# microsoft/singleshotpose

Hardware: AMD Instinct MI355X
Metric: images/sec (fwd+bwd) yolo-pose 416x416 bs=64/GPU (higher is better)
Workload: dtype f32; 1 GPU; cfg/yolo-pose.cfg train step (zero_grad+fwd+RegionLoss+bwd+grad all-reduce+SGD), 416x416, batch 64/GPU, random-init weights, 1 label/image; global_batch=64, parallelism=dp1

## Files before the change

include/ssp_hip.h:

```cpp
#ifndef SSP_HIP_H
#define SSP_HIP_H
#include <stdint.h>

#ifdef __cplusplus
extern "C" {
#endif

const char* ssp_last_error(void);
int ssp_abi_version(void);
int ssp_set_option(const char* name, int value);


int ssp_conv_fwd(const float* in, const float* wt, float* out, const float* bias, float* stats, int B, int H, int W,
                 int Cin, int Cout, int ldin, int ldout, int R, int accumulate, int plan, float* workspace,
                 int64_t workspace_floats, void* stream);
int ssp_conv_fwd_affine(const float* in, const float* wt, float* out, const float* scale, const float* shift,
                        float slope, int B, int H, int W, int Cin, int Cout, int ldin, int ldout, int R, int plan,
                        float* workspace, int64_t workspace_floats, void* stream);
int ssp_conv_stats_tile_m(int B, int H, int W, int Cin, int Cout, int R, int plan);
int ssp_conv_stats_tiles(int B, int H, int W, int Cin, int Cout, int R, int plan);
int64_t ssp_conv_stats_floats(int B, int H, int W, int Cin, int Cout, int R, int plan);
int ssp_conv_plan_wino_tile(int plan);
int64_t ssp_conv_wino_tiles(int B, int H, int W, int tile);
int ssp_wino_filter_transform_t(const float* w9, float* U, int rows, int K, int tile, void* stream);
int ssp_wino_filter_transform(const float* w9, float* U, int rows, int K, void* stream);
int64_t ssp_conv_workspace_floats(int B, int H, int W, int Cin, int Cout, int R, int plan);

int ssp_conv_dgrad(const float* dy, const float* wt, float* dx, int B, int H, int W, int Cout_dy, int Cin_dx, int lddy,
                   int lddx, int R, int accumulate, int plan, float* workspace, int64_t workspace_floats,
                   void* stream);

int ssp_conv_dgrad_bnbwd(const float* dy, const float* wt, float* dx, int B, int H, int W, int Cout_dy, int Cin_dx,
                         int lddy, int lddx, int R, int plan, float* workspace, int64_t workspace_floats,
                         const float* raw, int ldraw, const float* scale, const float* shift, const float* mean,
                         const float* invstd, float slope, float* partial, int partial_rows, void* stream);

int ssp_conv_wgrad(const float* dy, const float* x, float* dw, int B, int H, int W, int Cin, int Cout, int lddy,
                   int ldx, int R, void* stream);
int ssp_conv_wgrad_route(int B, int H, int W, int Cin, int Cout, int lddy, int ldx, int R);
int64_t ssp_conv_wgrad_wino_workspace_floats_t(int B, int H, int W, int Cin, int Cout, int tile);
int ssp_wino_input_transform_t(const float* x, int ldx, float* V, int B, int H, int W, int C, int tile, void* stream);
int ssp_conv_wgrad_wino_t(const float* dy, const float* x, float* dw, int B, int H, int W, int Cin, int Cout, int lddy,
                          int ldx, int tile, float* workspace, int64_t workspace_floats, void* stream);
int64_t ssp_conv_wgrad_wino_workspace_floats(int B, int H, int W, int Cin, int Cout);
int ssp_conv_wgrad_wino(const float* dy, const float* x, float* dw, int B, int H, int W, int Cin, int Cout, int lddy,
                        int ldx, float* workspace, int64_t workspace_floats, void* stream);

int ssp_bn_fwd_finalize(const float* stats, int ntile, int tile_m, int M, int C, const float* gamma,
                        const float* beta, float* running_mean, float* running_var, float momentum, float eps,
                        float* mean, float* invstd, float* scale, float* shift, void* stream);
int ssp_bn_eval_prepare(int C, const float* gamma, const float* beta, const float* running_mean,
                        const float* running_var, float eps, float* mean, float* invstd, float* scale, float* shift,
                        void* stream);
int ssp_bn_act_fwd(const float* x, int ldx, float* out, int ldo, const float* scale, const float* shift, int C, int B,
                   int H, int W, int pool, float slope, void* stream);
int ssp_bn_bwd_blocks(void);
int ssp_bn_act_bwd(const float* x, int ldx, const float* g, int ldg, float* dx, int lddx, const float* scale,
                   const float* shift, const float* mean, const float* invstd, int C, int B, int H, int W, int pool,
                   float slope, int training, float* partial, float* dgamma, float* dbeta, float* c1, float* c2,
                   void* stream);
int ssp_bn_act_bwd_partials(const float* x, int ldx, const float* g, int ldg, float* dx, int lddx, const float* scale,
                            const float* shift, const float* mean, const float* invstd, int C, int B, int H, int W,
                            float slope, int training, float* partial, int npartial, int zero_after, float* dgamma,
                            float* dbeta, float* c1, float* c2, void* stream);
int ssp_bn_act_bwd_affine(const float* x, int ldx, const float* g, int ldg, float* dx, int lddx, const float* scale,
                          const float* shift, const float* mean, const float* invstd, int C, int B, int H, int W, int pool,
                          float slope, void* stream);
int ssp_bn_bwd_finalize(float* partial, int npartial, int C, int64_t npix, int training, int zero_after, float* dgamma,
                        float* dbeta, float* c1, float* c2, void* stream);
int ssp_colsum(const float* g, int ldg, int64_t M, int C, float* out, void* stream);

int ssp_first_tile_pixels(void);
int ssp_first_groups(int B, int H, int W);
int ssp_first_fwd_stats(const float* x, const float* wt, float* stats, int B, int H, int W, void* stream);
int ssp_first_fwd_apply(const float* x, const float* wt, const float* scale, const float* shift, float slope, float* out,
                        int ldo, int B, int H, int W, void* stream);
int ssp_first_conv_raw(const float* x, const float* wt, float* raw, int ldraw, int B, int H, int W, void* stream);
int ssp_first_bwd_reduce(const float* x, const float* wt, const float* g, int ldg, const float* scale, const float* shift,
                         const float* mean, const float* invstd, float slope, float* partial, int B, int H, int W,
                         void* stream);
int ssp_first_bwd_wgrad(const float* x, const float* wt, const float* g, int ldg, const float* scale, const float* shift,
                        const float* mean, const float* invstd, const float* c1, const float* c2, float slope, float* dw,
                        float* workspace, int64_t workspace_floats, int B, int H, int W, void* stream);
int64_t ssp_first_wgrad_workspace_floats(int B, int H, int W);
int ssp_first_bwd_dgrad(const float* x, const float* wt, const float* g, int ldg, const float* scale, const float* shift,
                        const float* mean, const float* invstd, const float* c1, const float* c2, float slope, float* dx,
                        int B, int H, int W, void* stream);

int ssp_sgd_step(float* param, const float* grad, float* momentum_buf, int64_t n, float lr, float momentum,
                 float dampening, float weight_decay, int nesterov, int first_step, void* stream);
#define SSP_SGD_MAX_TUPLES 16
int ssp_sgd_step_table(float* param, const float* grad, float* momentum_buf, int64_t param_floats, int64_t grad_floats,
                       int64_t momentum_floats, const int64_t* table_dev, const int64_t* table_host, int nseg,
                       const float* hyper, int ntuple, void* stream);

int ssp_nchw_to_nhwc(const float* src, float* dst, int B, int C, int H, int W, int Cpad, int ld, void* stream);
int ssp_nhwc_to_nchw(const float* src, float* dst, int B, int C, int H, int W, int ld, void* stream);
int ssp_u8hwc_to_nhwc(const unsigned char* src, float* dst, int B, int H, int W, int C, int Cpad, int ld, void* stream);
typedef struct SspResampleDesc {
  const void* src;
  void* dst;
  const void* bounds;
  const void* kk;
  const void* img;
  const void* mask;
  const void* lut;
  int src_w, src_h, src_pitch;
  int x0, y0;
  int row0;
  int dst_w, dst_h, dst_pitch;
  int ksize, img_pitch, reserved;
} SspResampleDesc;
int ssp_resample_u8(const SspResampleDesc* descs_dev, int count, int pass, int epilogue, int max_dst_pixels, void* stream);
#define SSP_COMPOSITE_MAX_OBJS 8
typedef struct SspCompositeDesc {
  const void* scene;
  const void* scene_mask;
  const void* bg;
  void* out;
  const void* obj[SSP_COMPOSITE_MAX_OBJS];
  const void* obj_mask[SSP_COMPOSITE_MAX_OBJS];
  long long nbytes;
  int nobj, reserved;
} SspCompositeDesc;
int ssp_composite_u8(const SspCompositeDesc* descs_dev, int count, long long max_bytes, void* stream);
int ssp_distort_u8(const unsigned char* rgb, unsigned char* out, int64_t npix, const unsigned char* lut, int mode, void* stream);
int ssp_repack_fwd(const float* w, float* out, int Cout, int Cin, int Cinp, int R, void* stream);
int ssp_repack_dgrad(const float* w, float* out, int Cout, int Cin, int Coutp, int R, void* stream);
int ssp_repack_dgrad_packed(const float* wp, float* out, int Cout, int Cin, int Coutp, int R, void* stream);
int ssp_unpack_grad(const float* dwp, float* grad, int Cout, int Cin, int Cinp, int R, void* stream);
int ssp_reorg(const float* src, int lds, float* dst, int ldd, int C, int B, int H, int W, int backward,
              int accumulate, void* stream);
int ssp_copy_channels(const float* src, int lds, float* dst, int ldd, int C, int64_t M, int accumulate, void* stream);
int ssp_maxpool_fwd(const float* x, int ldx, float* out, int ldo, int C, int B, int H, int W, void* stream);
int ssp_maxpool_bwd(const float* x, int ldx, const float* g, int ldg, float* dx, int lddx, int C, int B, int H, int W,
                    int accumulate, void* stream);

int ssp_maxpool_s1_fwd(const float* x, int ldx, float* out, int ldo, int C, int B, int H, int W, void* stream);
int ssp_maxpool_s1_bwd(const float* x, int ldx, const float* g, int ldg, float* dx, int lddx, int C, int B, int H, int W,
                       int accumulate, void* stream);
int ssp_shortcut_fwd(const float* a, int lda, const float* b, int ldb, float* out, int ldo, int C, int64_t M, float slope,
                     void* stream);
int ssp_shortcut_bwd(const float* g, int ldg, const float* out, int ldo, float* da, int ldda, int acc_a, float* db, int lddb,
                     int acc_b, int C, int64_t M, float slope, void* stream);
int ssp_avgpool_fwd(const float* x, int ldx, float* out, int ldo, int C, int B, int H, int W, void* stream);
int ssp_avgpool_bwd(const float* g, int ldg, float* dx, int lddx, int C, int B, int H, int W, int accumulate, void* stream);
int ssp_softmax_fwd(const float* x, int ldx, float* y, int ldy, int C, int64_t M, void* stream);
int ssp_softmax_bwd(const float* y, int ldy, const float* g, int ldg, float* dx, int lddx, int C, int64_t M, int accumulate,
                    void* stream);

int ssp_region_loss(const float* out, const void* target, int target_is_f64, float* grad, float* partials,
                    float* stats, int nB, int nA, int nC, int nH, int nW, int num_keypoints, float noobject_scale,
                    float object_scale, float coord_scale, float class_scale, float thresh, int conf_on, int multi,
                    const float* anchors, int anchor_step, void* stream);
int ssp_region_decode_argmax(const float* out, float* boxes, int nB, int nA, int nC, int nH, int nW,
                             int num_keypoints, int only_objectness, void* stream);

int ssp_region_decode_all(const float* out, float* rows, int nB, int nA, int nC, int nH, int nW, int num_keypoints,
                          void* stream);

int ssp_region_match_multi(const float* out, const float* target, float* rows, int* meta, int nB, int nA, int nC, int nH,
                           int nW, int num_keypoints, float conf_thresh, int only_objectness, int im_width, int im_height,
                           void* stream);

int ssp_pnp_batched(const double* pts3d, const double* pts2d, const double* K, double* Rt, int n, int N, int max_iter,
                    void* stream);

int ssp_pose_errors(const double* vertices, int N, const double* Rt_gt, const double* Rt_pr, const double* K,
                    int k_per_pose, int n, double* out, void* stream);
int ssp_pts_diameter(const double* pts, int N, double* out, double* scratch, void* stream);
int ssp_pose_errors_models(const double* verts, const int* model_off, const int* pose_model, int nM, const double* Rt_gt,
                           const double* Rt_pr, const double* K, int k_per_pose, int n, double* out, void* stream);
int64_t ssp_adds_workspace_doubles(int n, int maxN);
int ssp_adds_errors(const double* verts, const int* model_off, const int* pose_model, int nM, int maxN,
                    const double* Rt_gt, const double* Rt_pr, int n, double* out, double* workspace,
                    int64_t workspace_doubles, void* stream);

int ssp_prof_enable(int mask);
int ssp_prof_nkinds(void);
int ssp_prof_collect(double* ms, double* work, int64_t* count);

#ifdef __cplusplus
}
#endif
#endif
```

singleshotpose_amd/_lib.py:

```python
import ctypes
import os
from ctypes import c_char_p, c_double, c_float, c_int, c_int64, c_void_p

_HERE = os.path.dirname(os.path.abspath(__file__))
LIB_PATH = os.environ.get("SSP_HIP_LIB") or os.path.join(_HERE, "libssp_hip.so")


class SspError(RuntimeError):
    pass


_lib = None

P = c_void_p
I = c_int
F = c_float
L = c_int64

_SIGS = {
    "ssp_abi_version": [],
    "ssp_set_option": [c_char_p, I],
    "ssp_conv_fwd": [P, P, P, P, P, I, I, I, I, I, I, I, I, I, I, P, L, P],
    "ssp_conv_fwd_affine": [P, P, P, P, P, F, I, I, I, I, I, I, I, I, I, P, L, P],
    "ssp_conv_stats_tile_m": [I, I, I, I, I, I, I],
    "ssp_conv_workspace_floats": [I, I, I, I, I, I, I],
    "ssp_conv_stats_tiles": [I, I, I, I, I, I, I],
    "ssp_conv_stats_floats": [I, I, I, I, I, I, I],
    "ssp_conv_plan_wino_tile": [I],
    "ssp_conv_wino_tiles": [I, I, I, I],
    "ssp_wino_filter_transform": [P, P, I, I, P],
    "ssp_wino_filter_transform_t": [P, P, I, I, I, P],
    "ssp_conv_dgrad": [P, P, P, I, I, I, I, I, I, I, I, I, I, P, L, P],
    "ssp_conv_dgrad_bnbwd": [P, P, P, I, I, I, I, I, I, I, I, I, P, L, P, I, P, P, P, P, F, P, I, P],
    "ssp_bn_act_bwd_partials": [P, I, P, I, P, I, P, P, P, P, I, I, I, I, F, I, P, I, I, P, P, P, P, P],
    "ssp_conv_wgrad": [P, P, P, I, I, I, I, I, I, I, I, P],
    "ssp_conv_wgrad_route": [I, I, I, I, I, I, I, I],
    "ssp_conv_wgrad_wino": [P, P, P, I, I, I, I, I, I, I, P, L, P],
    "ssp_conv_wgrad_wino_workspace_floats": [I, I, I, I, I],
    "ssp_conv_wgrad_wino_t": [P, P, P, I, I, I, I, I, I, I, I, P, L, P],
    "ssp_conv_wgrad_wino_workspace_floats_t": [I, I, I, I, I, I],
    "ssp_bn_fwd_finalize": [P, I, I, I, I, P, P, P, P, F, F, P, P, P, P, P],
    "ssp_bn_eval_prepare": [I, P, P, P, P, F, P, P, P, P, P],
    "ssp_bn_act_fwd": [P, I, P, I, P, P, I, I, I, I, I, F, P],
    "ssp_bn_bwd_blocks": [],
    "ssp_bn_act_bwd": [P, I, P, I, P, I, P, P, P, P, I, I, I, I, I, F, I, P, P, P, P, P, P],
    "ssp_bn_act_bwd_affine": [P, I, P, I, P, I, P, P, P, P, I, I, I, I, I, F, P],
    "ssp_bn_bwd_finalize": [P, I, I, L, I, I, P, P, P, P, P],
    "ssp_first_tile_pixels": [],
    "ssp_first_groups": [I, I, I],
    "ssp_first_fwd_stats": [P, P, P, I, I, I, P],
    "ssp_first_fwd_apply": [P, P, P, P, F, P, I, I, I, I, P],
    "ssp_first_conv_raw": [P, P, P, I, I, I, I, P],
    "ssp_first_bwd_reduce": [P, P, P, I, P, P, P, P, F, P, I, I, I, P],
    "ssp_first_bwd_wgrad": [P, P, P, I, P, P, P, P, P, P, F, P, P, L, I, I, I, P],
    "ssp_first_bwd_dgrad": [P, P, P, I, P, P, P, P, P, P, F, P, I, I, I, P],
    "ssp_wino_input_transform_t": [P, I, P, I, I, I, I, I, P],
    "ssp_first_wgrad_workspace_floats": [I, I, I],
    "ssp_colsum": [P, I, L, I, P, P],
    "ssp_pose_errors": [P, I, P, P, P, I, I, P, P],
    "ssp_pts_diameter": [P, I, P, P, P],
    "ssp_pose_errors_models": [P, P, P, I, P, P, P, I, I, P, P],
    "ssp_adds_workspace_doubles": [I, I],
    "ssp_adds_errors": [P, P, P, I, I, P, P, I, P, P, L, P],
    "ssp_sgd_step": [P, P, P, L, F, F, F, F, I, I, P],
    "ssp_sgd_step_table": [P, P, P, L, L, L, P, P, I, P, I, P],
    "ssp_nchw_to_nhwc": [P, P, I, I, I, I, I, I, P],
    "ssp_nhwc_to_nchw": [P, P, I, I, I, I, I, P],
    "ssp_u8hwc_to_nhwc": [P, P, I, I, I, I, I, I, P],
    "ssp_resample_u8": [P, I, I, I, I, P],
    "ssp_distort_u8": [P, P, L, P, I, P],
    "ssp_composite_u8": [P, I, L, P],
    "ssp_repack_fwd": [P, P, I, I, I, I, P],
    "ssp_repack_dgrad": [P, P, I, I, I, I, P],
    "ssp_repack_dgrad_packed": [P, P, I, I, I, I, P],
    "ssp_unpack_grad": [P, P, I, I, I, I, P],
    "ssp_reorg": [P, I, P, I, I, I, I, I, I, I, P],
    "ssp_copy_channels": [P, I, P, I, I, L, I, P],
    "ssp_maxpool_fwd": [P, I, P, I, I, I, I, I, P],
    "ssp_maxpool_bwd": [P, I, P, I, P, I, I, I, I, I, I, P],
    "ssp_maxpool_s1_fwd": [P, I, P, I, I, I, I, I, P],
    "ssp_maxpool_s1_bwd": [P, I, P, I, P, I, I, I, I, I, I, P],
    "ssp_shortcut_fwd": [P, I, P, I, P, I, I, L, F, P],
    "ssp_shortcut_bwd": [P, I, P, I, P, I, I, P, I, I, I, L, F, P],
    "ssp_avgpool_fwd": [P, I, P, I, I, I, I, I, P],
    "ssp_avgpool_bwd": [P, I, P, I, I, I, I, I, I, P],
    "ssp_softmax_fwd": [P, I, P, I, I, L, P],
    "ssp_softmax_bwd": [P, I, P, I, P, I, I, L, I, P],
    "ssp_region_loss": [P, P, I, P, P, P, I, I, I, I, I, I, F, F, F, F, F, I, I, P, I, P],
    "ssp_region_decode_argmax": [P, P, I, I, I, I, I, I, I, P],
    "ssp_region_decode_all": [P, P, I, I, I, I, I, I, P],
    "ssp_region_match_multi": [P, P, P, P, I, I, I, I, I, I, F, I, I, I, P],
    "ssp_pnp_batched": [P, P, P, P, I, I, I, P],
    "ssp_prof_enable": [I],
    "ssp_prof_nkinds": [],
    "ssp_prof_collect": [P, P, P],
}

_RET64 = ('ssp_conv_workspace_floats', 'ssp_conv_wgrad_wino_workspace_floats', 'ssp_conv_wgrad_wino_workspace_floats_t',
          'ssp_conv_stats_floats', 'ssp_conv_wino_tiles', 'ssp_first_wgrad_workspace_floats', 'ssp_adds_workspace_doubles')

PROF_KINDS = ("conv_fwd", "conv_dgrad", "conv_wgrad", "bn_act", "layout", "region", "optim", "first_block_fwd",
              "first_block_bwd", "wino_fwd", "wino_dgrad", "wino_wgrad", "onchip_fwd", "onchip_dgrad", "onchip_wgrad")


def csrc_digest():
    import glob
    import hashlib
    h = hashlib.sha1()
    files = sorted(glob.glob(os.path.join(_HERE, 'csrc', '*.hip')) + glob.glob(os.path.join(_HERE, 'csrc', '*.h')))
    files.append(os.path.join(os.path.dirname(_HERE), 'include', 'ssp_hip.h'))
    for f in files:
        h.update(os.path.basename(f).encode())
        with open(f, 'rb') as fp:
            h.update(fp.read())
    return h.hexdigest()


def exported_symbols():
    return ["ssp_last_error"] + list(_SIGS.keys())


def load():
    global _lib
    if _lib is not None:
        return _lib
    if not os.path.exists(LIB_PATH):
        raise SspError(
            "libssp_hip.so not found at %s - build it with `python -c 'import __graft_entry__ as g; g.build()'` "
            "or `make -C singleshotpose_amd/csrc`; there is no CPU fallback for the HIP path" % LIB_PATH)
    lib = ctypes.CDLL(LIB_PATH)
    lib.ssp_last_error.restype = c_char_p
    lib.ssp_last_error.argtypes = []
    for name, args in _SIGS.items():
        fn = getattr(lib, name)
        fn.restype = c_int64 if name in _RET64 else c_int
        fn.argtypes = args
    _lib = lib
    return lib


PROF_MASK = [0]


def call(name, *args):
    lib = load()
    if name == 'ssp_prof_enable':
        PROF_MASK[0] = int(args[0])
    rc = getattr(lib, name)(*args)
    if rc != 0:
        msg = lib.ssp_last_error()
        raise SspError("%s failed (%d): %s" % (name, rc, msg.decode() if msg else "?"))
    return rc


def query(name, *args):
    return getattr(load(), name)(*args)
```

singleshotpose_amd/csrc/conv_igemm.hip:

```cpp
#include "conv_igemm_common.h"
#include "conv_wino.h"

template <int BM, int BN, int WM, int WN, int BK, int ABL = 0, int PASS = 0>
__global__ void __launch_bounds__(WM* WN * 64, 2) conv_igemm_kernel(ConvArgs p) {
  constexpr int NT = WM * WN * 64;
  constexpr int LS = BK + 4;
  constexpr int TPR = BK / 4;
  constexpr int RPP = NT / TPR;
  constexpr int APASS = (BM + RPP - 1) / RPP;
  constexpr int BPASS = (BN + RPP - 1) / RPP;
  constexpr int WTM = BM / WM, WTN = BN / WN;
  constexpr int TM = WTM / 32, TN = WTN / 32;
  constexpr int VEC = (BK >= 8) ? 4 : 2;
  constexpr int NQ = BK / (2 * VEC);
  constexpr int SLOT = (BM + BN) * LS;
  static_assert(WTM % 32 == 0 && WTN % 32 == 0, "wave tile must be a multiple of the 32x32 MFMA");
  static_assert(NQ >= 1, "BK too small");

  extern __shared__ __attribute__((aligned(16))) float smem[];

  const int ntiles = p.ntile_m * p.ntile_n;
  const int nwg = ntiles * p.ksplit;
  const int lid0 = p.xcd_remap ? ssp_xcd_remap(blockIdx.x, nwg) : (int)blockIdx.x;
  const int split = lid0 / ntiles, lid = lid0 - split * ntiles;
// ... 264 lines not shown
        const float d = v[k] - mean[k];
        mean[k] += d * inv;
        m2[k] += d * (v[k] - mean[k]);
      }
      float* dst = out + (int64_t)m * ldout + c;
      f32x4 o = {v[0] * e4[0] + b4[0], v[1] * e4[1] + b4[1], v[2] * e4[2] + b4[2], v[3] * e4[3] + b4[3]};
#pragma unroll
      for (int k = 0; k < 4; ++k) o[k] = o[k] > 0.f ? o[k] : o[k] * act_slope;
      if (accumulate) {
        const f32x4 prev = *reinterpret_cast<const f32x4*>(dst);
        o[0] += prev[0]; o[1] += prev[1]; o[2] += prev[2]; o[3] += prev[3];
      }
      *reinterpret_cast<f32x4*>(dst) = o;
      if (bnb) {
        const f32x4 xr = *reinterpret_cast<const f32x4*>(bn_raw + (int64_t)m * bn_ld + c);
#pragma unroll
        for (int k = 0; k < 4; ++k) {
          const float y = xr[k] * bsc[k] + bsh[k];
          const float dyv = y > 0.f ? o[k] : o[k] * bn_slope;
          s1[k] += dyv;
          s2[k] += dyv * ((xr[k] - bmu[k]) * bis[k]);
        }
      }
    }
  }
  __shared__ float red[16][16][9];
  if (bnb) {
#pragma unroll
    for (int k = 0; k < 4; ++k) { red[pp][gl][1 + k] = s1[k]; red[pp][gl][5 + k] = s2[k]; }
    __syncthreads();
    if (tid < 64) {
      const int q = tid >> 2, k = tid & 3;
      const int ch = blockIdx.y * 64 + tid;
      if (ch < Cout) {
        float a = 0.f, b = 0.f;
        for (int w = 0; w < 16; ++w) { a += red[w][q][1 + k]; b += red[w][q][5 + k]; }
        const int t = m0 / tile_m;
        if (ntile_all > bn_nslot) {
          float* dst = bn_partial + ((int64_t)(t % bn_nslot) * Cout + ch) * 2;
          atomicAdd(dst, a);
          atomicAdd(dst + 1, b);
        } else {
          float* dst = bn_partial + ((int64_t)t * Cout + ch) * 2;
          dst[0] = a;
          dst[1] = b;
        }
      }
    }
    return;
  }
  if (stats == nullptr) return;
  red[pp][gl][0] = cnt;
#pragma unroll
  for (int k = 0; k < 4; ++k) { red[pp][gl][1 + k] = mean[k]; red[pp][gl][5 + k] = m2[k]; }
  __syncthreads();
  if (tid < 64) {
    const int q = tid >> 2, k = tid & 3;
    const int ch = blockIdx.y * 64 + tid;
    if (ch < Cout) {
      float n_ = red[0][q][0], mu = red[0][q][1 + k], s2 = red[0][q][5 + k];
      for (int w = 1; w < 16; ++w) chan_combine(n_, mu, s2, red[w][q][0], red[w][q][1 + k], red[w][q][5 + k]);
      float* st = stats + ((int64_t)(m0 / tile_m) * Cout + ch) * 2;
      st[0] = mu;
      st[1] = s2;
    }
  }
}

template <int BM, int BN, int WM, int WN, int BK, int ABL = 0, int PASS = 0>
static int launch_cfg(ConvArgs a, hipStream_t stream, int extra_lds = 0) {
  a.ntile_m = ssp_cdiv(a.M, BM);
  a.ntile_n = ssp_cdiv(a.Cout, BN);
  const int niter_total = a.R * a.R * (a.Cin / BK);
  a.it_per_split = ssp_cdiv(niter_total, a.ksplit);
  a.ksplit = ssp_cdiv(niter_total, a.it_per_split);
  dim3 grid(a.ntile_m * a.ntile_n * a.ksplit), block(WM * WN * 64);
  const int lds_bytes = 3 * (BM + BN) * (BK + 4) * 4 + extra_lds;
  auto kern = conv_igemm_kernel<BM, BN, WM, WN, BK, ABL, PASS>;
  static SspKernelCache cache;
  if (int rc = ssp_kernel_prepare((const void*)kern, lds_bytes, WM * WN * 64, &cache, nullptr, "conv_igemm")) return rc;
  hipLaunchKernelGGL(kern, grid, block, lds_bytes, stream, a);
  SSP_CHECK_LAUNCH("conv_igemm");
  return SSP_OK;
}

int ssp_conv_igemm_dma_launch(ConvArgs& a, int bm, int slots, int tail_ks, int is_dgrad, hipStream_t stream);

struct IgemmPlan { int bm, ksplit, slots, tail; };
static IgemmPlan select_plan(int M, int Cin, int Cout, int R, int plan_code) {
  IgemmPlan pl = {256, 1, 0, 0};
  if (Cout <= 64) {
    if (Cout > 32 && Cin % 16 == 0 && ssp_option(SSP_OPT_IGEMM_VARIANT) != 50) pl.bm = 128;
    if (Cin % 16 == 0 && Cout % 4 == 0 && ssp_option(SSP_OPT_IGEMM_VARIANT) != 50 && ssp_option(SSP_OPT_IGEMM_VARIANT) != 30) {
      const int64_t tiles = ssp_cdiv(M, pl.bm);
      const int niter = R * R * (Cin / 16);
      if (tiles < 256) {
        int64_t ks = 512 / tiles;
        if (ks > niter / 8) ks = niter / 8;
        if (ks > 8) ks = 8;
        if (ks >= 2) pl.ksplit = (int)ks;
      }
    }
    return pl;
  }
  pl.bm = 128;
  const int forced = plan_code > 0 ? plan_code : ssp_option(SSP_OPT_IGEMM_PLAN);
  if (forced > 0) {
    const int ftail = forced / 100000, fbm = (forced / 100) % 1000, fks = (forced / 10) % 10, fsl = forced % 10;
    const int niter16 = (Cin % 16 == 0) ? R * R * (Cin / 16) : 0;
    const bool ok = (fbm == 64 || fbm == 128) && fks >= 1 && (fsl == 3 || fsl == 4 || fsl == 8) &&
                    (fks == 1 || (niter16 / fks >= 8 && Cout % 4 == 0)) && Cin % 16 == 0 &&
                    (ftail == 0 || (ftail >= 2 && ftail <= 9 && fks == 1 && Cout % 4 == 0 && niter16 / ftail >= 8));
    if (ok) { pl.bm = fbm; pl.ksplit = fks; pl.slots = fsl; pl.tail = ftail; return pl; }
  }
  const int variant = ssp_option(SSP_OPT_IGEMM_VARIANT);
  if (variant == 20 || variant == 22) { pl.bm = 64; return pl; }
  if (variant >= 70 && variant <= 75) {
    const int niter = R * R * (Cin / 16);
    if (Cin % 16 == 0 && Cout % 4 == 0 && niter / (variant - 68) >= 8) pl.ksplit = variant - 68;
    return pl;
  }
  if (variant != 0 && variant != 30 && variant != 50 && variant != 61 && variant != 62 && variant != 63) return pl;
  const int64_t t128 = (int64_t)ssp_cdiv(M, 128) * ssp_cdiv(Cout, 128);
  const int64_t t64 = (int64_t)ssp_cdiv(M, 64) * ssp_cdiv(Cout, 128);
  if (t128 > 1400) return pl;
  auto wave_eff = [](int64_t wgs, int slots) { return (double)wgs / (double)(((wgs + slots - 1) / slots) * slots); };
  double best = wave_eff(t128, 512);
  const double e64 = 0.97 * wave_eff(t64, 768);
  if (e64 > best) { best = e64; pl.bm = 64; }
  if (variant == 30 || Cin % 16 != 0 || Cout % 4 != 0) return pl;
  const int niter = R * R * (Cin / 16);
  const double flop_time = 2.0 * M * (double)Cout * R * R * Cin / 110e12;
  for (int sp = 2; sp <= 6; ++sp) {
    if (niter / sp < 128) break;
    const double traffic = (2.0 * sp + 1.0) * (double)M * Cout * 4.0 / 4.0e12;
    const double eff = wave_eff(t128 * sp, 512) / (1.0 + traffic / flop_time);
    if (eff > best + 0.02) { best = eff; pl.bm = 128; pl.ksplit = sp; }
  }
  return pl;
}
int ssp_conv_tile_m(int M, int Cin, int Cout, int R, int plan) {
  if (ssp_wino_plan_tile(plan)) return 0;
  return select_plan(M, Cin, Cout, R, plan).bm;
}
int64_t ssp_conv_ws_floats(int M, int Cin, int Cout, int R, int plan) {
  IgemmPlan pl = select_plan(M, Cin, Cout, R, plan);
  const int deepest = pl.ksplit > pl.tail ? pl.ksplit : pl.tail;
  return deepest > 1 ? (int64_t)deepest * M * Cout : 0;
}

int64_t ssp_wino_ws_floats(int B, int H, int W, int Cin, int Cout, int tile) {
  return ssp_wino_planes(tile) * ssp_wino_tiles(B, H, W, tile) * ((int64_t)Cin + Cout);
}

static int wino_launch(ConvArgs& a, int B, int H, int W, float* ws, int64_t ws_floats, int plan, int prof_kind,
                       hipStream_t stream) {
  const int bm = (plan / 100) % 1000, slots = plan % 10, tile = ssp_wino_plan_tile(plan), P = ssp_wino_planes(tile);
  SSP_CHECK_ARG(a.R == 3 && a.Cin % 16 == 0 && a.Cout >= 64 && a.Cout % 4 == 0 && a.ldout % 4 == 0 && (((uintptr_t)a.out) & 15) == 0,
                "conv (Winograd plan): needs a 3x3 filter, Cin %% 16 == 0, Cout >= 64 and %% 4 == 0, an aligned output");
  SSP_CHECK_ARG((bm == 64 || bm == 128) && (slots == 3 || slots == 4 || slots == 8) && (plan / 10) % 10 == 1 &&
                    (plan / 100000) % 10 == 0, "conv: bad Winograd plan code %d", plan);
  const int64_t T = ssp_wino_tiles(B, H, W, tile);
  SSP_CHECK_ARG(T < (1ll << 31) && P * T * (int64_t)a.Cin < (1ll << 40), "conv (Winograd plan): too many tiles");
  SSP_CHECK_ARG(ws != nullptr && ws_floats >= ssp_wino_ws_floats(B, H, W, a.Cin, a.Cout, tile) && (((uintptr_t)ws) & 15) == 0,
                "conv (Winograd plan): needs a workspace of %lld floats (ssp_conv_workspace_floats)",
                (long long)ssp_wino_ws_floats(B, H, W, a.Cin, a.Cout, tile));
  SSP_CHECK_ARG((int64_t)(128 + 2) * a.Cin * 4 + (int64_t)a.Cin * 4 < (1ll << 31), "conv (Winograd plan): Cin too large");
  if (a.bn_partial != nullptr) SSP_CHECK_ARG(a.bn_ld % 4 == 0, "conv (Winograd plan): bn_ld must be a multiple of 4");
  SspProfScope prof(prof_kind, stream, 2.0 * (double)a.M * a.Cout * 9.0 * a.Cin);
  float* V = ws;
  float* Mw = ws + P * T * a.Cin;
  const int wkind = prof_kind == SSP_PROF_CONV_DGRAD ? SSP_PROF_WINO_DGRAD : SSP_PROF_WINO_FWD;
  if (int rc = ssp_wino_input_launch(a.in, a.ldin, V, B, H, W, a.Cin, tile, wkind, stream)) return rc;
  ConvArgs g = a;
  g.in = V; g.wt = a.wt; g.out = Mw; g.bias = nullptr; g.escale = nullptr; g.act_slope = 1.f; g.stats = nullptr;
  g.H = 1; g.W = (int)T; g.ldin = a.Cin; g.ldout = a.Cout; g.R = 1; g.M = (int)T; g.accumulate = 0;
  g.divW = ssp_fastdiv((unsigned)T); g.divH = ssp_fastdiv(1u);
  g.ws = nullptr; g.ksplit = 1; g.probe = 0;
  g.bn_partial = nullptr; g.bn_raw = nullptr;
  g.batch = P; g.batch_in = T * a.Cin; g.batch_wt = (int64_t)a.Cout * a.Cin; g.batch_out = T * a.Cout;
  if (int rc = ssp_conv_igemm_dma_launch(g, bm, slots, 0, prof_kind == SSP_PROF_CONV_DGRAD, stream)) return rc;
  WinoOutArgs o;
  o.Mw = Mw; o.out = a.out; o.bias = a.bias; o.escale = a.escale; o.act_slope = a.act_slope; o.stats = a.stats;
  o.Cout = a.Cout; o.ldout = a.ldout; o.accumulate = a.accumulate;
  o.bn_raw = a.bn_raw; o.bn_scale = a.bn_scale; o.bn_shift = a.bn_shift; o.bn_mean = a.bn_mean; o.bn_invstd = a.bn_invstd;
  o.bn_partial = a.bn_partial; o.bn_nslot = a.bn_nslot; o.bn_ld = a.bn_ld; o.bn_slope = a.bn_slope;
  return ssp_wino_output_launch(o, B, H, W, tile, wkind, stream);
}

int ssp_conv_igemm_launch(const float* in, const float* wt, float* out, const float* bias, float* stats, int B, int H,
                          int W, int Cin, int Cout, int ldin, int ldout, int R, int accumulate, float* ws,
                          int64_t ws_floats, int plan, int prof_kind, hipStream_t stream, const float* escale,
                          float act_slope, const SspBnBwdFuse* bnb) {
  SSP_CHECK_ARG(R == 1 || R == 3, "conv: only 1x1 and 3x3 filters are supported (got %d)", R);
  SSP_CHECK_ARG(Cin % 4 == 0 && Cin > 0, "conv: Cin must be a positive multiple of 4 (got %d)", Cin);
  SSP_CHECK_ARG(ldin % 4 == 0 && ldin >= Cin, "conv: ldin must be a multiple of 4 and >= Cin");
  SSP_CHECK_ARG(ldout >= Cout && Cout > 0, "conv: ldout < Cout");
  SSP_CHECK_ARG((int64_t)B * H * W < (1ll << 31), "conv: too many pixels");
  SSP_CHECK_ARG((((uintptr_t)in) & 15) == 0 && (((uintptr_t)wt) & 15) == 0, "conv: in/wt must be 16-byte aligned");
  ConvArgs a;
  a.in = in; a.wt = wt; a.out = out; a.bias = bias; a.stats = stats; a.escale = escale; a.act_slope = act_slope;
  a.H = H; a.W = W; a.Cin = Cin; a.Cout = Cout; a.ldin = ldin; a.ldout = ldout; a.R = R;
  a.M = B * H * W; a.accumulate = accumulate;
  a.divW = ssp_fastdiv((unsigned)W); a.divH = ssp_fastdiv((unsigned)H);
  a.xcd_remap = ssp_option(SSP_OPT_IGEMM_XCD);
  a.probe = ssp_option(SSP_OPT_IGEMM_VARIANT) == 63 ? 2 : 0;
  a.tail_begin = 0; a.tail_ks = 0; a.tail_it_per_split = 0; a.ws_row0 = 0; a.ws_rows = a.M; a.col_major = 0;
  a.bn_raw = nullptr; a.bn_scale = a.bn_shift = a.bn_mean = a.bn_invstd = nullptr; a.bn_partial = nullptr;
  a.bn_ld = 0; a.bn_slope = 1.f; a.bn_nslot = 1;
  a.batch = 0; a.batch_in = a.batch_wt = a.batch_out = 0;
  if (bnb != nullptr && bnb->partial != nullptr) {
    SSP_CHECK_ARG(accumulate == 0 && bias == nullptr && stats == nullptr && escale == nullptr,
                  "conv: the fused BatchNorm-backward reductions need a plain (non-accumulating) data-gradient launch");
    SSP_CHECK_ARG(bnb->raw != nullptr && bnb->scale != nullptr && bnb->shift != nullptr && bnb->mean != nullptr &&
                  bnb->invstd != nullptr && bnb->ldraw >= Cout && Cout % 4 == 0 && bnb->ldraw % 4 == 0 &&
                  ((((uintptr_t)bnb->raw) | ((uintptr_t)bnb->scale) | ((uintptr_t)bnb->shift) | ((uintptr_t)bnb->mean) |
                    ((uintptr_t)bnb->invstd)) & 15) == 0,
                  "conv: bad BatchNorm-backward operands (16-byte aligned, Cout %% 4 == 0, ldraw >= Cout)");
    a.bn_raw = bnb->raw; a.bn_ld = bnb->ldraw; a.bn_scale = bnb->scale; a.bn_shift = bnb->shift; a.bn_mean = bnb->mean;
    a.bn_invstd = bnb->invstd; a.bn_slope = bnb->slope; a.bn_partial = bnb->partial;
    SSP_CHECK_ARG(bnb->nslot >= 1, "conv: the BatchNorm-backward partial buffer needs at least one row");
    a.bn_nslot = bnb->nslot;
  }
  if (ssp_wino_plan_fused(plan)) {
    a.ksplit = 1; a.ws = nullptr;
    return ssp_wino_fused_launch(a, B, H, W, prof_kind, stream);
  }
  if (ssp_wino_plan_tile(plan)) return wino_launch(a, B, H, W, ws, ws_floats, plan, prof_kind, stream);
  IgemmPlan pl = select_plan(a.M, Cin, Cout, R, plan);
  if (Cout <= 64 && pl.ksplit > 1 &&
      (ws == nullptr || ws_floats < (int64_t)pl.ksplit * a.M * Cout || ldout % 4 != 0 || (((uintptr_t)out) & 15) != 0))
    pl.ksplit = 1;
  a.ksplit = pl.ksplit;
  a.ws = ws;
  if (pl.ksplit > 1)
    SSP_CHECK_ARG(ldout % 4 == 0 && (((uintptr_t)out) & 15) == 0, "conv: split-K output must be 16-byte aligned with ldout % 4 == 0");
  if (pl.ksplit > 1)
    SSP_CHECK_ARG(ws != nullptr && ws_floats >= (int64_t)pl.ksplit * a.M * Cout,
                  "conv: this shape runs split-K x%d and needs a workspace of %lld floats (ssp_conv_workspace_floats)",
                  pl.ksplit, (long long)pl.ksplit * a.M * Cout);
  if (pl.tail > 1) {
    SSP_CHECK_ARG(ws != nullptr && ws_floats >= (int64_t)pl.tail * a.M * Cout && ldout % 4 == 0 && (((uintptr_t)out) & 15) == 0,
                  "conv: the hybrid plan (tail split x%d) needs an aligned output and a workspace of %lld floats "
                  "(ssp_conv_workspace_floats)", pl.tail, (long long)pl.tail * a.M * Cout);
  }
  SspProfScope prof(prof_kind, stream, 2.0 * (double)a.M * Cout * (double)(R * R * Cin));
  const int variant = ssp_option(SSP_OPT_IGEMM_VARIANT);
  const int bk = (Cin % 32 == 0 && (variant == 2 || variant == 4 || variant == 5)) ? 32 : ((Cin % 16 == 0) ? 16 : 4);
  int rc = SSP_OK;
  if (Cout > 64) {
    switch (variant) {
      case 3: if (bk >= 16) return launch_cfg<256, 128, 4, 2, 16>(a, stream); break;
      case 4: if (bk == 32) return launch_cfg<128, 128, 2, 2, 32, 1>(a, stream); break;
      case 5: if (bk == 32) return launch_cfg<128, 128, 2, 2, 32, 2>(a, stream); break;
#ifdef SSP_PROBES
      case 10: if (bk >= 16) return launch_cfg<128, 128, 2, 2, 16, 1>(a, stream); break;
      case 14: if (bk >= 16) return launch_cfg<128, 128, 2, 2, 16, 1 | 4 | 8 | 16>(a, stream); break;
      case 17: if (bk >= 16) return launch_cfg<128, 128, 2, 2, 16, 1 | 4 | 8 | 16 | 32>(a, stream); break;
      case 40: if (bk >= 16) return launch_cfg<128, 128, 2, 2, 16, 29 | 64>(a, stream); break;
      case 41: if (bk >= 16) return launch_cfg<128, 128, 2, 2, 16, 29 | 128>(a, stream); break;
      case 42: if (bk >= 16) return launch_cfg<128, 128, 2, 2, 16, 29 | 256>(a, stream); break;
      case 43: if (bk >= 16) return launch_cfg<128, 128, 2, 2, 16, 29 | 64 | 128 | 256>(a, stream); break;
      case 18: if (bk >= 16) return launch_cfg<128, 128, 2, 2, 16, 32>(a, stream); break;
#endif
      case 21: if (bk >= 16) return launch_cfg<128, 64, 2, 2, 16>(a, stream); break;
      case 22: if (bk >= 16) return launch_cfg<64, 64, 2, 2, 16>(a, stream); break;
      default: break;
    }
    if (bk >= 16 && variant != 50 && ((int64_t)(128 + 2 * W + 2) * ldin * 4 + (int64_t)Cin * 4 < (1ll << 31))) {
      rc = ssp_conv_igemm_dma_launch(a, pl.bm, pl.slots, pl.tail, prof_kind == SSP_PROF_CONV_DGRAD, stream);
    } else if (pl.bm == 64) {
      rc = (bk >= 16) ? launch_cfg<64, 128, 2, 2, 16>(a, stream)
                      : (prof_kind == SSP_PROF_CONV_DGRAD ? launch_cfg<64, 128, 2, 2, 4, 0, 1>(a, stream) : launch_cfg<64, 128, 2, 2, 4>(a, stream));
    } else if (bk == 32) {
      rc = launch_cfg<128, 128, 2, 2, 32>(a, stream);
    } else if (bk == 16) {
      rc = launch_cfg<128, 128, 2, 2, 16>(a, stream);
    } else {
      rc = prof_kind == SSP_PROF_CONV_DGRAD ? launch_cfg<128, 128, 2, 2, 4, 0, 1>(a, stream) : launch_cfg<128, 128, 2, 2, 4>(a, stream);
    }
  } else if (Cout > 32) {
    if (pl.bm == 128) {
      SSP_CHECK_ARG((int64_t)(128 + 2 * W + 2) * ldin * 4 + (int64_t)Cin * 4 < (1ll << 31),
                    "conv: image rows too long for the 32-bit tile offsets of the LDS-direct loader");
      rc = ssp_conv_igemm_dma_launch(a, 128, 0, 0, prof_kind == SSP_PROF_CONV_DGRAD, stream);
    } else
      rc = (bk >= 16) ? launch_cfg<256, 64, 4, 1, 16>(a, stream) : launch_cfg<256, 64, 4, 1, 4>(a, stream);
  } else if (bk >= 16 && variant != 50 && ((int64_t)(256 + 2 * W + 2) * ldin * 4 + (int64_t)Cin * 4 < (1ll << 31))) {
    rc = ssp_conv_igemm_dma_launch(a, 256, 0, 0, prof_kind == SSP_PROF_CONV_DGRAD, stream);
  } else {
    rc = (bk >= 16) ? launch_cfg<256, 32, 4, 1, 16>(a, stream) : launch_cfg<256, 32, 4, 1, 4>(a, stream);
  }
  if (rc != SSP_OK) return rc;
  const int rt = (stats == nullptr && a.bn_partial == nullptr && a.M <= 16384) ? 16 : pl.bm;
  if (pl.ksplit > 1) {
    hipLaunchKernelGGL(splitk_reduce_kernel, dim3(ssp_cdiv(a.M, rt), ssp_cdiv(Cout, 64)), dim3(256), 0, stream, ws, pl.ksplit, out, ldout,
                       bias, stats, a.M, Cout, rt, accumulate, escale, act_slope, 0, a.bn_raw, a.bn_ld, a.bn_scale,
                       a.bn_shift, a.bn_mean, a.bn_invstd, a.bn_slope, a.bn_partial, a.bn_nslot, ssp_cdiv(a.M, pl.bm));
    SSP_CHECK_LAUNCH("splitk_reduce");
  } else if (a.tail_ks > 1) {
    hipLaunchKernelGGL(splitk_reduce_kernel, dim3(ssp_cdiv(a.M - a.ws_row0, rt), ssp_cdiv(Cout, 64)), dim3(256), 0, stream, ws,
                       a.tail_ks, out, ldout, bias, stats, a.M, Cout, rt, accumulate, escale, act_slope, a.ws_row0,
                       a.bn_raw, a.bn_ld, a.bn_scale, a.bn_shift, a.bn_mean, a.bn_invstd, a.bn_slope, a.bn_partial, a.bn_nslot,
                       ssp_cdiv(a.M, pl.bm));
    SSP_CHECK_LAUNCH("splitk_reduce(tail)");
  }
  return SSP_OK;
}
```

singleshotpose_amd/csrc/conv_wgrad.hip:

```cpp
#include "conv_wino.h"

struct WgradArgs {
  const float* dy;
  const float* x;
  float* dw;
  int H, W, Cin, Cout, lddy, ldx, R, M;
  int ntile_co, ntile_ci, nsplit, chunk_m;
};

template <int BMO, int BNI, int WM, int WN, int WK>
__global__ void __launch_bounds__(256, 2) conv_wgrad_kernel(WgradArgs p) {
  static_assert(WM * WN * WK == 4, "256-thread workgroups");
  constexpr int NT = 256;
  constexpr int RA = 16 * WK;
  constexpr int WTM = BMO / WM, WTN = BNI / WN;
  constexpr int TM = WTM / 32, TN = WTN / 32;
  constexpr int F4A = RA * BMO / 4, F4B = RA * BNI / 4;
  constexpr int APASS = (F4A + NT - 1) / NT, BPASS = (F4B + NT - 1) / NT;
  constexpr int SLOT = RA * (BMO + BNI);
  static_assert(WTM % 32 == 0 && WTN % 32 == 0, "wave tile must be a multiple of 32x32");

  extern __shared__ __attribute__((aligned(16))) float smem[];

  const int taps = p.R * p.R;
// ... 198 lines not shown
      }
      g_reg[i] = v;
    }
  };
  auto store_lds = [&](int buf) {
#pragma unroll
    for (int i = 0; i < 2; ++i)
      *reinterpret_cast<f32x4v*>(As + (buf * RA + a_row0 + i * 32) * LSA + a_c4) = a_reg[i];
#pragma unroll
    for (int i = 0; i < 3; ++i) {
      const int tap = g_tap0 + 4 * i;
      if (tap < 9) *reinterpret_cast<f32x4v*>(Bs + (buf * RA + g_pix) * LSB + tap * 4) = g_reg[i];
    }
  };

  f32x4v acc[2][3];
#pragma unroll
  for (int i = 0; i < 2; ++i)
#pragma unroll
    for (int j = 0; j < 3; ++j) acc[i][j] = f32x4v{0.f, 0.f, 0.f, 0.f};

  load_global(0);
  store_lds(0);
  __syncthreads();
  const int li = lane & 15, lk = lane >> 4;
  for (int it = 0; it < niter; ++it) {
    const int buf = it & 1;
    if (it + 1 < niter) load_global(it + 1);
    const float* Ab = As + (buf * RA + wid * 16 + lk) * LSA + li;
    const float* Bb = Bs + (buf * RA + wid * 16 + lk) * LSB + li;
#pragma unroll
    for (int kk = 0; kk < 4; ++kk) {
      float av[2], bv[3];
#pragma unroll
      for (int i = 0; i < 2; ++i) av[i] = Ab[kk * 4 * LSA + i * 16];
#pragma unroll
      for (int j = 0; j < 3; ++j) bv[j] = Bb[kk * 4 * LSB + j * 16];
#pragma unroll
      for (int i = 0; i < 2; ++i)
#pragma unroll
        for (int j = 0; j < 3; ++j) acc[i][j] = __builtin_amdgcn_mfma_f32_16x16x4f32(av[i], bv[j], acc[i][j], 0, 0, 0);
    }
    if (it + 1 < niter) store_lds(buf ^ 1);
    __syncthreads();
  }

  float* red = smem;
#pragma unroll
  for (int i = 0; i < 2; ++i)
#pragma unroll
    for (int j = 0; j < 3; ++j)
#pragma unroll
      for (int r = 0; r < 4; ++r) red[(wid * CO + i * 16 + lk * 4 + r) * NCOL + j * 16 + li] = acc[i][j][r];
  __syncthreads();
  for (int e = tid; e < CO * 36; e += 256) {
    int co = e / 36, col = e % 36;
    float v = red[(0 * CO + co) * NCOL + col] + red[(1 * CO + co) * NCOL + col] + red[(2 * CO + co) * NCOL + col] +
              red[(3 * CO + co) * NCOL + col];
    atomicAdd(p.dw + co * 36 + col, v);
  }
}

template <int BMO, int BNI, int WM, int WN, int WK>
static int launch_wgrad(WgradArgs a, hipStream_t stream) {
  constexpr int RA = 16 * WK;
  a.ntile_co = ssp_cdiv(a.Cout, BMO);
  a.ntile_ci = ssp_cdiv(a.Cin, BNI);
  const int64_t tiles = (int64_t)a.ntile_co * a.ntile_ci * a.R * a.R;
  const int lds_bytes = 3 * RA * (BMO + BNI) * 4;
  auto kern = conv_wgrad_kernel<BMO, BNI, WM, WN, WK>;
  static SspKernelCache cache;
  int slots = 0;
  if (int rc = ssp_kernel_prepare((const void*)kern, lds_bytes, 256, &cache, &slots, "conv_wgrad")) return rc;
  const int64_t max_split = (a.M + RA * 8 - 1) / (RA * 8);
  int64_t lo = (2 * (int64_t)slots + tiles - 1) / tiles, hi = (5 * (int64_t)slots) / tiles;
  if (lo < 1) lo = 1;
  if (hi < lo) hi = lo;
  if (lo > max_split) lo = max_split;
  if (hi > max_split) hi = max_split;
  int64_t nsplit = lo;
  double best = -1.0;
  for (int64_t sp = lo; sp <= hi; ++sp) {
    const double waves = (double)(tiles * sp) / slots;
    const double eff = waves / (double)((tiles * sp + slots - 1) / slots);
    if (eff > best + 1e-3) { best = eff; nsplit = sp; }
  }
  int64_t chunk = (a.M + nsplit - 1) / nsplit;
  chunk = (chunk + RA - 1) / RA * RA;
  nsplit = (a.M + chunk - 1) / chunk;
  a.nsplit = (int)nsplit;
  a.chunk_m = (int)chunk;
  dim3 grid((unsigned)(tiles * nsplit)), block(256);
  hipLaunchKernelGGL(kern, grid, block, lds_bytes, stream, a);
  SSP_CHECK_LAUNCH("conv_wgrad");
  return SSP_OK;
}

int ssp_conv_wgrad_dma_try(const float* dy, const float* x, float* dw, int B, int H, int W, int Cin, int Cout, int lddy,
                           int ldx, int R, hipStream_t stream, int batch = 0, int64_t batch_dy = 0, int64_t batch_x = 0,
                           int64_t batch_dw = 0, int overwrite = 0);

int ssp_conv_wgrad_launch(const float* dy, const float* x, float* dw, int B, int H, int W, int Cin, int Cout,
                          int lddy, int ldx, int R, hipStream_t stream) {
  SSP_CHECK_ARG(R == 1 || R == 3, "wgrad: only 1x1 and 3x3 filters are supported (got %d)", R);
  SSP_CHECK_ARG(Cin % 4 == 0 && Cin > 0, "wgrad: Cin must be a positive multiple of 4 (got %d)", Cin);
  SSP_CHECK_ARG(ldx % 4 == 0 && ldx >= Cin, "wgrad: ldx must be a multiple of 4 and >= Cin");
  SSP_CHECK_ARG(lddy % 4 == 0 && lddy >= Cout, "wgrad: lddy must be a multiple of 4 and >= Cout");
  SSP_CHECK_ARG((int64_t)B * H * W < (1ll << 31), "wgrad: too many pixels");
  SSP_CHECK_ARG((((uintptr_t)dy) & 15) == 0 && (((uintptr_t)x) & 15) == 0, "wgrad: dy/x must be 16-byte aligned");
  WgradArgs a;
  a.dy = dy; a.x = x; a.dw = dw;
  a.H = H; a.W = W; a.Cin = Cin; a.Cout = Cout; a.lddy = lddy; a.ldx = ldx; a.R = R; a.M = B * H * W;
  SspProfScope prof(SSP_PROF_CONV_WGRAD, stream, 2.0 * (double)a.M * Cout * (double)(R * R * Cin));
  const int route = ssp_wgrad_route(B, H, W, Cin, Cout, lddy, ldx, R, 0, ssp_option(SSP_OPT_WGRAD_VARIANT));
  if (route / 100000000 == SSP_WGRAD_LDS) {
    const int r = ssp_conv_wgrad_dma_try(dy, x, dw, B, H, W, Cin, Cout, lddy, ldx, R, stream);
    if (r != 0) return r < 0 ? r : SSP_OK;
    ssp_set_error("wgrad: the LDS-direct launcher declined route %d", route);
    return SSP_ERR_ARG;
  }
  switch (route) {
    case ssp_wgrad_code(SSP_WGRAD_C4, 2, false, false, 32, 4): {
      int64_t chunk = (a.M + 2047) / 2048;
      chunk = (chunk + 63) / 64 * 64;
      a.chunk_m = (int)chunk;
      a.nsplit = ssp_cdiv(a.M, chunk);
      hipLaunchKernelGGL(conv_wgrad_c4_kernel, dim3(a.nsplit), dim3(256), 0, stream, a);
      SSP_CHECK_LAUNCH("conv_wgrad_c4");
      return SSP_OK;
    }
    case ssp_wgrad_code(SSP_WGRAD_REG, 3, false, false, 128, 128): return launch_wgrad<128, 128, 2, 2, 1>(a, stream);
    case ssp_wgrad_code(SSP_WGRAD_REG, 3, false, false, 128, 64): return launch_wgrad<128, 64, 2, 2, 1>(a, stream);
    case ssp_wgrad_code(SSP_WGRAD_REG, 3, false, false, 128, 32): return launch_wgrad<128, 32, 4, 1, 1>(a, stream);
    case ssp_wgrad_code(SSP_WGRAD_REG, 3, false, false, 64, 128): return launch_wgrad<64, 128, 2, 2, 1>(a, stream);
    case ssp_wgrad_code(SSP_WGRAD_REG, 3, false, false, 64, 64): return launch_wgrad<64, 64, 2, 2, 1>(a, stream);
    case ssp_wgrad_code(SSP_WGRAD_REG, 3, false, false, 64, 32): return launch_wgrad<64, 32, 2, 1, 2>(a, stream);
    case ssp_wgrad_code(SSP_WGRAD_REG, 3, false, false, 32, 128): return launch_wgrad<32, 128, 1, 4, 1>(a, stream);
    case ssp_wgrad_code(SSP_WGRAD_REG, 3, false, false, 32, 64): return launch_wgrad<32, 64, 1, 2, 2>(a, stream);
    case ssp_wgrad_code(SSP_WGRAD_REG, 3, false, false, 32, 32): return launch_wgrad<32, 32, 1, 1, 4>(a, stream);
  }
  ssp_set_error("wgrad: no instantiation for route %d", route);
  return SSP_ERR_ARG;
}


int64_t ssp_conv_wgrad_wino_ws_floats(int B, int H, int W, int Cin, int Cout, int tile) {
  if (tile == SSP_WINO_WGRAD_FUSED) return ssp_wino_wgrad_fused_ws_floats(Cin, Cout);
  if (tile != 2 && tile != 4) return 0;
  const int64_t T = ssp_wino_tiles(B, H, W, tile);
  return ssp_wino_planes(tile) * (T * ((int64_t)Cin + Cout) + (int64_t)Cin * Cout);
}
int ssp_conv_wgrad_wino_launch(const float* dy, const float* x, float* dw, int B, int H, int W, int Cin, int Cout, int lddy,
                               int ldx, int tile, float* ws, int64_t ws_floats, hipStream_t stream) {
  if (tile == SSP_WINO_WGRAD_FUSED) return ssp_wino_wgrad_fused_launch(dy, x, dw, B, H, W, Cin, Cout, lddy, ldx, ws, ws_floats, stream);
  SSP_CHECK_ARG(tile == 2 || tile == 4, "wgrad (Winograd): tile must be 2, 4 or 12 (F(2x2) with both transforms on the chip)");
  SSP_CHECK_ARG(Cin % 16 == 0 && Cout % 16 == 0 && Cin >= 64 && Cout >= 64, "wgrad (Winograd): needs Cin, Cout >= 64 and %% 16 == 0");
  SSP_CHECK_ARG(ldx % 4 == 0 && ldx >= Cin && lddy % 4 == 0 && lddy >= Cout, "wgrad (Winograd): bad leading dimensions");
  SSP_CHECK_ARG((((uintptr_t)dy) | ((uintptr_t)x) | ((uintptr_t)dw) | ((uintptr_t)ws)) % 16 == 0, "wgrad (Winograd): operands must be 16-byte aligned");
  const int64_t T = ssp_wino_tiles(B, H, W, tile);
  const int P = ssp_wino_planes(tile);
  SSP_CHECK_ARG(T >= 16 && T < (1ll << 31), "wgrad (Winograd): tile count out of range (>= 16 tiles)");
  SSP_CHECK_ARG(ws != nullptr && ws_floats >= ssp_conv_wgrad_wino_ws_floats(B, H, W, Cin, Cout, tile),
                "wgrad (Winograd): needs a workspace of %lld floats (ssp_conv_wgrad_wino_workspace_floats)",
                (long long)ssp_conv_wgrad_wino_ws_floats(B, H, W, Cin, Cout, tile));
  SspProfScope prof(SSP_PROF_CONV_WGRAD, stream, 2.0 * (double)B * H * W * Cout * 9.0 * Cin);
  float* V = ws;
  float* dM = V + P * T * Cin;
  float* dU = dM + P * T * Cout;
  if (x != nullptr)
    if (int rc = ssp_wino_input_launch(x, ldx, V, B, H, W, Cin, tile, SSP_PROF_WINO_WGRAD, stream)) return rc;
  if (int rc = ssp_wino_outgrad_launch(dy, lddy, dM, B, H, W, Cout, tile, stream)) return rc;
  const int r = ssp_conv_wgrad_dma_try(dM, V, dU, 1, 1, (int)T, Cin, Cout, Cout, Cin, 1, stream, P, T * Cout, T * Cin,
                                       (int64_t)Cout * Cin, 1);
  if (r < 0) return r;
  SSP_CHECK_ARG(r == 1, "wgrad (Winograd): shape declined by the LDS-direct filter-gradient kernel");
  return ssp_wino_wgrad_finish_launch(dU, dw, Cout, Cin, tile, stream);
}
```

singleshotpose_amd/csrc/conv_wino.h:

```cpp
#pragma once
#include "ssp_common.h"

#define SSP_WINO2_PLAN 9000000
#define SSP_WINO4_PLAN 8000000
#define SSP_WINOF_PLAN 7000000
static inline int ssp_wino_plan_fused(int plan) { return plan >= SSP_WINOF_PLAN && plan < SSP_WINOF_PLAN + 1000000; }
static inline int ssp_wino_plan_tile(int plan) {
  if (plan >= SSP_WINO2_PLAN && plan < SSP_WINO2_PLAN + 1000000) return 2;
  if (plan >= SSP_WINO4_PLAN && plan < SSP_WINO4_PLAN + 1000000) return 4;
  if (ssp_wino_plan_fused(plan)) return 2;
  return 0;
}

#define SSP_WINO_TG 16

struct WinoOutArgs {
  const float* Mw;
  float* out;
  const float* bias;
  const float* escale;
  float act_slope;
  float* stats;
  int Cout, ldout, accumulate;
  const float* bn_raw;
  const float* bn_scale;
  const float* bn_shift;
  const float* bn_mean;
  const float* bn_invstd;
  float* bn_partial;
  int bn_nslot, bn_ld;
  float bn_slope;
};

int64_t ssp_wino_tiles(int B, int H, int W, int tile);
int ssp_wino_planes(int tile);
int64_t ssp_wino_stat_groups(int B, int H, int W, int tile);
int ssp_wino_input_launch(const float* in, int ldin, float* V, int B, int H, int W, int C, int tile, int prof_kind, hipStream_t stream);
int ssp_wino_filter_launch(const float* w, float* U, int rows, int K, int tile, hipStream_t stream);
int ssp_wino_outgrad_launch(const float* dy, int lddy, float* dM, int B, int H, int W, int C, int tile, hipStream_t stream);
int ssp_wino_wgrad_finish_launch(const float* dU, float* dw, int rows, int K, int tile, hipStream_t stream);
int ssp_wino_output_launch(const WinoOutArgs& a, int B, int H, int W, int tile, int prof_kind, hipStream_t stream);

struct ConvArgs;
int ssp_wino_fused_launch(const ConvArgs& a, int B, int H, int W, int prof_kind, hipStream_t stream);
int ssp_wino_fused_stat_groups(int B, int H, int W, int Cout);
bool ssp_wino_fused_fits(int B, int H, int W, int Cin, int Cout, int R);

#define SSP_WINO_WGRAD_FUSED 12
int ssp_wino_wgrad_fused_launch(const float* dy, const float* x, float* dw, int B, int H, int W, int Cin, int Cout, int lddy,
                                int ldx, float* ws, int64_t ws_floats, hipStream_t stream);
int64_t ssp_wino_wgrad_fused_ws_floats(int Cin, int Cout);
bool ssp_wino_wgrad_fused_fits(int B, int H, int W, int Cin, int Cout);
```

singleshotpose_amd/csrc/conv_wino.hip:

```cpp
#include <utility>

#include "conv_wino.h"

template <typename F, int... Is>
__device__ __forceinline__ void ssp_sfor_impl(F&& f, std::integer_sequence<int, Is...>) {
  (f(std::integral_constant<int, Is>{}), ...);
}
template <int N, typename F>
__device__ __forceinline__ void ssp_sfor(F&& f) {
  ssp_sfor_impl(f, std::make_integer_sequence<int, N>{});
}

template <typename V>
__device__ __forceinline__ void wino_mad(V& acc, const float c, const V& x) {
  if (c == 1.f) acc += x;
  else if (c == -1.f) acc -= x;
  else if (c != 0.f) acc += x * c;
}

template <int N> struct WinoMat;
template <> struct WinoMat<2> {
  static constexpr int A = 4;
  static constexpr float BT[4][4] = {{1.f, 0.f, -1.f, 0.f}, {0.f, 1.f, 1.f, 0.f}, {0.f, -1.f, 1.f, 0.f}, {0.f, 1.f, 0.f, -1.f}};
  static constexpr float G[4][3] = {{1.f, 0.f, 0.f}, {0.5f, 0.5f, 0.5f}, {0.5f, -0.5f, 0.5f}, {0.f, 0.f, 1.f}};
  static constexpr float AT[2][4] = {{1.f, 1.f, 1.f, 0.f}, {0.f, 1.f, -1.f, -1.f}};
};
template <> struct WinoMat<4> {
  static constexpr int A = 6;
  static constexpr float BT[6][6] = {{1.f, -1.5f, -2.f, 1.5f, 1.f, 0.f},
                                     {0.f, -1.f, 0.5f, 2.5f, 1.f, 0.f},
                                     {0.f, 1.f, -2.5f, 0.5f, 1.f, 0.f},
                                     {0.f, -2.f, -1.f, 2.f, 1.f, 0.f},
                                     {0.f, 0.5f, -1.f, -0.5f, 1.f, 0.f},
                                     {0.f, 1.f, -1.5f, -2.f, 1.5f, 1.f}};
  static constexpr float G[6][3] = {{1.f, 0.f, 0.f},
                                    {1.f / 3.f, 1.f / 3.f, 1.f / 3.f},
                                    {-1.f / 3.f, 1.f / 3.f, -1.f / 3.f},
                                    {-16.f / 15.f, -8.f / 15.f, -4.f / 15.f},
                                    {1.f / 15.f, -2.f / 15.f, 4.f / 15.f},
                                    {0.f, 0.f, 1.f}};
  static constexpr float AT[4][6] = {{1.f, 1.f, 1.f, 1.f, 1.f, 0.f},
                                     {0.f, 1.f, -1.f, 0.5f, -2.f, 0.f},
                                     {0.f, 1.f, 1.f, 0.25f, 4.f, 0.f},
                                     {0.f, 1.f, -1.f, 0.125f, -8.f, 1.f}};
};

struct WinoGeom {
  int H, W, th, tw;
  int64_t T;
  SspFastDiv div_tw, div_th;
  int G, B;
};
static WinoGeom wino_geom(int B, int H, int W, int tile) {
  WinoGeom g;
  g.H = H; g.W = W; g.B = B; g.G = 1;
  g.th = (H + tile - 1) / tile; g.tw = (W + tile - 1) / tile;
  g.T = (int64_t)B * g.th * g.tw;
  const int mth = (2 * H + 1 + tile - 1) / tile, mtw = (2 * W + 1 + tile - 1) / tile;
  const int64_t mT = (int64_t)((B + 3) / 4) * mth * mtw;
  if (mT < g.T) { g.G = 2; g.th = mth; g.tw = mtw; g.T = mT; }
  g.div_tw = ssp_fastdiv((unsigned)g.tw); g.div_th = ssp_fastdiv((unsigned)g.th);
  return g;
}
__device__ __forceinline__ bool wino_map(const WinoGeom& g, int mb, int Y, int X, int& b, int& y, int& x) {
  if (g.G == 1) {
    b = mb; y = Y; x = X;
    return ((unsigned)Y < (unsigned)g.H) && ((unsigned)X < (unsigned)g.W);
  }
  const int iy = Y > g.H ? 1 : 0, ix = X > g.W ? 1 : 0;
  y = Y - iy * (g.H + 1);
  x = X - ix * (g.W + 1);
  b = mb * 4 + iy * 2 + ix;
  return (Y >= 0) && (X >= 0) && (y < g.H) && (x < g.W) && (b < g.B);
}

template <int N, int CV, bool NT = false>
__global__ void __launch_bounds__(256) wino_input_kernel(const float* __restrict__ in, int ldin, float* __restrict__ V, int C,
                                                         WinoGeom g, SspFastDiv div_cg) {
  constexpr int A = N + 2;
  using M_ = WinoMat<N>;
  typedef float vec __attribute__((ext_vector_type(CV)));
  const int64_t gid = (int64_t)ssp_xcd_remap((int)blockIdx.x, (int)gridDim.x) * 256 + threadIdx.x;
  const int cgn = C / CV;
  if (gid >= g.T * cgn) return;
  const unsigned t = ssp_div((unsigned)gid, div_cg);
  const int c = (int)((unsigned)gid - t * (unsigned)cgn) * CV;
  const unsigned q = ssp_div(t, g.div_tw);
  const int tx = (int)(t - q * (unsigned)g.tw);
  const unsigned mb = ssp_div(q, g.div_th);
  const int ty = (int)(q - mb * (unsigned)g.th);
  const int y0 = N * ty - 1, x0 = N * tx - 1;
  const float* base = in + c;
  vec d[A][A];
#pragma unroll
  for (int i = 0; i < A; ++i) {
#pragma unroll
    for (int j = 0; j < A; ++j) {
      int b, y, x;
      const bool ok = wino_map(g, (int)mb, y0 + i, x0 + j, b, y, x);
      vec z;
#pragma unroll
      for (int k = 0; k < CV; ++k) z[k] = 0.f;
      d[i][j] = ok ? *reinterpret_cast<const vec*>(base + (((int64_t)b * g.H + y) * g.W + x) * ldin) : z;
    }
  }
  vec r[A][A];
  ssp_sfor<A>([&](auto I) {
    constexpr int i = decltype(I)::value;
    ssp_sfor<A>([&](auto J) {
      constexpr int j = decltype(J)::value;
      vec a;
#pragma unroll
      for (int k = 0; k < CV; ++k) a[k] = 0.f;
      ssp_sfor<A>([&](auto K) {
        constexpr int k = decltype(K)::value;
        { constexpr float cc_ = M_::BT[i][k]; wino_mad(a, cc_, d[k][j]); }
      });
      r[i][j] = a;
    });
  });
  float* dst = V + (int64_t)t * C + c;
  const int64_t plane = g.T * C;
  ssp_sfor<A>([&](auto I) {
    constexpr int i = decltype(I)::value;
    ssp_sfor<A>([&](auto J) {
      constexpr int j = decltype(J)::value;
      vec a;
#pragma unroll
      for (int k = 0; k < CV; ++k) a[k] = 0.f;
      ssp_sfor<A>([&](auto K) {
        constexpr int k = decltype(K)::value;
        { constexpr float cc_ = M_::BT[j][k]; wino_mad(a, cc_, r[i][k]); }
      });
      if constexpr (NT) __builtin_nontemporal_store(a, reinterpret_cast<vec*>(dst + (int64_t)(i * A + j) * plane));
      else *reinterpret_cast<vec*>(dst + (int64_t)(i * A + j) * plane) = a;
    });
  });
}

template <int N>
__global__ void __launch_bounds__(256) wino_filter_kernel(const float* __restrict__ w, float* __restrict__ U, int rows, int K) {
  constexpr int A = N + 2;
  using M_ = WinoMat<N>;
  const int64_t gid = (int64_t)blockIdx.x * 256 + threadIdx.x;
  const int k4n = K >> 2;
  if (gid >= (int64_t)rows * k4n) return;
  const int row = (int)(gid / k4n);
  const int k = (int)(gid - (int64_t)row * k4n) * 4;
  const float* src = w + ((int64_t)row * 9) * K + k;
  f32x4 g[3][3];
#pragma unroll
  for (int i = 0; i < 3; ++i)
#pragma unroll
    for (int j = 0; j < 3; ++j) g[i][j] = *reinterpret_cast<const f32x4*>(src + (int64_t)(i * 3 + j) * K);
  f32x4 h[A][3];
  ssp_sfor<A>([&](auto I) {
    constexpr int i = decltype(I)::value;
    ssp_sfor<3>([&](auto J) {
      constexpr int j = decltype(J)::value;
      f32x4 a = {0.f, 0.f, 0.f, 0.f};
      ssp_sfor<3>([&](auto Kk) {
        constexpr int kk = decltype(Kk)::value;
        { constexpr float cc_ = M_::G[i][kk]; wino_mad(a, cc_, g[kk][j]); }
      });
      h[i][j] = a;
    });
  });
  float* dst = U + (int64_t)row * K + k;
  const int64_t plane = (int64_t)rows * K;
  ssp_sfor<A>([&](auto I) {
    constexpr int i = decltype(I)::value;
    ssp_sfor<A>([&](auto J) {
      constexpr int j = decltype(J)::value;
      f32x4 a = {0.f, 0.f, 0.f, 0.f};
      ssp_sfor<3>([&](auto Kk) {
        constexpr int kk = decltype(Kk)::value;
        { constexpr float cc_ = M_::G[j][kk]; wino_mad(a, cc_, h[i][kk]); }
      });
      *reinterpret_cast<f32x4*>(dst + (int64_t)(i * A + j) * plane) = a;
    });
  });
}

template <int N, int CS>
__global__ void __launch_bounds__(256) wino_output_kernel(WinoOutArgs p, WinoGeom g) {
  constexpr int A = N + 2;
  constexpr int TP = 256 / CS;
  constexpr int NP = SSP_WINO_TG / TP;
  using M_ = WinoMat<N>;
  const int tid = threadIdx.x, gl = tid % CS, tl = tid / CS;
  const int c = blockIdx.y * (CS * 4) + gl * 4;
  const bool cok = c < p.Cout;
  const f32x4 z4 = {0.f, 0.f, 0.f, 0.f};
  f32x4 b4 = z4, e4 = {1.f, 1.f, 1.f, 1.f};
  if (cok && p.bias != nullptr) b4 = *reinterpret_cast<const f32x4*>(p.bias + c);
  if (cok && p.escale != nullptr) e4 = *reinterpret_cast<const f32x4*>(p.escale + c);
  const bool bnb = p.bn_partial != nullptr;
  const bool want_stats = p.stats != nullptr;
  f32x4 bsc = z4, bsh = z4, bmu = z4, bis = z4, s1 = z4, s2 = z4;
  if (bnb && cok) {
    bsc = *reinterpret_cast<const f32x4*>(p.bn_scale + c); bsh = *reinterpret_cast<const f32x4*>(p.bn_shift + c);
    bmu = *reinterpret_cast<const f32x4*>(p.bn_mean + c); bis = *reinterpret_cast<const f32x4*>(p.bn_invstd + c);
  }
  float rn = 0.f;
  f32x4 rmean = z4, rm2 = z4;
#pragma unroll 1
  for (int pass = 0; pass < NP; ++pass) {
    const int64_t t64 = (int64_t)blockIdx.x * SSP_WINO_TG + pass * TP + tl;
    const bool live = cok && (t64 < g.T);
    if (!live) continue;
    f32x4 Y[N][N];
#pragma unroll
    for (int i = 0; i < N; ++i)
#pragma unroll
      for (int j = 0; j < N; ++j) Y[i][j] = z4;
    const unsigned t = (unsigned)t64;
    const unsigned q = ssp_div(t, g.div_tw);
    const int tx = (int)(t - q * (unsigned)g.tw);
    const int mb = (int)ssp_div(q, g.div_th);
    const int ty = (int)(q - (unsigned)mb * (unsigned)g.th);
    const float* src = p.Mw + t64 * p.Cout + c;
    const int64_t plane = g.T * p.Cout;
    ssp_sfor<A>([&](auto I) {
      constexpr int i = decltype(I)::value;
      f32x4 m[A];
#pragma unroll
      for (int j = 0; j < A; ++j) m[j] = *reinterpret_cast<const f32x4*>(src + (int64_t)(i * A + j) * plane);
      ssp_sfor<N>([&](auto Q) {
        constexpr int qq = decltype(Q)::value;
        f32x4 rr = z4;
        ssp_sfor<A>([&](auto J) {
          constexpr int j = decltype(J)::value;
          { constexpr float cc_ = M_::AT[qq][j]; wino_mad(rr, cc_, m[j]); }
        });
        ssp_sfor<N>([&](auto Pp) {
          constexpr int pp = decltype(Pp)::value;
          { constexpr float cc_ = M_::AT[pp][i]; wino_mad(Y[pp][qq], cc_, rr); }
        });
      });
    });
    float cnt = 0.f;
    f32x4 sum = z4;
    unsigned valid = 0u;
#pragma unroll
    for (int i = 0; i < N; ++i) {
#pragma unroll
      for (int j = 0; j < N; ++j) {
        int b, y, x;
        if (wino_map(g, mb, N * ty + i, N * tx + j, b, y, x)) {
          valid |= 1u << (i * N + j);
          const f32x4 v = Y[i][j];
          cnt += 1.f;
          sum += v;
          const int64_t m = ((int64_t)b * g.H + y) * g.W + x;
          float* dst = p.out + m * p.ldout + c;
          f32x4 o = v * e4 + b4;
#pragma unroll
          for (int k = 0; k < 4; ++k) o[k] = o[k] > 0.f ? o[k] : o[k] * p.act_slope;
          if (p.accumulate) o += *reinterpret_cast<const f32x4*>(dst);
          *reinterpret_cast<f32x4*>(dst) = o;
          if (bnb) {
            const f32x4 xr = *reinterpret_cast<const f32x4*>(p.bn_raw + m * p.bn_ld + c);
#pragma unroll
            for (int k = 0; k < 4; ++k) {
              const float yy = xr[k] * bsc[k] + bsh[k];
              const float dyv = yy > 0.f ? o[k] : o[k] * p.bn_slope;
              s1[k] += dyv;
              s2[k] += dyv * ((xr[k] - bmu[k]) * bis[k]);
            }
          }
        }
      }
    }
    if (want_stats && cnt > 0.f) {
      const f32x4 mean = sum * (1.f / cnt);
      f32x4 m2 = z4;
#pragma unroll
      for (int i = 0; i < N; ++i)
#pragma unroll
        for (int j = 0; j < N; ++j)
          if ((valid >> (i * N + j)) & 1u) {
            const f32x4 dd = Y[i][j] - mean;
            m2 += dd * dd;
          }
      const float nt = rn + cnt, f = cnt / nt;
      const f32x4 dd = mean - rmean;
      rmean += dd * f;
      rm2 += m2 + dd * dd * (rn * f);
      rn = nt;
    }
  }
  __shared__ float red[TP][CS][9];
  if (bnb) {
#pragma unroll
    for (int k = 0; k < 4; ++k) { red[tl][gl][1 + k] = s1[k]; red[tl][gl][5 + k] = s2[k]; }
    __syncthreads();
    if (tid < CS * 4) {
      const int q = tid >> 2, k = tid & 3;
      const int ch = blockIdx.y * (CS * 4) + tid;
      if (ch < p.Cout) {
        float a = 0.f, bb = 0.f;
#pragma unroll
        for (int w = 0; w < TP; ++w) { a += red[w][q][1 + k]; bb += red[w][q][5 + k]; }
        if ((int)gridDim.x > p.bn_nslot) {
          float* dst = p.bn_partial + ((int64_t)(blockIdx.x % p.bn_nslot) * p.Cout + ch) * 2;
          atomicAdd(dst, a);
          atomicAdd(dst + 1, bb);
        } else {
          float* dst = p.bn_partial + ((int64_t)blockIdx.x * p.Cout + ch) * 2;
          dst[0] = a;
          dst[1] = bb;
        }
      }
    }
    return;
  }
  if (!want_stats) return;
  red[tl][gl][0] = rn;
#pragma unroll
  for (int k = 0; k < 4; ++k) { red[tl][gl][1 + k] = rmean[k]; red[tl][gl][5 + k] = rm2[k]; }
  __syncthreads();
  if (tid < CS * 4) {
    const int q = tid >> 2, k = tid & 3;
    const int ch = blockIdx.y * (CS * 4) + tid;
    if (ch < p.Cout) {
      float n_ = red[0][q][0], mu = red[0][q][1 + k], ss = red[0][q][5 + k];
#pragma unroll
      for (int w = 1; w < TP; ++w) {
        const float nb = red[w][q][0], mb = red[w][q][1 + k], m2b = red[w][q][5 + k];
        const float nt = n_ + nb;
        if (nt > 0.f) {
          const float dd = mb - mu, f = nb / nt;
          mu += dd * f;
          ss += m2b + dd * dd * n_ * f;
          n_ = nt;
        }
      }
      float* st = p.stats + ((int64_t)blockIdx.x * p.Cout + ch) * 2;
      st[0] = mu;
      st[1] = ss;
      if (ch == 0) p.stats[(int64_t)gridDim.x * p.Cout * 2 + blockIdx.x] = n_;
    }
  }
}

template <int N, int CV, bool NT = false>
__global__ void __launch_bounds__(256) wino_outgrad_kernel(const float* __restrict__ dy, int lddy, float* __restrict__ dM, int C,
                                                           WinoGeom g, SspFastDiv div_cg) {
  constexpr int A = N + 2;
  using M_ = WinoMat<N>;
  typedef float vec __attribute__((ext_vector_type(CV)));
  const int64_t gid = (int64_t)blockIdx.x * 256 + threadIdx.x;
  const int cgn = C / CV;
  if (gid >= g.T * cgn) return;
  const unsigned t = ssp_div((unsigned)gid, div_cg);
  const int c = (int)((unsigned)gid - t * (unsigned)cgn) * CV;
  const unsigned q = ssp_div(t, g.div_tw);
  const int tx = (int)(t - q * (unsigned)g.tw);
  const unsigned mb = ssp_div(q, g.div_th);
  const int ty = (int)(q - mb * (unsigned)g.th);
  const float* base = dy + c;
  vec d[N][N];
#pragma unroll
  for (int i = 0; i < N; ++i)
#pragma unroll
    for (int j = 0; j < N; ++j) {
      int b, y, x;
      const bool ok = wino_map(g, (int)mb, N * ty + i, N * tx + j, b, y, x);
      vec z;
#pragma unroll
      for (int k = 0; k < CV; ++k) z[k] = 0.f;
      d[i][j] = ok ? *reinterpret_cast<const vec*>(base + (((int64_t)b * g.H + y) * g.W + x) * lddy) : z;
    }
  vec r[A][N];
  ssp_sfor<A>([&](auto I) {
    constexpr int i = decltype(I)::value;
    ssp_sfor<N>([&](auto Q) {
      constexpr int qq = decltype(Q)::value;
      vec a;
#pragma unroll
      for (int k = 0; k < CV; ++k) a[k] = 0.f;
      ssp_sfor<N>([&](auto Pp) {
        constexpr int pp = decltype(Pp)::value;
        { constexpr float cc_ = M_::AT[pp][i]; wino_mad(a, cc_, d[pp][qq]); }
      });
      r[i][qq] = a;
    });
  });
  float* dst = dM + (int64_t)t * C + c;
  const int64_t plane = g.T * C;
  ssp_sfor<A>([&](auto I) {
    constexpr int i = decltype(I)::value;
    ssp_sfor<A>([&](auto J) {
      constexpr int j = decltype(J)::value;
      vec a;
#pragma unroll
      for (int k = 0; k < CV; ++k) a[k] = 0.f;
      ssp_sfor<N>([&](auto Q) {
        constexpr int qq = decltype(Q)::value;
        { constexpr float cc_ = M_::AT[qq][j]; wino_mad(a, cc_, r[i][qq]); }
      });
      if constexpr (NT) __builtin_nontemporal_store(a, reinterpret_cast<vec*>(dst + (int64_t)(i * A + j) * plane));
      else *reinterpret_cast<vec*>(dst + (int64_t)(i * A + j) * plane) = a;
    });
  });
}

template <int N>
__global__ void __launch_bounds__(256) wino_wgrad_finish_kernel(const float* __restrict__ dU, float* dw, int rows, int K) {
  constexpr int A = N + 2;
  using M_ = WinoMat<N>;
  const int64_t gid = (int64_t)blockIdx.x * 256 + threadIdx.x;
  const int k4n = K >> 2;
  if (gid >= (int64_t)rows * k4n) return;
  const int row = (int)(gid / k4n);
  const int k = (int)(gid - (int64_t)row * k4n) * 4;
  const float* src = dU + (int64_t)row * K + k;
  const int64_t plane = (int64_t)rows * K;
  const f32x4 z4 = {0.f, 0.f, 0.f, 0.f};
  f32x4 acc[3][3];
#pragma unroll
  for (int a = 0; a < 3; ++a)
#pragma unroll
    for (int bb = 0; bb < 3; ++bb) acc[a][bb] = z4;
  ssp_sfor<A>([&](auto I) {
    constexpr int i = decltype(I)::value;
    f32x4 u[A];
#pragma unroll
    for (int j = 0; j < A; ++j) u[j] = *reinterpret_cast<const f32x4*>(src + (int64_t)(i * A + j) * plane);
    ssp_sfor<3>([&](auto Bb) {
      constexpr int bb = decltype(Bb)::value;
      f32x4 h = z4;
      ssp_sfor<A>([&](auto J) {
        constexpr int j = decltype(J)::value;
        { constexpr float cc_ = M_::G[j][bb]; wino_mad(h, cc_, u[j]); }
      });
      ssp_sfor<3>([&](auto Aa) {
        constexpr int a = decltype(Aa)::value;
        { constexpr float cc_ = M_::G[i][a]; wino_mad(acc[a][bb], cc_, h); }
      });
    });
  });
  float* dst = dw + ((int64_t)row * 9) * K + k;
#pragma unroll
  for (int a = 0; a < 3; ++a)
#pragma unroll
    for (int bb = 0; bb < 3; ++bb) {
      f32x4* o = reinterpret_cast<f32x4*>(dst + (int64_t)(a * 3 + bb) * K);
      *o = *o + acc[a][bb];
    }
}

static inline bool wino_tile_ok(int tile) { return tile == 2 || tile == 4; }
int64_t ssp_wino_tiles(int B, int H, int W, int tile) { return wino_geom(B, H, W, tile).T; }
int ssp_wino_planes(int tile) { return (tile + 2) * (tile + 2); }
int64_t ssp_wino_stat_groups(int B, int H, int W, int tile) { return (ssp_wino_tiles(B, H, W, tile) + SSP_WINO_TG - 1) / SSP_WINO_TG; }

int ssp_wino_outgrad_launch(const float* dy, int lddy, float* dM, int B, int H, int W, int C, int tile, hipStream_t stream) {
  SSP_CHECK_ARG(wino_tile_ok(tile), "wino_outgrad: tile must be 2 or 4");
  const WinoGeom g = wino_geom(B, H, W, tile);
  const int wv = ssp_option(SSP_OPT_WINO_VARIANT);
  const int cv = (tile == 2 || (wv & 1)) ? 4 : 2;
  SSP_CHECK_ARG(C % 4 == 0 && lddy % 4 == 0 && (((uintptr_t)dy) & 15) == 0 && (((uintptr_t)dM) & 15) == 0,
                "wino_outgrad: channels must be a multiple of 4 and the operands 16-byte aligned");
  SSP_CHECK_ARG(g.T * (C / cv) < (1ll << 31), "wino_outgrad: too many (tile, channel) pairs");
  const int P = ssp_wino_planes(tile);
  SspProfScope prof(SSP_PROF_WINO_WGRAD, stream, 4.0 * C * ((double)B * H * W + (double)P * g.T));
  const int64_t n = g.T * (C / cv);
  const SspFastDiv dc = ssp_fastdiv((unsigned)(C / cv));
  const dim3 grid((unsigned)((n + 255) / 256));
  if (tile == 2 && (wv & 2)) hipLaunchKernelGGL((wino_outgrad_kernel<2, 4, true>), grid, dim3(256), 0, stream, dy, lddy, dM, C, g, dc);
  else if (tile == 2) hipLaunchKernelGGL((wino_outgrad_kernel<2, 4>), grid, dim3(256), 0, stream, dy, lddy, dM, C, g, dc);
  else if (cv == 4 && (wv & 2)) hipLaunchKernelGGL((wino_outgrad_kernel<4, 4, true>), grid, dim3(256), 0, stream, dy, lddy, dM, C, g, dc);
  else if (cv == 4) hipLaunchKernelGGL((wino_outgrad_kernel<4, 4>), grid, dim3(256), 0, stream, dy, lddy, dM, C, g, dc);
  else if (wv & 2) hipLaunchKernelGGL((wino_outgrad_kernel<4, 2, true>), grid, dim3(256), 0, stream, dy, lddy, dM, C, g, dc);
  else hipLaunchKernelGGL((wino_outgrad_kernel<4, 2>), grid, dim3(256), 0, stream, dy, lddy, dM, C, g, dc);
  SSP_CHECK_LAUNCH("wino_outgrad");
  return SSP_OK;
}

int ssp_wino_wgrad_finish_launch(const float* dU, float* dw, int rows, int K, int tile, hipStream_t stream) {
  SSP_CHECK_ARG(wino_tile_ok(tile), "wino_wgrad_finish: tile must be 2 or 4");
  const int64_t n = (int64_t)rows * (K / 4);
  SspProfScope prof(SSP_PROF_WINO_WGRAD, stream, 4.0 * (double)rows * K * (ssp_wino_planes(tile) + 18.0));
  if (tile == 2) hipLaunchKernelGGL(wino_wgrad_finish_kernel<2>, dim3((unsigned)((n + 255) / 256)), dim3(256), 0, stream, dU, dw, rows, K);
  else hipLaunchKernelGGL(wino_wgrad_finish_kernel<4>, dim3((unsigned)((n + 255) / 256)), dim3(256), 0, stream, dU, dw, rows, K);
  SSP_CHECK_LAUNCH("wino_wgrad_finish");
  return SSP_OK;
}

int ssp_wino_input_launch(const float* in, int ldin, float* V, int B, int H, int W, int C, int tile, int prof_kind, hipStream_t stream) {
  SSP_CHECK_ARG(wino_tile_ok(tile), "wino_input: tile must be 2 or 4");
  const WinoGeom g = wino_geom(B, H, W, tile);
  const int wv = ssp_option(SSP_OPT_WINO_VARIANT);
  const int cv = (tile == 2 || (wv & 1)) ? 4 : 2;
  SSP_CHECK_ARG(C % 4 == 0 && ldin % 4 == 0 && (((uintptr_t)in) & 15) == 0 && (((uintptr_t)V) & 15) == 0,
                "wino_input: channels must be a multiple of 4 and the operands 16-byte aligned");
  SSP_CHECK_ARG(g.T * (C / cv) < (1ll << 31), "wino_input: too many (tile, channel) pairs");
  const int P = ssp_wino_planes(tile);
  SspProfScope prof(prof_kind, stream, 4.0 * C * ((double)B * H * W + (double)P * g.T));
  const int64_t n = g.T * (C / cv);
  const SspFastDiv dc = ssp_fastdiv((unsigned)(C / cv));
  const dim3 grid((unsigned)((n + 255) / 256));
  if (tile == 2 && (wv & 2)) hipLaunchKernelGGL((wino_input_kernel<2, 4, true>), grid, dim3(256), 0, stream, in, ldin, V, C, g, dc);
  else if (tile == 2) hipLaunchKernelGGL((wino_input_kernel<2, 4>), grid, dim3(256), 0, stream, in, ldin, V, C, g, dc);
  else if (cv == 4 && (wv & 2)) hipLaunchKernelGGL((wino_input_kernel<4, 4, true>), grid, dim3(256), 0, stream, in, ldin, V, C, g, dc);
  else if (cv == 4) hipLaunchKernelGGL((wino_input_kernel<4, 4>), grid, dim3(256), 0, stream, in, ldin, V, C, g, dc);
  else if (wv & 2) hipLaunchKernelGGL((wino_input_kernel<4, 2, true>), grid, dim3(256), 0, stream, in, ldin, V, C, g, dc);
  else hipLaunchKernelGGL((wino_input_kernel<4, 2>), grid, dim3(256), 0, stream, in, ldin, V, C, g, dc);
  SSP_CHECK_LAUNCH("wino_input");
  return SSP_OK;
}

int ssp_wino_filter_launch(const float* w, float* U, int rows, int K, int tile, hipStream_t stream) {
  SSP_CHECK_ARG(wino_tile_ok(tile), "wino_filter: tile must be 2 or 4");
  SSP_CHECK_ARG(w != nullptr && U != nullptr && rows > 0 && K > 0 && K % 4 == 0 && (((uintptr_t)w) & 15) == 0 &&
                    (((uintptr_t)U) & 15) == 0,
                "wino_filter: [rows][9][K] filters with K % 4 == 0, 16-byte aligned operands");
  SspProfScope prof(SSP_PROF_LAYOUT, stream, 4.0 * (9.0 + ssp_wino_planes(tile)) * (double)rows * K);
  const int64_t n = (int64_t)rows * (K / 4);
  if (tile == 2) hipLaunchKernelGGL(wino_filter_kernel<2>, dim3((unsigned)((n + 255) / 256)), dim3(256), 0, stream, w, U, rows, K);
  else hipLaunchKernelGGL(wino_filter_kernel<4>, dim3((unsigned)((n + 255) / 256)), dim3(256), 0, stream, w, U, rows, K);
  SSP_CHECK_LAUNCH("wino_filter");
  return SSP_OK;
}

int ssp_wino_output_launch(const WinoOutArgs& a, int B, int H, int W, int tile, int prof_kind, hipStream_t stream) {
  SSP_CHECK_ARG(wino_tile_ok(tile), "wino_output: tile must be 2 or 4");
  const WinoGeom g = wino_geom(B, H, W, tile);
  const int P = ssp_wino_planes(tile);
  SspProfScope prof(prof_kind, stream, 4.0 * a.Cout * ((double)B * H * W * (a.accumulate ? 2.0 : 1.0) * (a.bn_partial ? 2.0 : 1.0) + (double)P * g.T));
  const bool wide = a.Cout >= 256 && (ssp_option(SSP_OPT_WINO_VARIANT) & 4);
  const dim3 grid((unsigned)((g.T + SSP_WINO_TG - 1) / SSP_WINO_TG), (unsigned)ssp_cdiv(a.Cout, wide ? 256 : 64));
  if (tile == 2 && wide) hipLaunchKernelGGL((wino_output_kernel<2, 64>), grid, dim3(256), 0, stream, a, g);
  else if (tile == 2) hipLaunchKernelGGL((wino_output_kernel<2, 16>), grid, dim3(256), 0, stream, a, g);
  else if (wide) hipLaunchKernelGGL((wino_output_kernel<4, 64>), grid, dim3(256), 0, stream, a, g);
  else hipLaunchKernelGGL((wino_output_kernel<4, 16>), grid, dim3(256), 0, stream, a, g);
  SSP_CHECK_LAUNCH("wino_output");
  return SSP_OK;
}
```

singleshotpose_amd/csrc/ssp_api.hip:

```cpp
#include <stdarg.h>
#include <mutex>
#include <vector>

#include "../../include/ssp_hip.h"
#include "conv_wino.h"

int ssp_conv_tile_m(int M, int Cin, int Cout, int R, int plan);
int64_t ssp_conv_ws_floats(int M, int Cin, int Cout, int R, int plan);
int ssp_conv_igemm_launch(const float* in, const float* wt, float* out, const float* bias, float* stats, int B, int H,
                          int W, int Cin, int Cout, int ldin, int ldout, int R, int accumulate, float* ws,
                          int64_t ws_floats, int plan, int prof_kind, hipStream_t stream,
                          const float* escale = nullptr, float act_slope = 1.f, const SspBnBwdFuse* bnb = nullptr);
int64_t ssp_wino_ws_floats(int B, int H, int W, int Cin, int Cout, int tile);
int ssp_conv_wgrad_launch(const float* dy, const float* x, float* dw, int B, int H, int W, int Cin, int Cout, int lddy,
                          int ldx, int R, hipStream_t stream);
int64_t ssp_conv_wgrad_wino_ws_floats(int B, int H, int W, int Cin, int Cout, int tile);
int ssp_conv_wgrad_wino_launch(const float* dy, const float* x, float* dw, int B, int H, int W, int Cin, int Cout, int lddy,
                               int ldx, int tile, float* ws, int64_t ws_floats, hipStream_t stream);
int ssp_bn_fwd_finalize_launch(const float* stats, int ntile, int BM, int M, int C, const float* gamma,
                               const float* beta, float* rmean, float* rvar, float momentum, float eps, float* mean,
                               float* invstd, float* scale, float* shift, hipStream_t stream);
int ssp_bn_eval_prepare_launch(int C, const float* gamma, const float* beta, const float* rmean, const float* rvar,
                               float eps, float* mean, float* invstd, float* scale, float* shift, hipStream_t stream);
int ssp_bn_act_fwd_launch(const float* x, int ldx, float* out, int ldo, const float* scale, const float* shift, int C,
                          int B, int H, int W, int pool, float slope, hipStream_t stream);
int ssp_bn_bwd_blocks_impl(void);
int ssp_bn_act_bwd_launch(const float* x, int ldx, const float* g, int ldg, float* dx, int lddx, const float* scale,
                          const float* shift, const float* mean, const float* invstd, int C, int B, int H, int W,
                          int pool, float slope, int training, float* partial, float* dgamma, float* dbeta, float* c1,
                          float* c2, hipStream_t stream);
int ssp_bn_act_bwd_partials_launch(const float* x, int ldx, const float* g, int ldg, float* dx, int lddx,
                                   const float* scale, const float* shift, const float* mean, const float* invstd,
                                   int C, int B, int H, int W, float slope, int training, float* partial,
                                   int npartial, int zero_after, float* dgamma, float* dbeta, float* c1, float* c2,
                                   hipStream_t stream);
int ssp_bn_act_bwd_affine_launch(const float* x, int ldx, const float* g, int ldg, float* dx, int lddx, const float* scale,
                                 const float* shift, const float* mean, const float* invstd, int C, int B, int H, int W,
                                 int pool, float slope, hipStream_t stream);
int ssp_bn_bwd_finalize_launch(float* partial, int npartial, int C, int64_t npix, int training, int zero_after,
                               float* dgamma, float* dbeta, float* c1, float* c2, hipStream_t stream);
int ssp_first_tile_pixels_impl(void);
int ssp_first_groups_impl(int B, int H, int W);
int ssp_first_fwd_stats_launch(const float* x, const float* wt, float* stats, int B, int H, int W, hipStream_t stream);
int ssp_first_fwd_apply_launch(const float* x, const float* wt, const float* scale, const float* shift, float slope,
                               float* out, int ldo, int B, int H, int W, hipStream_t stream);
int ssp_first_conv_raw_launch(const float* x, const float* wt, float* raw, int ldraw, int B, int H, int W,
                              hipStream_t stream);
int ssp_first_bwd_reduce_launch(const float* x, const float* wt, const float* g, int ldg, const float* scale,
                                const float* shift, const float* mean, const float* invstd, float slope, float* partial,
                                int B, int H, int W, hipStream_t stream);
int ssp_first_bwd_wgrad_launch(const float* x, const float* wt, const float* g, int ldg, const float* scale,
                               const float* shift, const float* mean, const float* invstd, const float* c1,
                               const float* c2, float slope, float* dw, float* workspace, int64_t workspace_floats, int B,
                               int H, int W, hipStream_t stream);
int64_t ssp_first_wgrad_workspace_floats_impl(int B, int H, int W);
int ssp_first_bwd_dgrad_launch(const float* x, const float* wt, const float* g, int ldg, const float* scale,
                               const float* shift, const float* mean, const float* invstd, const float* c1,
                               const float* c2, float slope, float* dx, int B, int H, int W, hipStream_t stream);
int ssp_colsum_launch(const float* g, int ldg, int64_t M, int C, float* out, hipStream_t stream);
int ssp_sgd_step_launch(float* p, const float* g, float* m, int64_t n, float lr, float momentum, float dampening,
                        float weight_decay, int nesterov, int first_step, hipStream_t stream);
int ssp_sgd_step_table_launch(float* p, const float* g, float* m, int64_t p_floats, int64_t g_floats, int64_t m_floats,
                              const int64_t* table_dev, const int64_t* table_host, int nseg, const float* hyper, int ntuple,
                              hipStream_t stream);
int ssp_nchw_to_nhwc_launch(const float* src, float* dst, int B, int C, int H, int W, int Cp, int ld, hipStream_t stream);
int ssp_nhwc_to_nchw_launch(const float* src, float* dst, int B, int C, int H, int W, int ld, hipStream_t stream);
int ssp_pose_errors_launch(const double* verts, int N, const double* Rt_gt, const double* Rt_pr, const double* K,
                           int k_per_pose, int n, double* out, hipStream_t stream);
int ssp_pts_diameter_launch(const double* pts, int N, double* out, double* scratch, hipStream_t stream);
int ssp_pose_errors_models_launch(const double* verts, const int* model_off, const int* pose_model, int nM,
                                  const double* Rt_gt, const double* Rt_pr, const double* K, int k_per_pose, int n,
                                  double* out, hipStream_t stream);
int64_t ssp_adds_workspace_doubles_impl(int n, int maxN);
int ssp_adds_errors_launch(const double* verts, const int* model_off, const int* pose_model, int nM, int maxN,
                           const double* Rt_gt, const double* Rt_pr, int n, double* out, double* workspace,
                           int64_t workspace_doubles, hipStream_t stream);
int ssp_resample_u8_launch(const SspResampleDesc* descs, int count, int pass, int epilogue, int max_dst_pixels, hipStream_t stream);
int ssp_distort_u8_launch(const unsigned char* rgb, unsigned char* out, int64_t npix, const unsigned char* lut, int mode, hipStream_t stream);
int ssp_composite_u8_launch(const SspCompositeDesc* descs, int count, int64_t max_bytes, hipStream_t stream);
int ssp_u8hwc_to_nhwc_launch(const unsigned char* src, float* dst, int B, int H, int W, int C, int Cp, int ld,
                             hipStream_t stream);
int ssp_repack_fwd_launch(const float* w, float* out, int Cout, int Cin, int Cinp, int R, hipStream_t stream);
int ssp_unpack_grad_launch(const float* dwp, float* grad, int Cout, int Cin, int Cinp, int R, hipStream_t stream);
int ssp_repack_dgrad_launch(const float* w, float* out, int Cout, int Cin, int Coutp, int R, hipStream_t stream);
int ssp_repack_dgrad_packed_launch(const float* wp, float* out, int Cout, int Cin, int Coutp, int R, hipStream_t stream);
int ssp_reorg_launch(const float* src, int lds_, float* dst, int ldd, int C, int B, int H, int W, int backward,
                     int accumulate, hipStream_t stream);
int ssp_copy_channels_launch(const float* src, int lds_, float* dst, int ldd, int C, int64_t M, int accumulate,
                             hipStream_t stream);
int ssp_maxpool_fwd_launch(const float* x, int ldx, float* out, int ldo, int C, int B, int H, int W, hipStream_t stream);
int ssp_maxpool_bwd_launch(const float* x, int ldx, const float* g, int ldg, float* dx, int lddx, int C, int B, int H,
                           int W, int accumulate, hipStream_t stream);
int ssp_maxpool_s1_fwd_launch(const float* x, int ldx, float* out, int ldo, int C, int B, int H, int W,
                              hipStream_t stream);
int ssp_maxpool_s1_bwd_launch(const float* x, int ldx, const float* g, int ldg, float* dx, int lddx, int C, int B, int H,
                              int W, int accumulate, hipStream_t stream);
int ssp_shortcut_fwd_launch(const float* a, int lda, const float* b, int ldb, float* out, int ldo, int C, int64_t M,
                            float slope, hipStream_t stream);
int ssp_shortcut_bwd_launch(const float* g, int ldg, const float* out, int ldo, float* da, int ldda, int acc_a, float* db,
                            int lddb, int acc_b, int C, int64_t M, float slope, hipStream_t stream);
int ssp_avgpool_fwd_launch(const float* x, int ldx, float* out, int ldo, int C, int B, int H, int W, hipStream_t stream);
int ssp_avgpool_bwd_launch(const float* g, int ldg, float* dx, int lddx, int C, int B, int H, int W, int accumulate,
                           hipStream_t stream);
int ssp_softmax_fwd_launch(const float* x, int ldx, float* y, int ldy, int C, int64_t M, hipStream_t stream);
int ssp_softmax_bwd_launch(const float* y, int ldy, const float* g, int ldg, float* dx, int lddx, int C, int64_t M,
                           int accumulate, hipStream_t stream);
int ssp_region_loss_launch(const float* out, const void* target, int target_is_f64, float* grad, float* partials,
                           float* stats, int nB, int nA, int nC, int nH, int nW, int num_keypoints,
                           float noobject_scale, float object_scale, float coord_scale, float class_scale, float thresh,
                           int conf_on, int multi, const float* anchors, int anchor_step, hipStream_t stream);
int ssp_region_decode_argmax_launch(const float* out, float* boxes, int nB, int nA, int nC, int nH, int nW,
                                    int num_keypoints, int only_objectness, hipStream_t stream);
int ssp_region_decode_all_launch(const float* out, float* rows, int nB, int nA, int nC, int nH, int nW,
                                 int num_keypoints, hipStream_t stream);
int ssp_region_match_multi_launch(const float* out, const float* target, float* rows, int* meta, int nB, int nA, int nC,
                                  int nH, int nW, int num_keypoints, float conf_thresh, int only_objectness, int im_width,
                                  int im_height, hipStream_t stream);
int ssp_pnp_batched_launch(const double* pts3d, const double* pts2d, const double* K, double* Rt, int n, int N,
                           int max_iter, hipStream_t stream);

static thread_local char g_err[512] = "";
void ssp_set_error(const char* fmt, ...) {
  va_list ap;
  va_start(ap, fmt);
  vsnprintf(g_err, sizeof(g_err), fmt, ap);
  va_end(ap);
}

static int g_options[SSP_OPT_COUNT] = {1, 0, 0, 0, 0, 0, 1};
static const char* g_option_names[SSP_OPT_COUNT] = {"igemm_xcd", "igemm_variant", "wgrad_variant", "igemm_plan", "wgrad_split", "wino_variant", "acc_chunk"};
int ssp_option(int which) { return g_options[which]; }

static std::mutex g_kernel_mu;
int ssp_kernel_prepare(const void* kern, int lds_bytes, int threads, SspKernelCache* cache, int* slots, const char* name) {
  int dev = 0;
  if (hipGetDevice(&dev) != hipSuccess || dev < 0 || dev >= SSP_MAX_DEVICES) {
    ssp_set_error("%s: no current HIP device (or device index >= %d)", name, SSP_MAX_DEVICES);
    return SSP_ERR_HIP;
  }
  std::lock_guard<std::mutex> lk(g_kernel_mu);
  if (lds_bytes > cache->configured[dev]) {
    if (hipFuncSetAttribute(kern, hipFuncAttributeMaxDynamicSharedMemorySize, lds_bytes) != hipSuccess) {
      ssp_set_error("%s: cannot reserve %d bytes of LDS", name, lds_bytes);
      return SSP_ERR_HIP;
    }
    int per_cu = 0, ncu = 0;
    if (hipOccupancyMaxActiveBlocksPerMultiprocessor(&per_cu, kern, threads, lds_bytes) != hipSuccess || per_cu < 1)
      per_cu = 2;
    if (hipDeviceGetAttribute(&ncu, hipDeviceAttributeMultiprocessorCount, dev) != hipSuccess || ncu < 1) ncu = 256;
    cache->slots[dev] = per_cu * ncu;
    cache->configured[dev] = lds_bytes;
  }
  if (slots != nullptr) *slots = cache->slots[dev];
  return SSP_OK;
}

namespace {
struct ProfRec {
  int kind;
  hipEvent_t start, stop;
  double work;
};
std::mutex g_prof_mu;
unsigned g_prof_mask = 0;
std::vector<ProfRec> g_recs;
std::vector<std::pair<hipEvent_t, hipEvent_t>> g_free_events;
}

SspProfScope::SspProfScope(int kind, hipStream_t s, double work) : slot(-1), stream(s) {
  if (!((g_prof_mask >> kind) & 1u)) return;
  std::lock_guard<std::mutex> lk(g_prof_mu);
  ProfRec r;
  r.kind = kind;
  r.work = work;
  if (!g_free_events.empty()) {
    r.start = g_free_events.back().first;
    r.stop = g_free_events.back().second;
    g_free_events.pop_back();
  } else {
    if (hipEventCreate(&r.start) != hipSuccess || hipEventCreate(&r.stop) != hipSuccess) return;
  }
  (void)hipEventRecord(r.start, s);
  g_recs.push_back(r);
  slot = (int)g_recs.size() - 1;
}
SspProfScope::~SspProfScope() {
  if (slot < 0) return;
  std::lock_guard<std::mutex> lk(g_prof_mu);
  (void)hipEventRecord(g_recs[slot].stop, stream);
}

extern "C" {

const char* ssp_last_error(void) { return g_err; }
int ssp_abi_version(void) { return 5; }
int ssp_set_option(const char* name, int value) {
  for (int i = 0; i < SSP_OPT_COUNT; ++i)
    if (name != nullptr && strcmp(name, g_option_names[i]) == 0) {
      g_options[i] = value;
      return SSP_OK;
    }
  ssp_set_error("set_option: unknown option '%s'", name ? name : "(null)");
  return SSP_ERR_ARG;
}

int ssp_conv_fwd(const float* in, const float* wt, float* out, const float* bias, float* stats, int B, int H, int W,
                 int Cin, int Cout, int ldin, int ldout, int R, int accumulate, int plan, float* workspace,
                 int64_t workspace_floats, void* stream) {
  return ssp_conv_igemm_launch(in, wt, out, bias, stats, B, H, W, Cin, Cout, ldin, ldout, R, accumulate, workspace,
                               workspace_floats, plan, SSP_PROF_CONV_FWD, (hipStream_t)stream);
}
int ssp_conv_fwd_affine(const float* in, const float* wt, float* out, const float* scale, const float* shift,
                        float slope, int B, int H, int W, int Cin, int Cout, int ldin, int ldout, int R, int plan,
                        float* workspace, int64_t workspace_floats, void* stream) {
  return ssp_conv_igemm_launch(in, wt, out, shift, nullptr, B, H, W, Cin, Cout, ldin, ldout, R, 0, workspace,
                               workspace_floats, plan, SSP_PROF_CONV_FWD, (hipStream_t)stream, scale, slope);
}
int ssp_conv_stats_tile_m(int B, int H, int W, int Cin, int Cout, int R, int plan) {
  return ssp_conv_tile_m(B * H * W, Cin, Cout, R, plan);
}
int ssp_conv_plan_wino_tile(int plan) { return ssp_wino_plan_tile(plan); }
int64_t ssp_conv_wino_tiles(int B, int H, int W, int tile) {
  if (tile != 2 && tile != 4) return 0;
  return ssp_wino_tiles(B, H, W, tile);
}
int ssp_conv_stats_tiles(int B, int H, int W, int Cin, int Cout, int R, int plan) {
  if (ssp_wino_plan_fused(plan)) return ssp_wino_fused_stat_groups(B, H, W, Cout);
  if (const int tile = ssp_wino_plan_tile(plan)) return (int)ssp_wino_stat_groups(B, H, W, tile);
  return ssp_cdiv((int64_t)B * H * W, ssp_conv_tile_m(B * H * W, Cin, Cout, R, plan));
}
int64_t ssp_conv_stats_floats(int B, int H, int W, int Cin, int Cout, int R, int plan) {
  const int64_t nt = ssp_conv_stats_tiles(B, H, W, Cin, Cout, R, plan);
  return nt * Cout * 2 + (ssp_wino_plan_tile(plan) ? nt : 0);
}
int64_t ssp_conv_workspace_floats(int B, int H, int W, int Cin, int Cout, int R, int plan) {
  if (ssp_wino_plan_fused(plan)) return 0;
  if (const int tile = ssp_wino_plan_tile(plan)) return ssp_wino_ws_floats(B, H, W, Cin, Cout, tile);
  return ssp_conv_ws_floats(B * H * W, Cin, Cout, R, plan);
}
int ssp_wino_filter_transform_t(const float* w9, float* U, int rows, int K, int tile, void* stream) {
  return ssp_wino_filter_launch(w9, U, rows, K, tile, (hipStream_t)stream);
}
int ssp_wino_filter_transform(const float* w9, float* U, int rows, int K, void* stream) {
  return ssp_wino_filter_launch(w9, U, rows, K, 2, (hipStream_t)stream);
}

int ssp_conv_dgrad(const float* dy, const float* wt, float* dx, int B, int H, int W, int Cout_dy, int Cin_dx, int lddy,
                   int lddx, int R, int accumulate, int plan, float* workspace, int64_t workspace_floats,
                   void* stream) {
  return ssp_conv_igemm_launch(dy, wt, dx, nullptr, nullptr, B, H, W, Cout_dy, Cin_dx, lddy, lddx, R, accumulate,
                               workspace, workspace_floats, plan, SSP_PROF_CONV_DGRAD, (hipStream_t)stream);
}

int ssp_conv_dgrad_bnbwd(const float* dy, const float* wt, float* dx, int B, int H, int W, int Cout_dy, int Cin_dx,
                         int lddy, int lddx, int R, int plan, float* workspace, int64_t workspace_floats,
                         const float* raw, int ldraw, const float* scale, const float* shift, const float* mean,
                         const float* invstd, float slope, float* partial, int partial_rows, void* stream) {
  SspBnBwdFuse f = {raw, ldraw, scale, shift, mean, invstd, slope, partial, partial_rows};
  if (partial == nullptr) {
    ssp_set_error("conv_dgrad_bnbwd: partial must not be NULL (use ssp_conv_dgrad)");
    return SSP_ERR_ARG;
  }
  return ssp_conv_igemm_launch(dy, wt, dx, nullptr, nullptr, B, H, W, Cout_dy, Cin_dx, lddy, lddx, R, 0, workspace,
                               workspace_floats, plan, SSP_PROF_CONV_DGRAD, (hipStream_t)stream, nullptr, 1.f, &f);
}
int ssp_bn_act_bwd_partials(const float* x, int ldx, const float* g, int ldg, float* dx, int lddx, const float* scale,
                            const float* shift, const float* mean, const float* invstd, int C, int B, int H, int W,
                            float slope, int training, float* partial, int npartial, int zero_after, float* dgamma,
                            float* dbeta, float* c1, float* c2, void* stream) {
  return ssp_bn_act_bwd_partials_launch(x, ldx, g, ldg, dx, lddx, scale, shift, mean, invstd, C, B, H, W, slope, training,
                                        partial, npartial, zero_after, dgamma, dbeta, c1, c2, (hipStream_t)stream);
}

int ssp_bn_bwd_finalize(float* partial, int npartial, int C, int64_t npix, int training, int zero_after, float* dgamma,
                        float* dbeta, float* c1, float* c2, void* stream) {
  return ssp_bn_bwd_finalize_launch(partial, npartial, C, npix, training, zero_after, dgamma, dbeta, c1, c2,
                                    (hipStream_t)stream);
}
int ssp_first_tile_pixels(void) { return ssp_first_tile_pixels_impl(); }
int ssp_first_groups(int B, int H, int W) { return ssp_first_groups_impl(B, H, W); }
int ssp_first_fwd_stats(const float* x, const float* wt, float* stats, int B, int H, int W, void* stream) {
  return ssp_first_fwd_stats_launch(x, wt, stats, B, H, W, (hipStream_t)stream);
}
int ssp_first_fwd_apply(const float* x, const float* wt, const float* scale, const float* shift, float slope, float* out,
                        int ldo, int B, int H, int W, void* stream) {
  return ssp_first_fwd_apply_launch(x, wt, scale, shift, slope, out, ldo, B, H, W, (hipStream_t)stream);
}
int ssp_first_conv_raw(const float* x, const float* wt, float* raw, int ldraw, int B, int H, int W, void* stream) {
  return ssp_first_conv_raw_launch(x, wt, raw, ldraw, B, H, W, (hipStream_t)stream);
}
int ssp_first_bwd_reduce(const float* x, const float* wt, const float* g, int ldg, const float* scale, const float* shift,
                         const float* mean, const float* invstd, float slope, float* partial, int B, int H, int W,
                         void* stream) {
  return ssp_first_bwd_reduce_launch(x, wt, g, ldg, scale, shift, mean, invstd, slope, partial, B, H, W,
                                     (hipStream_t)stream);
}
int ssp_first_bwd_wgrad(const float* x, const float* wt, const float* g, int ldg, const float* scale, const float* shift,
                        const float* mean, const float* invstd, const float* c1, const float* c2, float slope, float* dw,
                        float* workspace, int64_t workspace_floats, int B, int H, int W, void* stream) {
  return ssp_first_bwd_wgrad_launch(x, wt, g, ldg, scale, shift, mean, invstd, c1, c2, slope, dw, workspace,
                                    workspace_floats, B, H, W, (hipStream_t)stream);
}
int64_t ssp_first_wgrad_workspace_floats(int B, int H, int W) { return ssp_first_wgrad_workspace_floats_impl(B, H, W); }
int ssp_first_bwd_dgrad(const float* x, const float* wt, const float* g, int ldg, const float* scale, const float* shift,
                        const float* mean, const float* invstd, const float* c1, const float* c2, float slope, float* dx,
                        int B, int H, int W, void* stream) {
  return ssp_first_bwd_dgrad_launch(x, wt, g, ldg, scale, shift, mean, invstd, c1, c2, slope, dx, B, H, W,
                                    (hipStream_t)stream);
}

int ssp_conv_wgrad(const float* dy, const float* x, float* dw, int B, int H, int W, int Cin, int Cout, int lddy,
                   int ldx, int R, void* stream) {
  return ssp_conv_wgrad_launch(dy, x, dw, B, H, W, Cin, Cout, lddy, ldx, R, (hipStream_t)stream);
}

int ssp_conv_wgrad_route(int B, int H, int W, int Cin, int Cout, int lddy, int ldx, int R) {
  return ssp_wgrad_route(B, H, W, Cin, Cout, lddy, ldx, R, 0, ssp_option(SSP_OPT_WGRAD_VARIANT));
}
int64_t ssp_conv_wgrad_wino_workspace_floats_t(int B, int H, int W, int Cin, int Cout, int tile) {
  return ssp_conv_wgrad_wino_ws_floats(B, H, W, Cin, Cout, tile);
}
int ssp_conv_wgrad_wino_t(const float* dy, const float* x, float* dw, int B, int H, int W, int Cin, int Cout, int lddy,
                          int ldx, int tile, float* workspace, int64_t workspace_floats, void* stream) {
  return ssp_conv_wgrad_wino_launch(dy, x, dw, B, H, W, Cin, Cout, lddy, ldx, tile, workspace, workspace_floats, (hipStream_t)stream);
}
int ssp_wino_input_transform_t(const float* x, int ldx, float* V, int B, int H, int W, int C, int tile, void* stream) {
  return ssp_wino_input_launch(x, ldx, V, B, H, W, C, tile, SSP_PROF_WINO_WGRAD, (hipStream_t)stream);
}
int64_t ssp_conv_wgrad_wino_workspace_floats(int B, int H, int W, int Cin, int Cout) {
  return ssp_conv_wgrad_wino_ws_floats(B, H, W, Cin, Cout, 2);
}
int ssp_conv_wgrad_wino(const float* dy, const float* x, float* dw, int B, int H, int W, int Cin, int Cout, int lddy,
                        int ldx, float* workspace, int64_t workspace_floats, void* stream) {
  return ssp_conv_wgrad_wino_launch(dy, x, dw, B, H, W, Cin, Cout, lddy, ldx, 2, workspace, workspace_floats, (hipStream_t)stream);
}

int ssp_bn_fwd_finalize(const float* stats, int ntile, int tile_m, int M, int C, const float* gamma,
                        const float* beta, float* running_mean, float* running_var, float momentum, float eps,
                        float* mean, float* invstd, float* scale, float* shift, void* stream) {
  return ssp_bn_fwd_finalize_launch(stats, ntile, tile_m, M, C, gamma, beta, running_mean, running_var, momentum, eps,
                                    mean, invstd, scale, shift, (hipStream_t)stream);
}
int ssp_bn_eval_prepare(int C, const float* gamma, const float* beta, const float* running_mean,
                        const float* running_var, float eps, float* mean, float* invstd, float* scale, float* shift,
                        void* stream) {
  return ssp_bn_eval_prepare_launch(C, gamma, beta, running_mean, running_var, eps, mean, invstd, scale, shift,
                                    (hipStream_t)stream);
}
int ssp_bn_act_fwd(const float* x, int ldx, float* out, int ldo, const float* scale, const float* shift, int C, int B,
                   int H, int W, int pool, float slope, void* stream) {
  return ssp_bn_act_fwd_launch(x, ldx, out, ldo, scale, shift, C, B, H, W, pool, slope, (hipStream_t)stream);
}
int ssp_bn_act_bwd(const float* x, int ldx, const float* g, int ldg, float* dx, int lddx, const float* scale,
                   const float* shift, const float* mean, const float* invstd, int C, int B, int H, int W, int pool,
                   float slope, int training, float* partial, float* dgamma, float* dbeta, float* c1, float* c2,
                   void* stream) {
  return ssp_bn_act_bwd_launch(x, ldx, g, ldg, dx, lddx, scale, shift, mean, invstd, C, B, H, W, pool, slope, training,
                               partial, dgamma, dbeta, c1, c2, (hipStream_t)stream);
}
int ssp_bn_act_bwd_affine(const float* x, int ldx, const float* g, int ldg, float* dx, int lddx, const float* scale,
                          const float* shift, const float* mean, const float* invstd, int C, int B, int H, int W, int pool,
                          float slope, void* stream) {
  return ssp_bn_act_bwd_affine_launch(x, ldx, g, ldg, dx, lddx, scale, shift, mean, invstd, C, B, H, W, pool, slope,
                                      (hipStream_t)stream);
}
int ssp_bn_bwd_blocks(void) { return ssp_bn_bwd_blocks_impl(); }
int ssp_colsum(const float* g, int ldg, int64_t M, int C, float* out, void* stream) {
  return ssp_colsum_launch(g, ldg, M, C, out, (hipStream_t)stream);
}
int ssp_sgd_step(float* param, const float* grad, float* momentum_buf, int64_t n, float lr, float momentum,
                 float dampening, float weight_decay, int nesterov, int first_step, void* stream) {
  return ssp_sgd_step_launch(param, grad, momentum_buf, n, lr, momentum, dampening, weight_decay, nesterov, first_step,
                             (hipStream_t)stream);
}
int ssp_sgd_step_table(float* param, const float* grad, float* momentum_buf, int64_t param_floats, int64_t grad_floats,
                       int64_t momentum_floats, const int64_t* table_dev, const int64_t* table_host, int nseg,
                       const float* hyper, int ntuple, void* stream) {
  return ssp_sgd_step_table_launch(param, grad, momentum_buf, param_floats, grad_floats, momentum_floats, table_dev,
                                   table_host, nseg, hyper, ntuple, (hipStream_t)stream);
}

int ssp_nchw_to_nhwc(const float* src, float* dst, int B, int C, int H, int W, int Cpad, int ld, void* stream) {
  return ssp_nchw_to_nhwc_launch(src, dst, B, C, H, W, Cpad, ld, (hipStream_t)stream);
}
int ssp_u8hwc_to_nhwc(const unsigned char* src, float* dst, int B, int H, int W, int C, int Cpad, int ld, void* stream) {
  return ssp_u8hwc_to_nhwc_launch(src, dst, B, H, W, C, Cpad, ld, (hipStream_t)stream);
}
int ssp_resample_u8(const SspResampleDesc* descs_dev, int count, int pass, int epilogue, int max_dst_pixels, void* stream) {
  return ssp_resample_u8_launch(descs_dev, count, pass, epilogue, max_dst_pixels, (hipStream_t)stream);
}
int ssp_composite_u8(const SspCompositeDesc* descs_dev, int count, long long max_bytes, void* stream) {
  return ssp_composite_u8_launch(descs_dev, count, (int64_t)max_bytes, (hipStream_t)stream);
}
int ssp_distort_u8(const unsigned char* rgb, unsigned char* out, int64_t npix, const unsigned char* lut, int mode, void* stream) {
  return ssp_distort_u8_launch(rgb, out, npix, lut, mode, (hipStream_t)stream);
}
int ssp_nhwc_to_nchw(const float* src, float* dst, int B, int C, int H, int W, int ld, void* stream) {
  return ssp_nhwc_to_nchw_launch(src, dst, B, C, H, W, ld, (hipStream_t)stream);
}
int ssp_repack_fwd(const float* w, float* out, int Cout, int Cin, int Cinp, int R, void* stream) {
  return ssp_repack_fwd_launch(w, out, Cout, Cin, Cinp, R, (hipStream_t)stream);
}
int ssp_repack_dgrad_packed(const float* wp, float* out, int Cout, int Cin, int Coutp, int R, void* stream) {
  return ssp_repack_dgrad_packed_launch(wp, out, Cout, Cin, Coutp, R, (hipStream_t)stream);
}
int ssp_repack_dgrad(const float* w, float* out, int Cout, int Cin, int Coutp, int R, void* stream) {
  return ssp_repack_dgrad_launch(w, out, Cout, Cin, Coutp, R, (hipStream_t)stream);
}
int ssp_unpack_grad(const float* dwp, float* grad, int Cout, int Cin, int Cinp, int R, void* stream) {
  return ssp_unpack_grad_launch(dwp, grad, Cout, Cin, Cinp, R, (hipStream_t)stream);
}
int ssp_reorg(const float* src, int lds, float* dst, int ldd, int C, int B, int H, int W, int backward, int accumulate,
              void* stream) {
  return ssp_reorg_launch(src, lds, dst, ldd, C, B, H, W, backward, accumulate, (hipStream_t)stream);
}
int ssp_copy_channels(const float* src, int lds, float* dst, int ldd, int C, int64_t M, int accumulate, void* stream) {
  return ssp_copy_channels_launch(src, lds, dst, ldd, C, M, accumulate, (hipStream_t)stream);
}
// ... 113 lines not shown
```

singleshotpose_amd/engine.py:

```python
import collections
import os
import weakref

import torch

from . import _lib
from .cfg import layer_shapes, resolve_layers

WINO = 9000000
WINO4 = 8000000
WGRAD_FUSED = 12
WINOF = 7000001
IGEMM_CANDS = (12813, 12814, 6414, 6413, 12824, 12834, 306413, 306414, 312813, 312814, 206413, 212814,
               12823, 6423, 6424, 206414, 212813, 406413, 406414, 412813)
IGEMM_LATENCY_CANDS = (6418, 12818, 6428, 12828, 6438)
WINO_GEMM_CANDS = (6413, 6414, 12813, 12814)


def _tune_tag():
    if os.environ.get('SSP_WINOGRAD', '1') == '0':
        return 'r5-direct'
    return 'r6-w%s-c%s-%s-f%s' % (os.environ.get('SSP_WINO_TILES', '2,4'), os.environ.get('SSP_WINO_MIN_CHANNELS', '128'),
                                  os.environ.get('SSP_WINO4_MIN_CHANNELS', '64'),
                                  os.environ.get('SSP_WINO_FUSED', '1') + os.environ.get('SSP_WGRAD_FUSED_PREFER', '') +
                                  os.environ.get('SSP_ONCHIP_PREFER', '') + os.environ.get('SSP_ONCHIP_CREDIT_MS', ''))


def wino_fused(code):
    return 7000000 <= code < 8000000


def wino_tile(code):
    return 2 if (WINO <= code < WINO + 1000000 or wino_fused(code)) else (4 if WINO4 <= code < WINO4 + 1000000 else 0)
BN_EPS = 1e-4
BN_MOMENTUM = 0.1


_WEIGHTS_EPOCH = [0]
_TUNE_CACHE = {}
_TUNE_FAMILY = {}
_HEAD_BUDGET_CACHE = {}
_HEAD_BUDGET_PINNED = {}
_TUNE_VERIFIED = {}
_TUNE_VERIFIED_ALSO = set()
TUNE_REJECTED = []
_TUNE_CACHE_FILE = [None]


def _tune_cache_load():
    path = os.environ.get('SSP_TUNE_CACHE')
    if not path or _TUNE_CACHE_FILE[0] == path:
        return
    _TUNE_CACHE_FILE[0] = path
    if os.path.isfile(path):
        import json
        with open(path) as f:
            for k, v in json.load(f).items():
                if k.startswith('fam|'):
                    _TUNE_FAMILY.setdefault(tuple(json.loads(k[4:])), {int(f_): (int(c), t) for f_, (c, t) in v.items()})
                elif k.startswith('budget|'):
                    _HEAD_BUDGET_PINNED.setdefault(tuple(json.loads(k[7:])), {int(i): int(c) for i, c in v.items()})
                else:
                    _TUNE_CACHE.setdefault(tuple(json.loads(k)), int(v))


def _tune_cache_save():
    path = _TUNE_CACHE_FILE[0]
    if path:
        import json
        tmp = path + '.tmp.%d' % os.getpid()
        with open(tmp, 'w') as f:
            out = {json.dumps(list(k)): v for k, v in _TUNE_CACHE.items()}
            out.update({'fam|' + json.dumps(list(k)): {str(f_): [c, t] for f_, (c, t) in v.items()} for k, v in _TUNE_FAMILY.items()})
            out.update({'budget|' + json.dumps(list(k)): {str(i): c for i, c in v.items()} for k, v in _HEAD_BUDGET_PINNED.items()})
            json.dump(out, f, indent=0, sort_keys=True)
        os.replace(tmp, path)


def _storage_refs(t):
    fn = getattr(torch._C, '_storage_Use_Count', None)
    return fn(t.untyped_storage()._cdata) if fn is not None else None


def _storage_shared(t, refs_alone, params):
    refs = _storage_refs(t)
    if refs is not None and refs_alone is not None:
        return refs != refs_alone
    sp = t.untyped_storage().data_ptr()
    return any(p.grad is not None and p.grad.untyped_storage().data_ptr() == sp for p in params)


_SIDE_STREAMS = {}


def _side_stream(device):
    key = (device.type, device.index if device.index is not None else torch.cuda.current_device())
    st = _SIDE_STREAMS.get(key)
    if st is None:
        st = _SIDE_STREAMS[key] = torch.cuda.Stream(device=device, priority=int(os.environ.get('SSP_SIDE_PRIORITY', '-1')))
    return st


def weights_changed():
    _WEIGHTS_EPOCH[0] += 1


def _is_packed(wt, cinp):
    if wt.dim() == 2:
        return wt.size(1) == cinp and wt.is_contiguous()
    return wt.size(1) == cinp and wt.permute(0, 2, 3, 1).is_contiguous()


def _ptr(t, offset=0):
    return t.data_ptr() + 4 * offset


def _pad4(c):
    return (c + 3) // 4 * 4


def choose_under_budget(table, budget):
    choice = {i: 0 for i in table}
    moved = []
    total = lambda: sum(table[i][choice[i]][3] ** 2 for i in table) ** 0.5
    while total() > budget:
        best, gain = None, 0.0
        for i, rows in table.items():
            k = choice[i]
            for k2 in range(k + 1, len(rows)):
                if rows[k2][3] < rows[k][3]:
                    dt = max((rows[k2][2] or 0.0) - (rows[k][2] or 0.0), 1e-6)
                    g = (rows[k][3] ** 2 - rows[k2][3] ** 2) / dt
                    if g > gain:
                        best, gain = (i, k2), g
                    break
        if best is None:
            break
        moved.append((best[0], table[best[0]][choice[best[0]]][0], table[best[0]][best[1]][0]))
        choice[best[0]] = best[1]
    return choice, moved


_SLOPES = {'leaky': 0.1, 'linear': 1.0, 'relu': 0.0}


class _Act(object):
    __slots__ = ('t', 'off', 'C', 'H', 'W', 'ld', 'flat', 'producer')

    def __init__(self, t, off, C, H, W, ld, flat=False):
        self.t, self.off, self.C, self.H, self.W, self.ld = t, off, C, H, W, ld
        self.flat = flat
        self.producer = None

    @property
    def ptr(self):
        return _ptr(self.t, self.off)


INPUT = -1

OpSchedule = collections.namedtuple('OpSchedule', 'ind kind visited dgrad wgrad bias dgamma dbeta bn_reduce fold_bn')


class _Op(object):
    __slots__ = ('kind', 'ind', 'srcs', 'out', 'slope')

    def __init__(self, kind, ind, srcs, out, slope=None):
        self.kind, self.ind, self.srcs, self.out, self.slope = kind, ind, srcs, out, slope

    @property
    def oind(self):
        return self.ind


class _ConvSpec(object):
    kind = 'conv'
    _raw = None
    _raw_spec = None
    wbuf = gbuf = None
    wino_u = wino_ud = None
    wino_ws = wino_ws_floats = None
    wgrad_wino = 0
    ws_dgrad = 0
    fwd_fams = None
    stats = None
    first_fused = False
    first_partial = first_wpart = None
    bnp = bn_fuse_src = None
    v_live = False
    packed = False
    bn_train = False
    has_raw = False
    fsched = None

    @property
    def oind(self):
        return self.ind + 1 if self.pool else self.ind

    @property
    def raw(self):
        if self._raw is None:
            alloc, n, kw = self._raw_spec
            self._raw = alloc(n, **kw)
        return self._raw


class Plan(object):

    def __init__(self, net, B, H, W, device):
        self.net = net
        self.B, self.H, self.W = B, H, W
        self.device = device
        blocks = net.blocks
        self.shapes = layer_shapes(blocks, W, H)
        nl = len(blocks) - 1
        self.nl = nl

        consumers = [[] for _ in range(nl)]
        for ind, block in enumerate(blocks[1:]):
            t = block['type']
            if t in ('convolutional', 'maxpool', 'reorg', 'avgpool', 'softmax', 'connected'):
                if ind > 0:
                    consumers[ind - 1].append(ind)
            elif t == 'route':
                for l in resolve_layers(block['layers'], ind):
                    consumers[l].append(ind)
            elif t == 'shortcut':
                if ind == 0:
                    raise NotImplementedError("shortcut as the first block (it needs two earlier layers)")
                consumers[resolve_layers(block['from'], ind)[0]].append(ind)
                consumers[ind - 1].append(ind)
            elif t in ('region', 'cost'):
                pass
            else:
                raise NotImplementedError(
                    "block type '%s' is outside the yolo-pose hot path (SURVEY.md section 8); not built" % t)
        self.consumers = consumers
        self.last = max(i for i, b in enumerate(blocks[1:]) if b['type'] not in ('region', 'cost'))

        f32 = dict(dtype=torch.float32, device=device)
        in_c = int(blocks[0].get('channels', 3))
        self.in_c = in_c
        self.in_cp = _pad4(in_c)
        self.x_nhwc = torch.empty(B * H * W * self.in_cp, **f32)
        self.input_act = _Act(self.x_nhwc, 0, in_c, H, W, self.in_cp)
        self.input_act.producer = INPUT
        self._dpack_in = None

        self.convs = {}
        self.fused_pool = set()
        self.acts = [None] * nl
        self.ops = []
        wsz = dsz = 0
        prev = self.input_act
        for ind, block in enumerate(blocks[1:]):
            t = block['type']
            w, h, c = self.shapes[ind]
            zeros_or_empty = torch.empty if _pad4(c) == c else torch.zeros
            if t in ('convolutional', 'connected'):
                if t == 'convolutional':
                    k, s = int(block['size']), int(block['stride'])
                    if s != 1 or k not in (1, 3) or (k == 3 and not int(block['pad'])):
                        raise NotImplementedError("conv size=%d stride=%d pad=%s is outside the yolo-pose hot path" % (k, s, block['pad']))
                    bn = int(block['batch_normalize']) != 0
                    seq = net.models[ind]
                    conv, bnm = seq[0], (seq[1] if bn else None)
                else:
                    if prev.H != 1 or prev.W != 1:
                        raise NotImplementedError("connected block %d on a %d x %d map: nn.Linear needs a (B, C) input - put "
                                                  "an avgpool (or a 1x1 map) in front of it" % (ind, prev.H, prev.W))
                    k, bn, bnm = 1, False, None
                    m = net.models[ind]
                    conv = m[0] if isinstance(m, torch.nn.Sequential) else m
                cs = _ConvSpec()
                cs.ind, cs.k = ind, k
                cs.bn = bn
                act = block['activation']
                if act not in _SLOPES:
                    raise NotImplementedError("activation '%s'" % act)
                cs.slope = _SLOPES[act]
                cs.inp = prev
                cs.first = prev is self.input_act
                cs.cin = in_c if cs.first else prev.C
                cs.cinp = _pad4(cs.cin)
                cs.cout = c
                if conv.weight.shape[1] != cs.cin:
                    raise NotImplementedError("block %d (%s): its parameter takes %d input channels but the map it is given "
                                              "has %d" % (ind, t, conv.weight.shape[1], cs.cin))
                if prev.ld < cs.cinp:
                    raise NotImplementedError("block %d (%s): its %d-channel input map has a row stride of %d floats, narrower "
                                              "than the padded channel count %d" % (ind, t, cs.cin, prev.ld, cs.cinp))
                cs.H, cs.W = prev.H, prev.W
                cs.coutp = _pad4(c)
                cs.conv, cs.bnm = conv, bnm
                nxt = blocks[ind + 2] if ind + 2 < len(blocks) else None
                cs.pool = bool(cs.bn and nxt is not None and nxt['type'] == 'maxpool' and int(nxt['size']) == 2 and
                               int(nxt['stride']) == 2 and consumers[ind] == [ind + 1] and cs.H % 2 == 0 and cs.W % 2 == 0)
                M = B * cs.H * cs.W
                cs.M = M
                alloc = torch.empty if cs.coutp == c else torch.zeros
                cs._raw_spec = (alloc, M * cs.coutp, f32)
                cs.ldraw = cs.coutp
                cs.needs_act = cs.bn or cs.slope != 1.0
                if cs.needs_act:
                    Ho, Wo = (cs.H // 2, cs.W // 2) if cs.pool else (cs.H, cs.W)
                    cs.out = _Act(alloc(B * Ho * Wo * cs.coutp, **f32), 0, c, Ho, Wo, cs.coutp)
                else:
                    cs.out = _Act(cs.raw, 0, c, cs.H, cs.W, cs.coutp)
                cs.out.flat = t == 'connected'
                cs.plan_fwd = cs.plan_dgrad = 0
                cs.vec = torch.zeros(8, cs.coutp, **f32)
                if not cs.bn:
                    cs.vec[1].fill_(1.0)
                    cs.vec[2].fill_(1.0)
                cs.woff, cs.doff = wsz, dsz
                wsz += c * k * k * cs.cinp
                dsz += cs.cinp * k * k * cs.coutp if not cs.first else 0
                self.convs[ind] = cs
                if cs.pool:
                    self.fused_pool.add(ind + 1)
                op = cs
            elif t == 'maxpool':
                if ind in self.fused_pool:
                    continue
                k, s = int(block['size']), int(block['stride'])
                if s != 1 and (k != 2 or s != 2):
                    raise NotImplementedError("maxpool size=%d stride=%d (MaxPoolStride1, darknet.py:8-14) is not instantiated by the pose cfgs; not built" % (k, s))
                if s == 2 and (prev.H % 2 or prev.W % 2):
                    raise NotImplementedError("block %d (maxpool): a standalone 2x2/2 max-pool of a %d x %d map "
                                              "(ssp_maxpool_fwd needs even H and W)" % (ind, prev.W, prev.H))
                op = _Op('maxpool_s1' if s == 1 else 'maxpool', ind, [prev],
                         _Act(torch.empty(B * h * w * prev.ld, **f32), 0, c, h, w, prev.ld))
            elif t == 'reorg':
                if int(block['stride']) != 2:
                    raise NotImplementedError("reorg stride != 2")
# ... 221 lines not shown
                    if best is not None and best[0] != cs.plan_fwd:
                        cs.plan_fwd = best[0]
                        self._size_layer(cs)
            self._fit_workspace()

    def _bn_gains(self):
        bn = [cs for _, cs in sorted(self.convs.items()) if cs.bn]
        if not bn:
            return None
        return torch.stack([cs.vec[2][:cs.cout].abs().max() for cs in bn]).cpu()

    def head_budget_drifted(self):
        if self._hb_gains is None:
            return False
        now = self._bn_gains()
        r = (now / self._hb_gains.clamp_min(1e-30)).clamp_min(1e-30)
        return bool(((r > 2.0) | (r < 0.5)).any())

    def _sync_codes(self, stage):
        fn = getattr(self.net, '_plan_sync', None)
        if fn is None:
            return
        order = sorted(self.convs)
        if stage == 0:
            mine = [self.convs[i].plan_fwd for i in order]
        else:
            mine = [self.convs[i].plan_dgrad for i in order] + [self.convs[i].wgrad_wino for i in order]
        head = [self.B, self.H, self.W, stage, len(order)]
        got = fn(head + mine)
        ok = got[:5] == head and len(got) == len(head) + len(mine)
        if ok:
            wino_on = os.environ.get('SSP_WINOGRAD', '1') != '0'
            tiles = tuple(int(t) for t in os.environ.get('SSP_WINO_TILES', '2,4').split(',') if t)
            fused_on = os.environ.get('SSP_WINO_FUSED', '1') != '0'
            for k, v in enumerate(got[5:]):
                if v == mine[k] or v == 0:
                    continue
                wg = stage == 1 and k >= len(order)
                t = (2 if v == WGRAD_FUSED else v) if wg else wino_tile(v)
                if t and (not wino_on or t not in tiles or ((v == WGRAD_FUSED if wg else wino_fused(v)) and not fused_on)):
                    ok = False
        all_ok = getattr(fn, 'all_ok', None)
        if all_ok is not None:
            ok = all_ok(ok)
        vals = got[5:] if ok else [0] * len(mine)
        for k, i in enumerate(order):
            cs = self.convs[i]
            if stage == 0:
                if vals[k] != cs.plan_fwd:
                    cs.plan_fwd = vals[k]
                    self._size_layer(cs)
            else:
                cs.plan_dgrad = vals[k]
                w = vals[len(order) + k]
                if w != cs.wgrad_wino:
                    cs.wgrad_wino = w
                    if w:
                        cs.wino_ws_floats = _lib.query('ssp_conv_wgrad_wino_workspace_floats_t', self.B, cs.H, cs.W, cs.cinp, cs.cout, w)
                    cs.wino_ws = None
        if stage == 0:
            self._fit_workspace()

    def _fit_workspace(self):
        need = max([1] + [cs.ws_fwd for cs in self.convs.values()] + [cs.ws_dgrad for cs in self.convs.values()])
        if need > self.ws_floats:
            torch.cuda.current_stream().synchronize()
            self.ws_floats = need
            self.ws = torch.empty(need, dtype=torch.float32, device=self.device)
            self._graph = None

    def _forward_tensors(self):
        ts = [self.x_nhwc, self.ws, self.bn_partial] + [a.t for a in self.acts if a is not None]
        for cs in self.convs.values():
            ts += [cs._raw, cs.vec, cs.stats, cs.first_partial]
        return ts

    @staticmethod
    def _distinct_bytes(ts):
        seen, total = set(), 0
        for t in ts:
            if t is not None and t.data_ptr() not in seen:
                seen.add(t.data_ptr())
                total += t.numel() * t.element_size()
        return total

    def footprint(self):
        pending = sum(cs._raw_spec[1] * 4 for cs in self.convs.values() if cs._raw is None and not cs.first_fused)
        return pending + self._distinct_bytes(self._forward_tensors())

    def nbytes_now(self):
        ts = self._forward_tensors() + [self._dpack] + [g.t for g in self.grads.values()]
        for cs in self.convs.values():
            ts += [cs.wbuf, cs.gbuf, cs.wino_ws, cs.first_wpart, cs.bnp[0] if cs.bnp is not None else None]
            ts += list((cs.wino_u or {}).values()) + list((cs.wino_ud or {}).values())
        return self._distinct_bytes(ts)

    def _wbuf(self, cs):
        if cs.wbuf is None:
            cs.wbuf = torch.empty(cs.cout * cs.k * cs.k * cs.cinp, dtype=torch.float32, device=self.device)
        return cs.wbuf

    def _wino_u(self, cs, tile):
        if cs.wino_u is None:
            cs.wino_u = {}
        if tile not in cs.wino_u:
            cs.wino_u[tile] = torch.empty((tile + 2) ** 2 * cs.cout * cs.cinp, dtype=torch.float32, device=self.device)
        return cs.wino_u[tile]

    def _wino_ud(self, cs, tile):
        if cs.wino_ud is None:
            cs.wino_ud = {}
        if tile not in cs.wino_ud:
            cs.wino_ud[tile] = torch.empty((tile + 2) ** 2 * cs.cin * cs.coutp, dtype=torch.float32, device=self.device)
        return cs.wino_ud[tile]

    def _wino_ws(self, cs):
        if cs.wino_ws is None:
            n = cs.wino_ws_floats
            if wino_tile(cs.plan_fwd) and not wino_fused(cs.plan_fwd):
                n = max(n, _lib.query('ssp_conv_workspace_floats', self.B, cs.H, cs.W, cs.cinp, cs.cout, cs.k, cs.plan_fwd))
            cs.wino_ws = torch.empty(n, dtype=torch.float32, device=self.device)
        return cs.wino_ws

    def _gbuf(self, cs):
        if cs.gbuf is None:
            cs.gbuf = torch.empty(cs.cout * cs.k * cs.k * cs.cinp, dtype=torch.float32, device=self.device)
        return cs.gbuf

    def _prepare_backward(self, tune=True):
        if self._dpack is None:
            self._dpack = torch.empty(self._dpack_floats, dtype=torch.float32, device=self.device)
        if self._dgrad_tuned or (not tune and self._dgrad_fallback):
            return
        self._dgrad_tuned = tune
        self._dgrad_fallback = True
        if self._tune and tune:
            self._autotune('dgrad')
            self._tune_wgrad()
        elif self._tune:
            wino_on = os.environ.get('SSP_WINOGRAD', '1') != '0'
            for cs in self.convs.values():
                key = self._dgrad_key(cs)
                code = _TUNE_CACHE.get(key, 0)
                cs.plan_dgrad = code if _TUNE_VERIFIED.get(key) == code and (not wino_tile(code) or wino_on) else 0
                cs.wgrad_wino = 0
        if tune:
            self._sync_codes(1)
        for cs in self.convs.values():
            cs.ws_dgrad = 0 if cs.first else _lib.query('ssp_conv_workspace_floats', self.B, cs.H, cs.W, cs.coutp,
                                                        cs.cin, cs.k, cs.plan_dgrad)
        self._plan_bn_fusion()
        self._fit_workspace()

    def _wgrad_key(self, cs):
        return ('wgrad', self.B, cs.H, cs.W, cs.cinp, cs.cout, cs.ldraw, cs.inp.ld, _tune_tag())

    def _tune_wgrad(self):
        call = _lib.call
        st = torch.cuda.current_stream().cuda_stream
        wino_on = os.environ.get('SSP_WINOGRAD', '1') != '0'
        verify = os.environ.get('SSP_TUNE_VERIFY', '1') != '0'
        tiles = tuple(int(t) for t in os.environ.get('SSP_WINO_TILES', '2,4').split(',') if t)
        gen = torch.Generator(device=self.device)
        gen.manual_seed(4321)
        n_known = len(_TUNE_CACHE)
        for cs in self.convs.values():
            cs.wgrad_wino = 0
            cmin = min(cs.cin, cs.cout)
            if not (wino_on and cs.k == 3 and not cs.first and cs.cinp == cs.cin and cs.coutp == cs.cout and
                    cs.cin % 16 == 0 and cs.cout % 16 == 0):
                continue
            ts_ok = [t for t in tiles if cmin >= 64 and cmin >= int(os.environ.get('SSP_WINO_MIN_CHANNELS', '128') if t == 2 else
                                                                    os.environ.get('SSP_WINO4_MIN_CHANNELS', '64')) and
                     self.B * ((cs.H + t - 1) // t) * ((cs.W + t - 1) // t) >= 16]
            if (2 in tiles and os.environ.get('SSP_WINO_FUSED', '1') != '0' and cs.cin % 32 == 0 and cs.cout % 32 == 0 and
                    (self.B * cs.H * cs.W + cs.W + 1) * max(cs.inp.ld, cs.ldraw) * 4 < (1 << 31)):
                ts_ok.append(WGRAD_FUSED)
            if not ts_ok:
                continue
            key = self._wgrad_key(cs)
            wsn = {t: _lib.query('ssp_conv_wgrad_wino_workspace_floats_t', self.B, cs.H, cs.W, cs.cinp, cs.cout, t) for t in ts_ok}
            cached = _TUNE_CACHE.get(key)
            if cached is not None and (cached == 0 or (cached in ts_ok and (not verify or _TUNE_VERIFIED.get(key) == cached))):
                cs.wgrad_wino = cached
            else:
                ws = torch.empty(max(wsn.values()), dtype=torch.float32, device=self.device)
                dw = [torch.zeros(cs.cout * 9 * cs.cinp, dtype=torch.float32, device=self.device) for _ in range(2)]
                a = cs.inp
                a.t.view(-1, a.ld)[:, a.off % a.ld:a.off % a.ld + cs.cinp].uniform_(-1.0, 1.0, generator=gen)
                cs.raw.view(-1, cs.ldraw)[:, :cs.cout].uniform_(-1.0, 1.0, generator=gen)

                def direct(out, cs=cs):
                    call('ssp_conv_wgrad', cs.raw.data_ptr(), cs.inp.ptr, out.data_ptr(), self.B, cs.H, cs.W, cs.cinp, cs.cout,
                         cs.ldraw, cs.inp.ld, cs.k, st)

                def wino(out, t, cs=cs, ws=ws):
                    call('ssp_conv_wgrad_wino_t', cs.raw.data_ptr(), cs.inp.ptr, out.data_ptr(), self.B, cs.H, cs.W, cs.cinp,
                         cs.cout, cs.ldraw, cs.inp.ld, t, ws.data_ptr(), ws.numel(), st)

                def timed(fn):
                    fn(torch.empty_like(dw[0]))
                    best = None
                    for _ in range(3):
                        e0, e1 = torch.cuda.Event(enable_timing=True), torch.cuda.Event(enable_timing=True)
                        e0.record()
                        fn(torch.empty_like(dw[0]))
                        e1.record()
                        e1.synchronize()
                        t = e0.elapsed_time(e1)
                        best = t if best is None else min(best, t)
                    return best

                use, t_best = 0, None
                try:
                    t_best = timed(direct)
                    dw[0].zero_()
                    direct(dw[0])
                    den = float(dw[0].abs().max())
                except _lib.SspError:
                    t_best, den = None, 1.0
                for t in ts_ok:
                    if t_best is None:
                        break
                    try:
                        tt = timed(lambda out, t=t: wino(out, t))
                        if t == WGRAD_FUSED:
                            if tt >= float(os.environ.get('SSP_ONCHIP_CREDIT_MS', '0.25')):
                                tt *= float(os.environ.get('SSP_WGRAD_FUSED_PREFER', '0.8'))
                        if not tt < 0.985 * t_best:
                            continue
                        dw[1].zero_()
                        wino(dw[1], t)
                        err = float((dw[0] - dw[1]).abs().max())
                        ok = err <= 3e-5 * max(den, 1e-30)
                    except _lib.SspError:
                        continue
                    if not ok:
                        TUNE_REJECTED.append((key, 'wgrad_wino%d' % t))
                        import warnings
                        warnings.warn("singleshotpose_amd: verify-after-tune refused the Winograd F(%dx%d) filter gradient "
                                      "for %s" % (t, t, key))
                        continue
                    use, t_best = t, tt
                _TUNE_CACHE[key] = use
                _TUNE_VERIFIED[key] = use
                cs.wgrad_wino = use
                del ws, dw
            if cs.wgrad_wino:
                cs.wino_ws_floats = wsn[cs.wgrad_wino]
        torch.cuda.synchronize()
        if len(_TUNE_CACHE) != n_known:
            _tune_cache_save()
        torch.cuda.empty_cache()

    def _dgrad_key(self, cs):
        return ('dgrad', self.B, cs.H, cs.W, cs.coutp, cs.cin, cs.k, cs.ldraw, cs.inp.ld, _tune_tag())

    def _plan_bn_fusion(self):
        on = os.environ.get('SSP_BN_FUSE', '1') != '0'
        for cs in self.convs.values():
            cs.bn_fuse_src = None
            cs.bnp = None
        if not on:
            return
        for cs in self.convs.values():
            if cs.first:
                continue
            src = cs.inp.producer
            scs = self.convs.get(src)
            if (scs is None or scs.pool or not scs.bn or not scs.needs_act or scs.out is not cs.inp or
                    self.consumers[src] != [cs.ind] or scs.coutp != scs.cout or cs.cin != scs.cout or
                    cs.inp.ld != scs.ldraw or cs.inp.off != 0 or cs.cin % 4):
                continue
            ntile = _lib.query('ssp_conv_stats_tiles', self.B, cs.H, cs.W, cs.coutp, cs.cin, cs.k, cs.plan_dgrad)
            rows = min(ntile, 1024)
            cs.bn_fuse_src = scs
            scs.bnp = (torch.zeros(rows * scs.cout * 2, dtype=torch.float32, device=self.device), rows, ntile > rows)

    def _repack_dgrad(self, cs, stream):
        src = cs.conv.weight.detach()
        if not cs.packed:
            with torch.cuda.stream(stream):
                src = src.contiguous()
                src.record_stream(stream)
        _lib.call('ssp_repack_dgrad_packed' if cs.packed else 'ssp_repack_dgrad', src.data_ptr(),
                  _ptr(self._dpack, cs.doff), cs.cout, cs.cin, cs.coutp, cs.k, stream.cuda_stream)
        tile = wino_tile(cs.plan_dgrad)
        if tile:
            _lib.call('ssp_wino_filter_transform_t', _ptr(self._dpack, cs.doff), self._wino_ud(cs, tile).data_ptr(), cs.cin,
                      cs.coutp, tile, stream.cuda_stream)

    def _autotune(self, which):
        B = self.B
        call = _lib.call
        st = torch.cuda.current_stream().cuda_stream
        f32 = dict(dtype=torch.float32, device=self.device)
        _tune_cache_load()
        n_known = len(_TUNE_CACHE)
        cands = IGEMM_CANDS
        lat = IGEMM_LATENCY_CANDS
        elig = [cs for cs in self.convs.values() if cs.cinp % 16 == 0]
        if not elig:
            return
        gemm_cands = WINO_GEMM_CANDS
        wino_on = os.environ.get('SSP_WINOGRAD', '1') != '0'
        wino_min = int(os.environ.get('SSP_WINO_MIN_CHANNELS', '128'))
        wino_tiles = tuple(int(t) for t in os.environ.get('SSP_WINO_TILES', '2,4').split(',') if t)

        def wino_bases(cs, which):
            if not (wino_on and cs.k == 3 and not cs.first and cs.cinp == cs.cin and cs.coutp == cs.cout and
                    cs.cin % 16 == 0 and cs.cout % 16 == 0):
                return ()
            bases = []
            if 2 in wino_tiles and min(cs.cin, cs.cout) >= wino_min:
                bases.append(WINO)
            if 4 in wino_tiles and min(cs.cin, cs.cout) >= int(os.environ.get('SSP_WINO4_MIN_CHANNELS', '64')):
                bases.append(WINO4)
            return tuple(bases)

        fused_on = wino_on and os.environ.get('SSP_WINO_FUSED', '1') != '0' and 2 in wino_tiles

        def fused_ok(cs, which):
            return (fused_on and cs.k == 3 and not cs.first and cs.cinp == cs.cin and cs.coutp == cs.cout and
                    cs.cin % 32 == 0 and cs.cout % 32 == 0 and B * cs.H * cs.W * max(cs.inp.ld, cs.ldraw) * 4 < (1 << 31))

        def wino_codes(cs, which, small=False):
            codes = []
            for base in wino_bases(cs, which):
                codes += [base + c for c in gemm_cands]
                if small:
                    codes += [base + 6418, base + 12818]
            if fused_ok(cs, which):
                codes.append(WINOF)
            return tuple(codes)
        def ws_need(cs):
            mc = cs.M * max(cs.coutp, cs.cinp)
            need = 9 * mc if mc <= (1 << 21) else (4 * mc if mc <= (1 << 25) else 1)
            need = max(need, _lib.query('ssp_conv_workspace_floats', B, cs.H, cs.W, cs.cinp, cs.cout, cs.k, 0))
            if not cs.first:
                need = max(need, _lib.query('ssp_conv_workspace_floats', B, cs.H, cs.W, cs.coutp, cs.cin, cs.k, 0))
            for base in wino_bases(cs, 'fwd') + wino_bases(cs, 'dgrad'):
                need = max(need, _lib.query('ssp_conv_workspace_floats', B, cs.H, cs.W, cs.cinp, cs.cout, cs.k, base + 6413))
                need = max(need, _lib.query('ssp_conv_workspace_floats', B, cs.H, cs.W, cs.coutp, cs.cin, cs.k, base + 6413))
            return need
        max_ws = max(ws_need(cs) for cs in elig)
        ws = torch.empty(max_ws, **f32)
        stats = torch.empty(max(((cs.M + 15) // 16 + 16) * (cs.cout * 2 + 1) for cs in elig), **f32) if which == 'fwd' else None
        gscratch = torch.zeros(max(cs.M * max(cs.inp.ld, cs.ldraw) for cs in elig), **f32) if which == 'dgrad' else None
        verify = os.environ.get('SSP_TUNE_VERIFY', '1') != '0'
        gen = torch.Generator(device=self.device)
        gen.manual_seed(1234)

        def best_of(launch, mn, key, extra=(), direct=None):
            keep = True
            if key in _TUNE_CACHE:
                if not wino_tile(_TUNE_CACHE[key]) or _TUNE_CACHE[key] in extra:
                    return _TUNE_CACHE[key]
                keep = False
            best, best_t = 0, None
            fams = {}
            deep = tuple(bm * 100 + ks * 10 + sl for bm in (64, 128) for ks in (4, 5, 6, 8, 9) for sl in (3, 4, 8)) \
                if mn <= (1 << 21) else ()
            for code in (tuple(direct) if direct is not None else cands + (lat if mn <= (1 << 23) else ()) + deep) + tuple(extra):
                if not wino_tile(code) and ((code // 10) % 10 > 1 or code >= 100000) and mn > (1 << 25):
                    continue
                try:
                    launch(code)
                    ts = []
                    for _ in range(2):
                        e0, e1 = torch.cuda.Event(enable_timing=True), torch.cuda.Event(enable_timing=True)
                        e0.record()
                        launch(code)
                        e1.record()
                        e1.synchronize()
                        ts.append(e0.elapsed_time(e1))
                except _lib.SspError:
                    continue
                t = min(ts)
                if wino_fused(code) and key[0] == 'dgrad':
                    if t >= float(os.environ.get('SSP_ONCHIP_CREDIT_MS', '0.25')):
                        t *= float(os.environ.get('SSP_ONCHIP_PREFER', '0.85'))
                if best_t is None or t < best_t * 0.985:
                    best, best_t = code, t
                f_ = wino_tile(code)
                if f_ not in fams or t < fams[f_][1] * 0.985:
                    fams[f_] = (code, t)
            if keep:
                _TUNE_CACHE[key] = best
                _TUNE_FAMILY[key] = fams
            return best

        def admitted(code, key, launch, out_of, operands, bn_of=None, prep=None, primary=True):
            if code == 0 or not verify or _TUNE_VERIFIED.get(key) == code or (key, code) in _TUNE_VERIFIED_ALSO:
                return code
            for t in operands:
                (t[0].view(-1, t[1])[:, t[2]:t[2] + t[3]] if isinstance(t, tuple) else t).uniform_(-1.0, 1.0, generator=gen)
            if prep is not None:
                prep()
            bar = 3e-5 if wino_tile(code) else 1e-5
            res = []
            for c in (0, code):
                launch(c)
                r = [out_of().clone()]
                if bn_of is not None:
                    r += bn_of(c)
                res.append(r)
            ok = True
            for a, b in zip(res[0], res[1]):
                den = float(a.abs().max())
                err = float((a - b).abs().max())
                if not (err <= bar * max(den, 1e-30)):
                    ok = False
            if ok:
                if primary:
                    _TUNE_VERIFIED[key] = code
                else:
                    _TUNE_VERIFIED_ALSO.add((key, code))
                return code
            TUNE_REJECTED.append((key, code))
            if primary:
                _TUNE_CACHE[key] = 0
            import warnings
            warnings.warn("singleshotpose_amd: verify-after-tune refused plan %d for launch %s (result differs from the "
                          "default plan's); the default plan runs" % (code, key))
            return 0

        for cs in elig:
            if which == 'fwd' and (cs.cout > 64 or fused_ok(cs, which)):
                wop = cs.conv.weight if cs.cinp == cs.cin else self._wbuf(cs)
                key = ('fwd', B, cs.H, cs.W, cs.cinp, cs.cout, cs.k, cs.inp.ld, cs.ldraw, bool(cs.bn), _tune_tag())

                wc = wino_codes(cs, which, cs.M * cs.coutp <= (1 << 23))

                def prep_f(tile, cs=cs, wop=wop):
                    call('ssp_wino_filter_transform_t', wop.data_ptr(), self._wino_u(cs, tile).data_ptr(), cs.cout, cs.cinp,
                         tile, st)

                def launch(code, cs=cs, wop=wop):
                    wt = self._wino_u(cs, wino_tile(code)) if wino_tile(code) else wop
                    call('ssp_conv_fwd', cs.inp.ptr, wt.data_ptr(), cs.raw.data_ptr(), None,
                         stats.data_ptr() if cs.bn else None, B, cs.H, cs.W, cs.cinp, cs.cout, cs.inp.ld, cs.ldraw,
                         cs.k, 0, code, ws.data_ptr(), max_ws, st)

# ... 233 lines not shown
                     bn.weight.data_ptr(), bn.bias.data_ptr(), bn.running_mean.data_ptr(),
                     bn.running_var.data_ptr(), self.bn_momentum, BN_EPS, v[0].data_ptr(), v[1].data_ptr(),
                     v[2].data_ptr(), v[3].data_ptr(), st)
            call('ssp_first_fwd_apply', cs.inp.ptr, wptr, v[2].data_ptr(), v[3].data_ptr(), cs.slope,
                 cs.out.ptr, cs.out.ld, B, cs.H, cs.W, st)
            cs.first_live = bn_train
            return
        if (not bn_train and not keep and (cs.bn or not training) and cs.needs_act and not cs.pool and
                cs.coutp == cs.cout):
            call('ssp_conv_fwd_affine', cs.inp.ptr, wptr, cs.out.ptr, v[2].data_ptr() if cs.bn else None,
                 v[3].data_ptr() if cs.bn else bias, cs.slope, B, cs.H, cs.W, cs.cinp, cs.cout, cs.inp.ld,
                 cs.out.ld, cs.k, cs.plan_fwd, self.ws.data_ptr(), self.ws_floats, st)
            return
        ws_t = self.ws
        cs.v_live = False
        share_v = os.environ.get('SSP_WINO_SHARE_V', '1') != '0'
        cs.has_raw = True
        want_v = keep and cs.fsched.wgrad
        if (want_v and wino_tile(cs.plan_fwd) and not wino_fused(cs.plan_fwd) and
                cs.wgrad_wino == wino_tile(cs.plan_fwd) and share_v):
            ws_t = self._wino_ws(cs)
            cs.v_live = True
        elif (want_v and cs.wgrad_wino and share_v and self.side_stream is not None and
                os.environ.get('SSP_WINO_EARLY_V', '0') == '1'):
            wws = self._wino_ws(cs)
            ready = torch.cuda.current_stream().record_event()
            self.side_stream.wait_event(ready)
            call('ssp_wino_input_transform_t', cs.inp.ptr, cs.inp.ld, wws.data_ptr(), B, cs.H, cs.W, cs.cinp,
                 cs.wgrad_wino, self.side_stream.cuda_stream)
            cs.v_live = True
        call('ssp_conv_fwd', cs.inp.ptr, wptr, cs.raw.data_ptr(), bias,
             cs.stats.data_ptr() if use_stats else None, B, cs.H, cs.W, cs.cinp, cs.cout, cs.inp.ld, cs.ldraw,
             cs.k, 0, cs.plan_fwd, ws_t.data_ptr(), ws_t.numel(), st)
        if bn_train:
            bn = cs.bnm
            call('ssp_bn_fwd_finalize', cs.stats.data_ptr(), cs.ntile, cs.tile_m, cs.M, cs.cout,
                 bn.weight.data_ptr(), bn.bias.data_ptr(), bn.running_mean.data_ptr(),
                 bn.running_var.data_ptr(), self.bn_momentum, BN_EPS, v[0].data_ptr(), v[1].data_ptr(),
                 v[2].data_ptr(), v[3].data_ptr(), st)
        if cs.needs_act:
            call('ssp_bn_act_fwd', cs.raw.data_ptr(), cs.ldraw, cs.out.ptr, cs.out.ld, v[2].data_ptr(),
                 v[3].data_ptr(), cs.coutp, B, cs.H, cs.W, 1 if cs.pool else 0, cs.slope, st)

    def _graph_tensors(self):
        ts = []
        for cs in self.convs.values():
            ts.append(cs.conv.weight)
            if cs.conv.bias is not None:
                ts.append(cs.conv.bias)
            if cs.bn:
                ts += [cs.bnm.weight, cs.bnm.bias, cs.bnm.running_mean, cs.bnm.running_var]
        return ts

    def forward_graph(self, x):
        if self._graph_failed:
            return self.forward(x, False)
        key = (x.dtype,) + tuple((t.data_ptr(), tuple(t.stride())) for t in self._graph_tensors())
        if self._graph is None or self._graph_key != key:
            try:
                self._x_static = torch.empty_like(x)
                self._x_static.copy_(x)
                self.forward(self._x_static, False, inline_repack=True)
                torch.cuda.synchronize(self.device)
                g = torch.cuda.CUDAGraph()
                with torch.cuda.graph(g):
                    y = self.forward(self._x_static, False, inline_repack=True)
                self._graph, self._y_static, self._graph_key = g, y, key
            except Exception as e:
                import warnings
                warnings.warn("hipGraph capture of the inference chain failed (%s); using eager launches" % (e,))
                self._graph, self._graph_failed = None, True
                torch.cuda.synchronize(self.device)
                return self.forward(x, False)
        self._x_static.copy_(x)
        self._graph.replay()
        self.consumed = True
        return self._y_static.clone()

    def backward_schedule(self, trainable_ids=None, want_input=False, bn_training=None):
        T = None if trainable_ids is None else frozenset(trainable_ids)

        def has(p):
            return p is not None and (T is None or id(p) in T)

        def bn_mode(cs):
            if not cs.bn:
                return False
            if bn_training is None:
                return bool(cs.bnm.training)
            if isinstance(bn_training, dict):
                return bool(bn_training[cs.ind])
            return bool(bn_training)

        def srcs_of(op):
            return [op.inp] if op.kind == 'conv' else op.srcs

        rel = {INPUT: bool(want_input)}
        own = {}
        for op in self.ops:
            mine = False
            if op.kind == 'conv':
                own[op.ind] = (has(op.conv.weight), has(op.conv.bias), bool(op.bn) and has(op.bnm.weight),
                               bool(op.bn) and has(op.bnm.bias))
                mine = any(own[op.ind])
            rel[op.oind] = mine or any(rel[a.producer] for a in srcs_of(op))

        def bn_reduce(cs):
            return bool(cs.bn) and (bn_mode(cs) or own[cs.ind][2] or own[cs.ind][3])

        reach = set([self.last])
        out = [None] * len(self.ops)
        for i in range(len(self.ops) - 1, -1, -1):
            op = self.ops[i]
            srcs = srcs_of(op)
            if not (op.oind in reach and rel[op.oind]):
                out[i] = OpSchedule(op.ind, op.kind, False, (False,) * len(srcs), False, False, False, False, False, False)
                continue
            dgrad = tuple(rel[a.producer] for a in srcs)
            for a, d in zip(srcs, dgrad):
                if d:
                    reach.add(a.producer)
            if op.kind != 'conv':
                out[i] = OpSchedule(op.ind, op.kind, True, dgrad, False, False, False, False, False, False)
                continue
            w, b, dg, db = own[op.ind]
            fold = bool(dgrad[0] and op.bn_fuse_src is not None and bn_reduce(op.bn_fuse_src))
            out[i] = OpSchedule(op.ind, 'conv', True, dgrad, w, b, dg, db, bn_reduce(op), fold)
        return out

    def _schedule(self, trainable, want_input, modes=None):
        if modes is None:
            modes = {cs.ind: bool(cs.bn and cs.bnm.training) for cs in self.convs.values()}
        own = None if trainable is None else tuple(
            tuple(p is not None and id(p) in trainable for p in (
                cs.conv.weight, cs.conv.bias, cs.bnm.weight if cs.bn else None, cs.bnm.bias if cs.bn else None))
            for cs in self.convs.values())
        key = (own, bool(want_input), tuple(sorted(modes.items())), tuple(
            None if cs.bn_fuse_src is None else cs.bn_fuse_src.ind for cs in self.convs.values()))
        sched = self._schedules.get(key)
        if sched is None:
            if len(self._schedules) >= 32:
                self._schedules.clear()
            sched = self._schedules[key] = self.backward_schedule(trainable, want_input, modes)
        return sched

    def _grad_buf(self, ind, like):
        g = self.grads.get(ind)
        if g is None:
            g = _Act(torch.empty(self.B * like.H * like.W * like.ld, dtype=torch.float32, device=self.device), 0,
                     like.C, like.H, like.W, like.ld)
            self.grads[ind] = g
        return g

    def _dgrad(self, cs, src, dy_ptr, dy_ld, written, fused_stats, st, fold=True):
        call = _lib.call
        B = self.B
        gin = self._grad_buf(src, cs.inp)
        scs = cs.bn_fuse_src
        dwt = (self._wino_ud(cs, wino_tile(cs.plan_dgrad)).data_ptr() if wino_tile(cs.plan_dgrad)
               else _ptr(self._dpack, cs.doff))
        if scs is not None and fold and src not in written:
            sv = scs.vec
            call('ssp_conv_dgrad_bnbwd', dy_ptr, dwt, gin.ptr, B, cs.H, cs.W,
                 cs.coutp, cs.cin, dy_ld, gin.ld, cs.k, cs.plan_dgrad, self.ws.data_ptr(), self.ws_floats,
                 scs.raw.data_ptr(), scs.ldraw, sv[2].data_ptr(), sv[3].data_ptr(), sv[0].data_ptr(),
                 sv[1].data_ptr(), scs.slope, scs.bnp[0].data_ptr(), scs.bnp[1], st)
            fused_stats.add(src)
        else:
            call('ssp_conv_dgrad', dy_ptr, dwt, gin.ptr, B, cs.H, cs.W, cs.coutp,
                 cs.cin, dy_ld, gin.ld, cs.k, 1 if src in written else 0, cs.plan_dgrad, self.ws.data_ptr(),
                 self.ws_floats, st)
        written.add(src)

    def backward(self, grad_out, want_input=False, want_params=True):
        if want_params is True:
            trainable = None
        elif want_params is False:
            trainable = frozenset()
        else:
            trainable = frozenset(want_params) & frozenset(self.grad_layout)
            if len(trainable) == len(self.grad_layout):
                trainable = None
        want_params = trainable is None or len(trainable) > 0
        if not (want_input or want_params):
            raise ValueError("Plan.backward: neither the input nor the parameter gradients are wanted")
        if self.consumed:
            raise RuntimeError("Darknet backward called twice on the same forward: the HIP path rewrites the saved "
                               "conv outputs in place (no retain_graph support)")
        self.consumed = True
        B = self.B
        st = torch.cuda.current_stream().cuda_stream
        call = _lib.call
        o = self.out_act
        if tuple(grad_out.shape) != ((B, o.C) if self.out_flat else (B, o.C, o.H, o.W)):
            raise ValueError("Darknet backward: gradient of shape %s for an output of shape %s" % (
                tuple(grad_out.shape), (B, o.C) if self.out_flat else (B, o.C, o.H, o.W)))
        g_last = self._grad_buf(self.last, o)
        call('ssp_nchw_to_nhwc', grad_out.data_ptr(), g_last.ptr, B, o.C, o.H, o.W, o.C, o.ld, st)
        if self.side_stream is None:
            self.side_stream = _side_stream(self.device)
        sched = self._schedule(trainable, want_input, {cs.ind: cs.bn_train for cs in self.convs.values()})
        for op, s in zip(self.ops, sched):
            if s.visited and op.kind == 'conv' and not (op.has_raw or op.first_live):
                raise RuntimeError("Darknet backward: block %d was run without gradient bookkeeping by the last forward "
                                   "(it was frozen then, or the forward ran in inference form) - its raw conv output "
                                   "does not exist" % op.ind)
        if not want_params:
            return self._backward_body(None, want_input, sched)
        ent = self.net._flat_grads.get(self.device)
        flat = None
        if ent is not None and ent[0].numel() == self.grad_total and not _storage_shared(ent[0], ent[1], self.net._params()):
            flat = ent[0]
        if flat is None:
            flat = torch.empty(self.grad_total, dtype=torch.float32, device=self.device)
            self.net._flat_grads[self.device] = (flat, _storage_refs(flat))
        flat.record_stream(self.side_stream)
        self.last_flat_grad = flat
        return self._backward_body(flat, want_input, sched)

    def _backward_body(self, flat, want_input, sched):
        B = self.B
        st = torch.cuda.current_stream().cuda_stream
        call = _lib.call
        written = set()
        fused_stats = set()
        written.add(self.last)
        if flat is not None:
            flat.zero_()
            for op, s in zip(self.ops, sched):
                if s.wgrad and not op.packed and not op.first_live:
                    self._gbuf(op).zero_()
        main = torch.cuda.current_stream()
        side = main if self.serial_backward else self.side_stream
        if self.dgrad_ready is not None:
            main.wait_event(self.dgrad_ready)
        else:
            self._prepare_backward(tune=False)
            by_ind = {s.ind: s for s in sched if s.kind == 'conv'}
            for ind in sorted(self.convs.keys(), reverse=True):
                cs = self.convs[ind]
                if not cs.first and by_ind[ind].dgrad[0]:
                    self._repack_dgrad(cs, main)
        out_grads = {}
        tail_sched = side is not main and os.environ.get('SSP_TAIL_SCHED', '1') != '0'
        if self.reducer is not None and flat is not None:
            self.reducer.begin(flat)

        def gview(prm, channels_last=False):
            off, n, shape = self.grad_layout[id(prm)]
            if channels_last:
                return torch.as_strided(flat, shape, prm.stride(), off)
            return flat[off:off + n].view(shape)

        def grad_in(a):
            gin = self._grad_buf(a.producer, a)
            acc = 1 if a.producer in written else 0
            written.add(a.producer)
            return gin, acc

        def grad_scratch(a):
            return self._grad_buf(a.producer, a), 0

        for op, s in zip(reversed(self.ops), reversed(sched)):
            if not s.visited or op.oind not in written:
                if op.kind == 'conv' and flat is not None and self.reducer is not None:
                    with torch.cuda.stream(side):
                        self.reducer.layer_done(flat, op.grad_lo, op.grad_hi)
                continue
            g = self.grads[op.oind]
            kind = op.kind
            if kind == 'conv':
                self._conv_bwd(op, s, g, flat, gview, out_grads, written, fused_stats, main, side, tail_sched)
            elif kind == 'shortcut':
                a, b = op.srcs
                ga, acc_a = grad_in(a) if s.dgrad[0] else grad_scratch(a)
                gb, acc_b = (ga, acc_a) if b is a else (grad_in(b) if s.dgrad[1] else grad_scratch(b))
                out = op.out
                call('ssp_shortcut_bwd', g.ptr, g.ld, out.ptr, out.ld, ga.ptr, ga.ld, acc_a, gb.ptr, gb.ld, acc_b,
                     _pad4(out.C), B * out.H * out.W, op.slope, st)
            elif kind in ('alias', 'concat'):
                off = 0
                for a, d in zip(op.srcs, s.dgrad):
                    if d:
                        gin, acc = grad_in(a)
                        call('ssp_copy_channels', _ptr(g.t, g.off + off), g.ld, gin.ptr, gin.ld, a.C, B * a.H * a.W, acc, st)
                    off += a.C
            elif s.dgrad[0]:
                src = op.srcs[0]
                gin, acc = grad_in(src)
                if kind in ('maxpool', 'maxpool_s1'):
                    call('ssp_maxpool_bwd' if kind == 'maxpool' else 'ssp_maxpool_s1_bwd', src.ptr, src.ld, g.ptr, g.ld,
                         gin.ptr, gin.ld, _pad4(src.C), B, src.H, src.W, acc, st)
                elif kind == 'reorg':
                    call('ssp_reorg', g.ptr, g.ld, gin.ptr, gin.ld, src.C, B, src.H, src.W, 1, acc, st)
                elif kind == 'avgpool':
                    call('ssp_avgpool_bwd', g.ptr, g.ld, gin.ptr, gin.ld, _pad4(src.C), B, src.H, src.W, acc, st)
                else:
                    call('ssp_softmax_bwd', op.out.ptr, op.out.ld, g.ptr, g.ld, gin.ptr, gin.ld, src.C, B * src.H * src.W,
                         acc, st)
        dx = None
        if want_input:
            o = self.input_act
            dx = torch.empty(B, self.in_c, self.H, self.W, dtype=torch.float32, device=self.device)
            if INPUT in written:
                call('ssp_nhwc_to_nchw', self.grads[INPUT].ptr, dx.data_ptr(), B, self.in_c, o.H, o.W, o.ld, st)
            else:
                dx.zero_()
        if flat is not None:
            main.wait_stream(side)
        return out_grads, dx

    def _conv_bwd(self, cs, s, g, flat, gview, out_grads, written, fused_stats, main, side, tail_sched):
        B = self.B
        call = _lib.call
        st, st2 = main.cuda_stream, side.cuda_stream
        training = cs.bn_train
        v = cs.vec
        params = flat is not None

        def hand_out(prm):
            gv = gview(prm)
            out_grads[id(prm)] = gv
            return gv

        if cs.first_live:
            dg_ptr = hand_out(cs.bnm.weight).data_ptr() if s.dgamma else v[6].data_ptr()
            db_ptr = hand_out(cs.bnm.bias).data_ptr() if s.dbeta else v[7].data_ptr()
            wptr = self._wbuf(cs).data_ptr()
            call('ssp_first_bwd_reduce', cs.inp.ptr, wptr, g.ptr, g.ld, v[2].data_ptr(), v[3].data_ptr(),
                 v[0].data_ptr(), v[1].data_ptr(), cs.slope, cs.first_partial.data_ptr(), B, cs.H, cs.W, st)
            call('ssp_bn_bwd_finalize', cs.first_partial.data_ptr(), cs.first_groups, cs.cout, cs.M,
                 1 if training else 0, 0, dg_ptr, db_ptr, v[4].data_ptr(), v[5].data_ptr(), st)
            if s.dgrad[0]:
                self._first_input_dgrad(cs, g, written, st)
            if not params:
                return
            fst = st if tail_sched else st2
            if s.wgrad:
                if not tail_sched:
                    side.wait_stream(main)
                gw = gview(cs.conv.weight, False)
                if cs.first_wpart is None:
                    cs.first_wpart = torch.empty(_lib.query('ssp_first_wgrad_workspace_floats', B, cs.H, cs.W),
                                                 dtype=torch.float32, device=self.device)
                call('ssp_first_bwd_wgrad', cs.inp.ptr, wptr, g.ptr, g.ld, v[2].data_ptr(), v[3].data_ptr(),
                     v[0].data_ptr(), v[1].data_ptr(), v[4].data_ptr(), v[5].data_ptr(), cs.slope,
                     self._gbuf(cs).data_ptr(), cs.first_wpart.data_ptr(), cs.first_wpart.numel(), B, cs.H, cs.W, fst)
                call('ssp_unpack_grad', self._gbuf(cs).data_ptr(), gw.data_ptr(), cs.cout, cs.cin, cs.cinp, cs.k, fst)
                out_grads[id(cs.conv.weight)] = gw
            if self.reducer is not None:
                if tail_sched or not s.wgrad:
                    side.wait_stream(main)
                with torch.cuda.stream(side):
                    self.reducer.layer_done(flat, cs.grad_lo, cs.grad_hi)
            return
        if cs.needs_act:
            if cs.bn and not s.bn_reduce:
                call('ssp_bn_act_bwd_affine', cs.raw.data_ptr(), cs.ldraw, g.ptr, g.ld, cs.raw.data_ptr(), cs.ldraw,
                     v[2].data_ptr(), v[3].data_ptr(), v[0].data_ptr(), v[1].data_ptr(), cs.coutp, B, cs.H, cs.W,
                     1 if cs.pool else 0, cs.slope, st)
            else:
                direct = cs.bn and cs.coutp == cs.cout
                dg_ptr = hand_out(cs.bnm.weight).data_ptr() if (direct and s.dgamma) else v[6].data_ptr()
                db_ptr = hand_out(cs.bnm.bias).data_ptr() if (direct and s.dbeta) else v[7].data_ptr()
                partial = self.bn_partial.data_ptr()
                if cs.ind in fused_stats:
                    ptile, rows, folded = cs.bnp
                    call('ssp_bn_act_bwd_partials', cs.raw.data_ptr(), cs.ldraw, g.ptr, g.ld, cs.raw.data_ptr(),
                         cs.ldraw, v[2].data_ptr(), v[3].data_ptr(), v[0].data_ptr(), v[1].data_ptr(), cs.coutp, B,
                         cs.H, cs.W, cs.slope, 1 if training else 0, ptile.data_ptr(), rows, 1 if folded else 0,
                         dg_ptr, db_ptr, v[4].data_ptr(), v[5].data_ptr(), st)
                else:
                    call('ssp_bn_act_bwd', cs.raw.data_ptr(), cs.ldraw, g.ptr, g.ld, cs.raw.data_ptr(), cs.ldraw,
                         v[2].data_ptr(), v[3].data_ptr(), v[0].data_ptr(), v[1].data_ptr(), cs.coutp, B, cs.H, cs.W,
                         1 if cs.pool else 0, cs.slope, 1 if training else 0, partial,
                         dg_ptr, db_ptr, v[4].data_ptr(), v[5].data_ptr(), st)
                if cs.bn and not direct:
                    if s.dgamma:
                        hand_out(cs.bnm.weight).copy_(v[6][:cs.cout])
                    if s.dbeta:
                        hand_out(cs.bnm.bias).copy_(v[7][:cs.cout])
            dy_ptr, dy_ld = cs.raw.data_ptr(), cs.ldraw
        else:
            dy_ptr, dy_ld = g.ptr, g.ld
        if s.bias:
            db = hand_out(cs.conv.bias)
            call('ssp_colsum', dy_ptr, dy_ld, cs.M, cs.cout, db.data_ptr(), st)
        src = None if cs.first else cs.inp.producer
        owner = None if src is None else (self.convs.get(src - 1) if src in self.fused_pool else self.convs.get(src))
        defer = params and tail_sched and owner is not None and owner.first_live and s.dgrad[0]
        if defer:
            self._dgrad(cs, src, dy_ptr, dy_ld, written, fused_stats, st, s.fold_bn)
        if params:
            side.wait_stream(main)
        if s.wgrad:
            gw = gview(cs.conv.weight, cs.packed)
            if cs.packed and cs.wgrad_wino:
                wws = self._wino_ws(cs)
                call('ssp_conv_wgrad_wino_t', dy_ptr, None if cs.v_live else cs.inp.ptr, gw.data_ptr(),
                     B, cs.H, cs.W, cs.cinp, cs.cout, dy_ld, cs.inp.ld, cs.wgrad_wino, wws.data_ptr(), wws.numel(), st2)
                cs.v_live = False
            elif cs.packed:
                call('ssp_conv_wgrad', dy_ptr, cs.inp.ptr, gw.data_ptr(), B, cs.H, cs.W, cs.cinp, cs.cout, dy_ld,
                     cs.inp.ld, cs.k, st2)
            else:
                call('ssp_conv_wgrad', dy_ptr, cs.inp.ptr, self._gbuf(cs).data_ptr(), B, cs.H, cs.W, cs.cinp,
                     cs.cout, dy_ld, cs.inp.ld, cs.k, st2)
                call('ssp_unpack_grad', self._gbuf(cs).data_ptr(), gw.data_ptr(), cs.cout, cs.cin, cs.cinp, cs.k, st2)
            out_grads[id(cs.conv.weight)] = gw
        if params and self.reducer is not None:
            with torch.cuda.stream(side):
                self.reducer.layer_done(flat, cs.grad_lo, cs.grad_hi)
        if s.dgrad[0] and not defer:
            if cs.first:
                self._input_dgrad(cs, dy_ptr, dy_ld, written, st)
            else:
                self._dgrad(cs, src, dy_ptr, dy_ld, written, fused_stats, st, s.fold_bn)

    def _input_gbuf(self, written):
        gin = self._grad_buf(INPUT, self.input_act)
        acc = 1 if INPUT in written else 0
        written.add(INPUT)
        return gin, acc

    def _input_dgrad(self, cs, dy_ptr, dy_ld, written, st):
        call = _lib.call
        if self._dpack_in is None:
            self._dpack_in = torch.zeros(self.in_cp * cs.k * cs.k * cs.coutp, dtype=torch.float32, device=self.device)
        src = cs.conv.weight.detach()
        if not cs.packed:
            src = src.contiguous()
        call('ssp_repack_dgrad_packed' if cs.packed else 'ssp_repack_dgrad', src.data_ptr(), self._dpack_in.data_ptr(),
             cs.cout, cs.cin, cs.coutp, cs.k, st)
        gin, acc = self._input_gbuf(written)
        call('ssp_conv_dgrad', dy_ptr, self._dpack_in.data_ptr(), gin.ptr, self.B, cs.H, cs.W, cs.coutp, self.in_cp,
             dy_ld, gin.ld, cs.k, acc, 0, None, 0, st)

    def _first_input_dgrad(self, cs, g, written, st):
        gin, acc = self._input_gbuf(written)
        if acc:
            raise NotImplementedError("the network input feeds the fused first block and another block: its gradient "
                                      "would need an accumulating ssp_first_bwd_dgrad")
        v = cs.vec
        _lib.call('ssp_first_bwd_dgrad', cs.inp.ptr, self._wbuf(cs).data_ptr(), g.ptr, g.ld, v[2].data_ptr(),
                  v[3].data_ptr(), v[0].data_ptr(), v[1].data_ptr(), v[4].data_ptr(), v[5].data_ptr(), cs.slope, gin.ptr,
                  self.B, cs.H, cs.W, st)


def _trainable(params, needs):
    return frozenset(id(p) for p, n in zip(params, needs) if n)


class _DarknetFn(torch.autograd.Function):

    @staticmethod
    def forward(ctx, plan, training, x, *params):
        ctx.plan = plan
        ctx.params = params
        need = ctx.needs_input_grad
        y = plan.forward(x, training, need_grad=True, trainable=_trainable(params, need[3:]), want_input=need[2])
        ctx.generation = plan.generation
        return y

    @staticmethod
    def backward(ctx, grad_out):
        plan = ctx.plan if ctx.plan is not None else ctx.plan_ref()
        if plan is None:
            raise RuntimeError("Darknet backward called twice on the same forward, and the plan of that input shape has "
                               "left the plan cache since (another resolution took its memory): run the forward again")
        if plan.generation != ctx.generation:
            raise RuntimeError("Darknet backward after a newer forward on the same input shape: the plan's saved "
                               "activations were overwritten")
        want_x = ctx.needs_input_grad[2]
        want_p = _trainable(ctx.params, ctx.needs_input_grad[3:])
        grads, dx = plan.backward(grad_out.contiguous(), want_input=want_x, want_params=want_p if (want_p or want_x) else True)
        ctx.plan_ref = weakref.ref(plan)
        ctx.plan = None
        res = [None, None, dx]
        for p in ctx.params:
            res.append(grads.get(id(p)))
        return tuple(res)


class _DarknetEvalFn(torch.autograd.Function):

    @staticmethod
    def forward(ctx, plan, x, *params):
        ctx.plan = plan
        ctx.params = params
        ctx.x = x
        ctx.xver = x._version
        return plan.forward(x, False)

    @staticmethod
    def backward(ctx, grad_out):
        plan = ctx.plan
        if ctx.x._version != ctx.xver:
            raise RuntimeError("Darknet (eval mode) backward: the input tensor was modified in place after the forward")
        want_x = ctx.needs_input_grad[1]
        want_p = _trainable(ctx.params, ctx.needs_input_grad[2:])
        if not (want_p or want_x):
            want_p = _trainable(ctx.params, [True] * len(ctx.params))
        plan.forward(ctx.x, False, need_grad=True, trainable=want_p, want_input=want_x)
        grads, dx = plan.backward(grad_out.contiguous(), want_input=want_x, want_params=want_p)
        res = [None, dx]
        for p in ctx.params:
            res.append(grads.get(id(p)))
        return tuple(res)
```

Before: 2547 images/s.

## Share Winograd output-gradient transform between dgrad and wgrad via adjoint data gradient

Adds an adjoint Winograd data-gradient path that reuses the transformed output gradient dM, which the Winograd wgrad already needs, instead of separately input-transforming dy for dgrad. The filter transform gets a flipped variant, and the output stage gains an adjoint form that pulls in neighbouring-tile contributions at tile borders. dM is computed once per layer on the main stream and handed to both dgrad and wgrad, so one tile transform pass over dy and its workspace traffic go away. In exchange, the output kernel must read extra neighbour-tile planes, and wgrad on the side stream now depends on dM written on the main stream, which adds an ordering risk.

```diff
diff --git a/include/ssp_hip.h b/include/ssp_hip.h
--- a/include/ssp_hip.h
+++ b/include/ssp_hip.h
@@ -34,6 +34,18 @@
                          int lddy, int lddx, int R, int plan, float* workspace, int64_t workspace_floats,
                          const float* raw, int ldraw, const float* scale, const float* shift, const float* mean,
                          const float* invstd, float slope, float* partial, int partial_rows, void* stream);
+
+int ssp_wino_outgrad_transform_t(const float* dy, int lddy, float* dM, int B, int H, int W, int C, int tile, void* stream);
+int ssp_wino_filter_transform_adj_t(const float* w9d, float* Ut, int rows, int K, int tile, void* stream);
+int64_t ssp_conv_dgrad_adj_workspace_floats(int B, int H, int W, int Cout_dy, int Cin_dx, int plan, int own_dm);
+int ssp_conv_dgrad_adj(const float* dy, const float* wt, float* dx, int B, int H, int W, int Cout_dy, int Cin_dx, int lddy,
+                       int lddx, int R, int accumulate, int plan, float* workspace, int64_t workspace_floats,
+                       const float* dM, void* stream);
+int ssp_conv_dgrad_adj_bnbwd(const float* dy, const float* wt, float* dx, int B, int H, int W, int Cout_dy, int Cin_dx,
+                             int lddy, int lddx, int R, int plan, float* workspace, int64_t workspace_floats,
+                             const float* raw, int ldraw, const float* scale, const float* shift, const float* mean,
+                             const float* invstd, float slope, float* partial, int partial_rows, const float* dM,
+                             void* stream);
 
 int ssp_conv_wgrad(const float* dy, const float* x, float* dw, int B, int H, int W, int Cin, int Cout, int lddy,
                    int ldx, int R, void* stream);
diff --git a/singleshotpose_amd/_lib.py b/singleshotpose_amd/_lib.py
--- a/singleshotpose_amd/_lib.py
+++ b/singleshotpose_amd/_lib.py
@@ -32,6 +32,11 @@
     "ssp_wino_filter_transform_t": [P, P, I, I, I, P],
     "ssp_conv_dgrad": [P, P, P, I, I, I, I, I, I, I, I, I, I, P, L, P],
     "ssp_conv_dgrad_bnbwd": [P, P, P, I, I, I, I, I, I, I, I, I, P, L, P, I, P, P, P, P, F, P, I, P],
+    "ssp_wino_outgrad_transform_t": [P, I, P, I, I, I, I, I, P],
+    "ssp_wino_filter_transform_adj_t": [P, P, I, I, I, P],
+    "ssp_conv_dgrad_adj_workspace_floats": [I, I, I, I, I, I, I],
+    "ssp_conv_dgrad_adj": [P, P, P, I, I, I, I, I, I, I, I, I, I, P, L, P, P],
+    "ssp_conv_dgrad_adj_bnbwd": [P, P, P, I, I, I, I, I, I, I, I, I, P, L, P, I, P, P, P, P, F, P, I, P, P],
     "ssp_bn_act_bwd_partials": [P, I, P, I, P, I, P, P, P, P, I, I, I, I, F, I, P, I, I, P, P, P, P, P],
     "ssp_conv_wgrad": [P, P, P, I, I, I, I, I, I, I, I, P],
     "ssp_conv_wgrad_route": [I, I, I, I, I, I, I, I],
@@ -96,7 +101,7 @@
     "ssp_prof_collect": [P, P, P],
 }
 
-_RET64 = ('ssp_conv_workspace_floats', 'ssp_conv_wgrad_wino_workspace_floats', 'ssp_conv_wgrad_wino_workspace_floats_t',
+_RET64 = ('ssp_conv_workspace_floats', 'ssp_conv_dgrad_adj_workspace_floats', 'ssp_conv_wgrad_wino_workspace_floats', 'ssp_conv_wgrad_wino_workspace_floats_t',
           'ssp_conv_stats_floats', 'ssp_conv_wino_tiles', 'ssp_first_wgrad_workspace_floats', 'ssp_adds_workspace_doubles')
 
 PROF_KINDS = ("conv_fwd", "conv_dgrad", "conv_wgrad", "bn_act", "layout", "region", "optim", "first_block_fwd",
diff --git a/singleshotpose_amd/csrc/conv_igemm.hip b/singleshotpose_amd/csrc/conv_igemm.hip
--- a/singleshotpose_amd/csrc/conv_igemm.hip
+++ b/singleshotpose_amd/csrc/conv_igemm.hip
@@ -440,9 +440,12 @@
 int64_t ssp_wino_ws_floats(int B, int H, int W, int Cin, int Cout, int tile) {
   return ssp_wino_planes(tile) * ssp_wino_tiles(B, H, W, tile) * ((int64_t)Cin + Cout);
 }
+int64_t ssp_wino_adj_ws_floats(int B, int H, int W, int Cout_dy, int Cin_dx, int tile, bool own_dm) {
+  return ssp_wino_planes(tile) * ssp_wino_tiles(B, H, W, tile) * ((int64_t)Cin_dx + (own_dm ? Cout_dy : 0));
+}
 
 static int wino_launch(ConvArgs& a, int B, int H, int W, float* ws, int64_t ws_floats, int plan, int prof_kind,
-                       hipStream_t stream) {
+                       hipStream_t stream, bool adj = false, const float* dM = nullptr) {
   const int bm = (plan / 100) % 1000, slots = plan % 10, tile = ssp_wino_plan_tile(plan), P = ssp_wino_planes(tile);
   SSP_CHECK_ARG(a.R == 3 && a.Cin % 16 == 0 && a.Cout >= 64 && a.Cout % 4 == 0 && a.ldout % 4 == 0 && (((uintptr_t)a.out) & 15) == 0,
                 "conv (Winograd plan): needs a 3x3 filter, Cin %% 16 == 0, Cout >= 64 and %% 4 == 0, an aligned output");
@@ -450,16 +453,27 @@
                     (plan / 100000) % 10 == 0, "conv: bad Winograd plan code %d", plan);
   const int64_t T = ssp_wino_tiles(B, H, W, tile);
   SSP_CHECK_ARG(T < (1ll << 31) && P * T * (int64_t)a.Cin < (1ll << 40), "conv (Winograd plan): too many tiles");
-  SSP_CHECK_ARG(ws != nullptr && ws_floats >= ssp_wino_ws_floats(B, H, W, a.Cin, a.Cout, tile) && (((uintptr_t)ws) & 15) == 0,
-                "conv (Winograd plan): needs a workspace of %lld floats (ssp_conv_workspace_floats)",
-                (long long)ssp_wino_ws_floats(B, H, W, a.Cin, a.Cout, tile));
+  const int64_t need = adj ? ssp_wino_adj_ws_floats(B, H, W, a.Cin, a.Cout, tile, dM == nullptr)
+                           : ssp_wino_ws_floats(B, H, W, a.Cin, a.Cout, tile);
+  SSP_CHECK_ARG(ws != nullptr && ws_floats >= need && (((uintptr_t)ws) & 15) == 0,
+                "conv (Winograd plan): needs a workspace of %lld floats (ssp_conv_workspace_floats)", (long long)need);
+  SSP_CHECK_ARG((((uintptr_t)dM) & 15) == 0, "conv (Winograd plan): dM must be 16-byte aligned");
   SSP_CHECK_ARG((int64_t)(128 + 2) * a.Cin * 4 + (int64_t)a.Cin * 4 < (1ll << 31), "conv (Winograd plan): Cin too large");
   if (a.bn_partial != nullptr) SSP_CHECK_ARG(a.bn_ld % 4 == 0, "conv (Winograd plan): bn_ld must be a multiple of 4");
   SspProfScope prof(prof_kind, stream, 2.0 * (double)a.M * a.Cout * 9.0 * a.Cin);
-  float* V = ws;
+  const float* V = ws;
   float* Mw = ws + P * T * a.Cin;
   const int wkind = prof_kind == SSP_PROF_CONV_DGRAD ? SSP_PROF_WINO_DGRAD : SSP_PROF_WINO_FWD;
-  if (int rc = ssp_wino_input_launch(a.in, a.ldin, V, B, H, W, a.Cin, tile, wkind, stream)) return rc;
+  if (adj) {
+    Mw = ws;
+    V = dM;
+    if (dM == nullptr) {
+      SSP_CHECK_ARG(a.in != nullptr, "conv (adjoint data gradient): dy must be given when dM is NULL");
+      float* own = ws + P * T * a.Cout;
+      if (int rc = ssp_wino_outgrad_launch(a.in, a.ldin, own, B, H, W, a.Cin, tile, stream, wkind)) return rc;
+      V = own;
+    }
+  } else if (int rc = ssp_wino_input_launch(a.in, a.ldin, ws, B, H, W, a.Cin, tile, wkind, stream)) return rc;
   ConvArgs g = a;
   g.in = V; g.wt = a.wt; g.out = Mw; g.bias = nullptr; g.escale = nullptr; g.act_slope = 1.f; g.stats = nullptr;
   g.H = 1; g.W = (int)T; g.ldin = a.Cin; g.ldout = a.Cout; g.R = 1; g.M = (int)T; g.accumulate = 0;
@@ -473,13 +487,13 @@
   o.Cout = a.Cout; o.ldout = a.ldout; o.accumulate = a.accumulate;
   o.bn_raw = a.bn_raw; o.bn_scale = a.bn_scale; o.bn_shift = a.bn_shift; o.bn_mean = a.bn_mean; o.bn_invstd = a.bn_invstd;
   o.bn_partial = a.bn_partial; o.bn_nslot = a.bn_nslot; o.bn_ld = a.bn_ld; o.bn_slope = a.bn_slope;
-  return ssp_wino_output_launch(o, B, H, W, tile, wkind, stream);
+  return ssp_wino_output_launch(o, B, H, W, tile, wkind, stream, adj);
 }
 
 int ssp_conv_igemm_launch(const float* in, const float* wt, float* out, const float* bias, float* stats, int B, int H,
                           int W, int Cin, int Cout, int ldin, int ldout, int R, int accumulate, float* ws,
                           int64_t ws_floats, int plan, int prof_kind, hipStream_t stream, const float* escale,
-                          float act_slope, const SspBnBwdFuse* bnb) {
+                          float act_slope, const SspBnBwdFuse* bnb, bool adj, const float* dM) {
   SSP_CHECK_ARG(R == 1 || R == 3, "conv: only 1x1 and 3x3 filters are supported (got %d)", R);
   SSP_CHECK_ARG(Cin % 4 == 0 && Cin > 0, "conv: Cin must be a positive multiple of 4 (got %d)", Cin);
   SSP_CHECK_ARG(ldin % 4 == 0 && ldin >= Cin, "conv: ldin must be a multiple of 4 and >= Cin");
@@ -510,6 +524,11 @@
     SSP_CHECK_ARG(bnb->nslot >= 1, "conv: the BatchNorm-backward partial buffer needs at least one row");
     a.bn_nslot = bnb->nslot;
   }
+  if (adj) {
+    SSP_CHECK_ARG(R == 3 && ssp_wino_plan_tile(plan) && !ssp_wino_plan_fused(plan),
+                  "conv (adjoint data gradient): needs a through-memory Winograd plan (8xxxxxx / 9xxxxxx), got %d", plan);
+    return wino_launch(a, B, H, W, ws, ws_floats, plan, prof_kind, stream, true, dM);
+  }
   if (ssp_wino_plan_fused(plan)) {
     a.ksplit = 1; a.ws = nullptr;
     return ssp_wino_fused_launch(a, B, H, W, prof_kind, stream);
diff --git a/singleshotpose_amd/csrc/conv_wgrad.hip b/singleshotpose_amd/csrc/conv_wgrad.hip
--- a/singleshotpose_amd/csrc/conv_wgrad.hip
+++ b/singleshotpose_amd/csrc/conv_wgrad.hip
@@ -374,7 +374,10 @@
 }
 int ssp_conv_wgrad_wino_launch(const float* dy, const float* x, float* dw, int B, int H, int W, int Cin, int Cout, int lddy,
                                int ldx, int tile, float* ws, int64_t ws_floats, hipStream_t stream) {
-  if (tile == SSP_WINO_WGRAD_FUSED) return ssp_wino_wgrad_fused_launch(dy, x, dw, B, H, W, Cin, Cout, lddy, ldx, ws, ws_floats, stream);
+  if (tile == SSP_WINO_WGRAD_FUSED) {
+    SSP_CHECK_ARG(dy != nullptr, "wgrad (Winograd, both transforms on the chip): dy must be given (no dM in memory to share)");
+    return ssp_wino_wgrad_fused_launch(dy, x, dw, B, H, W, Cin, Cout, lddy, ldx, ws, ws_floats, stream);
+  }
   SSP_CHECK_ARG(tile == 2 || tile == 4, "wgrad (Winograd): tile must be 2, 4 or 12 (F(2x2) with both transforms on the chip)");
   SSP_CHECK_ARG(Cin % 16 == 0 && Cout % 16 == 0 && Cin >= 64 && Cout >= 64, "wgrad (Winograd): needs Cin, Cout >= 64 and %% 16 == 0");
   SSP_CHECK_ARG(ldx % 4 == 0 && ldx >= Cin && lddy % 4 == 0 && lddy >= Cout, "wgrad (Winograd): bad leading dimensions");
@@ -391,7 +394,8 @@
   float* dU = dM + P * T * Cout;
   if (x != nullptr)
     if (int rc = ssp_wino_input_launch(x, ldx, V, B, H, W, Cin, tile, SSP_PROF_WINO_WGRAD, stream)) return rc;
-  if (int rc = ssp_wino_outgrad_launch(dy, lddy, dM, B, H, W, Cout, tile, stream)) return rc;
+  if (dy != nullptr)
+    if (int rc = ssp_wino_outgrad_launch(dy, lddy, dM, B, H, W, Cout, tile, stream)) return rc;
   const int r = ssp_conv_wgrad_dma_try(dM, V, dU, 1, 1, (int)T, Cin, Cout, Cout, Cin, 1, stream, P, T * Cout, T * Cin,
                                        (int64_t)Cout * Cin, 1);
   if (r < 0) return r;
diff --git a/singleshotpose_amd/csrc/conv_wino.h b/singleshotpose_amd/csrc/conv_wino.h
--- a/singleshotpose_amd/csrc/conv_wino.h
+++ b/singleshotpose_amd/csrc/conv_wino.h
@@ -36,10 +36,12 @@
 int ssp_wino_planes(int tile);
 int64_t ssp_wino_stat_groups(int B, int H, int W, int tile);
 int ssp_wino_input_launch(const float* in, int ldin, float* V, int B, int H, int W, int C, int tile, int prof_kind, hipStream_t stream);
-int ssp_wino_filter_launch(const float* w, float* U, int rows, int K, int tile, hipStream_t stream);
-int ssp_wino_outgrad_launch(const float* dy, int lddy, float* dM, int B, int H, int W, int C, int tile, hipStream_t stream);
+int ssp_wino_filter_launch(const float* w, float* U, int rows, int K, int tile, hipStream_t stream, bool flip = false);
+int ssp_wino_outgrad_launch(const float* dy, int lddy, float* dM, int B, int H, int W, int C, int tile, hipStream_t stream,
+                            int prof_kind = SSP_PROF_WINO_WGRAD);
 int ssp_wino_wgrad_finish_launch(const float* dU, float* dw, int rows, int K, int tile, hipStream_t stream);
-int ssp_wino_output_launch(const WinoOutArgs& a, int B, int H, int W, int tile, int prof_kind, hipStream_t stream);
+int ssp_wino_output_launch(const WinoOutArgs& a, int B, int H, int W, int tile, int prof_kind, hipStream_t stream,
+                           bool adj = false);
 
 struct ConvArgs;
 int ssp_wino_fused_launch(const ConvArgs& a, int B, int H, int W, int prof_kind, hipStream_t stream);
diff --git a/singleshotpose_amd/csrc/conv_wino.hip b/singleshotpose_amd/csrc/conv_wino.hip
--- a/singleshotpose_amd/csrc/conv_wino.hip
+++ b/singleshotpose_amd/csrc/conv_wino.hip
@@ -138,7 +138,7 @@
   });
 }
 
-template <int N>
+template <int N, bool FLIP = false>
 __global__ void __launch_bounds__(256) wino_filter_kernel(const float* __restrict__ w, float* __restrict__ U, int rows, int K) {
   constexpr int A = N + 2;
   using M_ = WinoMat<N>;
@@ -152,7 +152,7 @@
 #pragma unroll
   for (int i = 0; i < 3; ++i)
 #pragma unroll
-    for (int j = 0; j < 3; ++j) g[i][j] = *reinterpret_cast<const f32x4*>(src + (int64_t)(i * 3 + j) * K);
+    for (int j = 0; j < 3; ++j) g[i][j] = *reinterpret_cast<const f32x4*>(src + (int64_t)(FLIP ? 8 - (i * 3 + j) : i * 3 + j) * K);
   f32x4 h[A][3];
   ssp_sfor<A>([&](auto I) {
     constexpr int i = decltype(I)::value;
@@ -182,12 +182,101 @@
   });
 }
 
-template <int N, int CS>
-__global__ void __launch_bounds__(256) wino_output_kernel(WinoOutArgs p, WinoGeom g) {
+template <int N>
+__device__ __forceinline__ void wino_form_output(f32x4 (&Y)[N][N], const float* __restrict__ src, const int64_t plane) {
   constexpr int A = N + 2;
+  using M_ = WinoMat<N>;
+  const f32x4 z4 = {0.f, 0.f, 0.f, 0.f};
+  ssp_sfor<A>([&](auto I) {
+    constexpr int i = decltype(I)::value;
+    f32x4 m[A];
+#pragma unroll
+    for (int j = 0; j < A; ++j) m[j] = *reinterpret_cast<const f32x4*>(src + (int64_t)(i * A + j) * plane);
+    ssp_sfor<N>([&](auto Q) {
+      constexpr int qq = decltype(Q)::value;
+      f32x4 rr = z4;
+      ssp_sfor<A>([&](auto J) {
+        constexpr int j = decltype(J)::value;
+        { constexpr float cc_ = M_::AT[qq][j]; wino_mad(rr, cc_, m[j]); }
+      });
+      ssp_sfor<N>([&](auto Pp) {
+        constexpr int pp = decltype(Pp)::value;
+        { constexpr float cc_ = M_::AT[pp][i]; wino_mad(Y[pp][qq], cc_, rr); }
+      });
+    });
+  });
+}
+
+template <int N>
+__device__ __forceinline__ void wino_form_adjoint(f32x4 (&Y)[N][N], const float* __restrict__ src, const int64_t plane,
+                                                  const int C, const WinoGeom& g, const int ty, const int tx) {
+  constexpr int A = N + 2;
+  using M_ = WinoMat<N>;
+  const f32x4 z4 = {0.f, 0.f, 0.f, 0.f};
+  constexpr float c0 = M_::BT[0][0], cl = M_::BT[A - 1][A - 1];
+  constexpr float c00 = c0 * c0, c0l = c0 * cl, cll = cl * cl;
+  ssp_sfor<A>([&](auto I) {
+    constexpr int i = decltype(I)::value;
+    f32x4 m[A];
+#pragma unroll
+    for (int j = 0; j < A; ++j) m[j] = *reinterpret_cast<const f32x4*>(src + (int64_t)(i * A + j) * plane);
+    ssp_sfor<N>([&](auto Q) {
+      constexpr int qq = decltype(Q)::value;
+      f32x4 rr = z4;
+      ssp_sfor<A>([&](auto J) {
+        constexpr int j = decltype(J)::value;
+        { constexpr float cc_ = M_::BT[j][qq + 1]; wino_mad(rr, cc_, m[j]); }
+      });
+      ssp_sfor<N>([&](auto Pp) {
+        constexpr int pp = decltype(Pp)::value;
+        { constexpr float cc_ = M_::BT[i][pp + 1]; wino_mad(Y[pp][qq], cc_, rr); }
+      });
+    });
+  });
+  const bool up = ty > 0, dn = ty + 1 < g.th, lf = tx > 0, rt = tx + 1 < g.tw;
+  const int64_t trow = (int64_t)g.tw * C;
+  auto vertical = [&](const float* __restrict__ s, auto PR, auto OR, const float ce, const float cleft, const float cright) {
+    constexpr int pr = decltype(PR)::value, orow = decltype(OR)::value;
+    f32x4 m[A];
+#pragma unroll
+    for (int j = 0; j < A; ++j) m[j] = *reinterpret_cast<const f32x4*>(s + (int64_t)(pr * A + j) * plane);
+    ssp_sfor<N>([&](auto Q) {
+      constexpr int qq = decltype(Q)::value;
+      f32x4 rr = z4;
+      ssp_sfor<A>([&](auto J) {
+        constexpr int j = decltype(J)::value;
+        { constexpr float cc_ = M_::BT[j][qq + 1]; wino_mad(rr, cc_, m[j]); }
+      });
+      wino_mad(Y[orow][qq], ce, rr);
+    });
+    if (lf) wino_mad(Y[orow][0], cleft, *reinterpret_cast<const f32x4*>(s - C + (int64_t)(pr * A + A - 1) * plane));
+    if (rt) wino_mad(Y[orow][N - 1], cright, *reinterpret_cast<const f32x4*>(s + C + (int64_t)(pr * A) * plane));
+  };
+  if (up) vertical(src - trow, std::integral_constant<int, A - 1>{}, std::integral_constant<int, 0>{}, cl, cll, c0l);
+  if (dn) vertical(src + trow, std::integral_constant<int, 0>{}, std::integral_constant<int, N - 1>{}, c0, c0l, c00);
+  auto horizontal = [&](const float* __restrict__ s, auto PC, auto OC, const float ce) {
+    constexpr int pc = decltype(PC)::value, ocol = decltype(OC)::value;
+    f32x4 m[A];
+#pragma unroll
+    for (int i = 0; i < A; ++i) m[i] = *reinterpret_cast<const f32x4*>(s + (int64_t)(i * A + pc) * plane);
+    ssp_sfor<N>([&](auto Pp) {
+      constexpr int pp = decltype(Pp)::value;
+      f32x4 rr = z4;
+      ssp_sfor<A>([&](auto I) {
+        constexpr int i = decltype(I)::value;
+        { constexpr float cc_ = M_::BT[i][pp + 1]; wino_mad(rr, cc_, m[i]); }
+      });
+      wino_mad(Y[pp][ocol], ce, rr);
+    });
+  };
+  if (lf) horizontal(src - C, std::integral_constant<int, A - 1>{}, std::integral_constant<int, 0>{}, cl);
+  if (rt) horizontal(src + C, std::integral_constant<int, 0>{}, std::integral_constant<int, N - 1>{}, c0);
+}
+
+template <int N, int CS, bool ADJ>
+__device__ __forceinline__ void wino_finish_body(const WinoOutArgs& p, const WinoGeom& g) {
   constexpr int TP = 256 / CS;
   constexpr int NP = SSP_WINO_TG / TP;
-  using M_ = WinoMat<N>;
   const int tid = threadIdx.x, gl = tid % CS, tl = tid / CS;
   const int c = blockIdx.y * (CS * 4) + gl * 4;
   const bool cok = c < p.Cout;
@@ -221,24 +310,8 @@
     const int ty = (int)(q - (unsigned)mb * (unsigned)g.th);
     const float* src = p.Mw + t64 * p.Cout + c;
     const int64_t plane = g.T * p.Cout;
-    ssp_sfor<A>([&](auto I) {
-      constexpr int i = decltype(I)::value;
-      f32x4 m[A];
-#pragma unroll
-      for (int j = 0; j < A; ++j) m[j] = *reinterpret_cast<const f32x4*>(src + (int64_t)(i * A + j) * plane);
-      ssp_sfor<N>([&](auto Q) {
-        constexpr int qq = decltype(Q)::value;
-        f32x4 rr = z4;
-        ssp_sfor<A>([&](auto J) {
-          constexpr int j = decltype(J)::value;
-          { constexpr float cc_ = M_::AT[qq][j]; wino_mad(rr, cc_, m[j]); }
-        });
-        ssp_sfor<N>([&](auto Pp) {
-          constexpr int pp = decltype(Pp)::value;
-          { constexpr float cc_ = M_::AT[pp][i]; wino_mad(Y[pp][qq], cc_, rr); }
-        });
-      });
-    });
+    if constexpr (ADJ) wino_form_adjoint<N>(Y, src, plane, p.Cout, g, ty, tx);
+    else wino_form_output<N>(Y, src, plane);
     float cnt = 0.f;
     f32x4 sum = z4;
     unsigned valid = 0u;
@@ -342,6 +415,16 @@
       if (ch == 0) p.stats[(int64_t)gridDim.x * p.Cout * 2 + blockIdx.x] = n_;
     }
   }
+}
+
+template <int N, int CS>
+__global__ void __launch_bounds__(256) wino_output_kernel(WinoOutArgs p, WinoGeom g) {
+  wino_finish_body<N, CS, false>(p, g);
+}
+template <int N, int CS>
+__global__ void __launch_bounds__(256) __attribute__((amdgpu_waves_per_eu(CS == 16 ? 2 : 1)))
+wino_dgrad_finish_kernel(WinoOutArgs p, WinoGeom g) {
+  wino_finish_body<N, CS, true>(p, g);
 }
 
 template <int N, int CV, bool NT = false>
@@ -456,7 +539,8 @@
 int ssp_wino_planes(int tile) { return (tile + 2) * (tile + 2); }
 int64_t ssp_wino_stat_groups(int B, int H, int W, int tile) { return (ssp_wino_tiles(B, H, W, tile) + SSP_WINO_TG - 1) / SSP_WINO_TG; }
 
-int ssp_wino_outgrad_launch(const float* dy, int lddy, float* dM, int B, int H, int W, int C, int tile, hipStream_t stream) {
+int ssp_wino_outgrad_launch(const float* dy, int lddy, float* dM, int B, int H, int W, int C, int tile, hipStream_t stream,
+                            int prof_kind) {
   SSP_CHECK_ARG(wino_tile_ok(tile), "wino_outgrad: tile must be 2 or 4");
   const WinoGeom g = wino_geom(B, H, W, tile);
   const int wv = ssp_option(SSP_OPT_WINO_VARIANT);
@@ -465,7 +549,7 @@
                 "wino_outgrad: channels must be a multiple of 4 and the operands 16-byte aligned");
   SSP_CHECK_ARG(g.T * (C / cv) < (1ll << 31), "wino_outgrad: too many (tile, channel) pairs");
   const int P = ssp_wino_planes(tile);
-  SspProfScope prof(SSP_PROF_WINO_WGRAD, stream, 4.0 * C * ((double)B * H * W + (double)P * g.T));
+  SspProfScope prof(prof_kind, stream, 4.0 * C * ((double)B * H * W + (double)P * g.T));
   const int64_t n = g.T * (C / cv);
   const SspFastDiv dc = ssp_fastdiv((unsigned)(C / cv));
   const dim3 grid((unsigned)((n + 255) / 256));
@@ -512,26 +596,37 @@
   return SSP_OK;
 }
 
-int ssp_wino_filter_launch(const float* w, float* U, int rows, int K, int tile, hipStream_t stream) {
+int ssp_wino_filter_launch(const float* w, float* U, int rows, int K, int tile, hipStream_t stream, bool flip) {
   SSP_CHECK_ARG(wino_tile_ok(tile), "wino_filter: tile must be 2 or 4");
   SSP_CHECK_ARG(w != nullptr && U != nullptr && rows > 0 && K > 0 && K % 4 == 0 && (((uintptr_t)w) & 15) == 0 &&
                     (((uintptr_t)U) & 15) == 0,
                 "wino_filter: [rows][9][K] filters with K % 4 == 0, 16-byte aligned operands");
   SspProfScope prof(SSP_PROF_LAYOUT, stream, 4.0 * (9.0 + ssp_wino_planes(tile)) * (double)rows * K);
   const int64_t n = (int64_t)rows * (K / 4);
-  if (tile == 2) hipLaunchKernelGGL(wino_filter_kernel<2>, dim3((unsigned)((n + 255) / 256)), dim3(256), 0, stream, w, U, rows, K);
-  else hipLaunchKernelGGL(wino_filter_kernel<4>, dim3((unsigned)((n + 255) / 256)), dim3(256), 0, stream, w, U, rows, K);
+  const dim3 grid((unsigned)((n + 255) / 256));
+  if (tile == 2 && flip) hipLaunchKernelGGL((wino_filter_kernel<2, true>), grid, dim3(256), 0, stream, w, U, rows, K);
+  else if (tile == 2) hipLaunchKernelGGL((wino_filter_kernel<2>), grid, dim3(256), 0, stream, w, U, rows, K);
+  else if (flip) hipLaunchKernelGGL((wino_filter_kernel<4, true>), grid, dim3(256), 0, stream, w, U, rows, K);
+  else hipLaunchKernelGGL((wino_filter_kernel<4>), grid, dim3(256), 0, stream, w, U, rows, K);
   SSP_CHECK_LAUNCH("wino_filter");
   return SSP_OK;
 }
 
-int ssp_wino_output_launch(const WinoOutArgs& a, int B, int H, int W, int tile, int prof_kind, hipStream_t stream) {
+int ssp_wino_output_launch(const WinoOutArgs& a, int B, int H, int W, int tile, int prof_kind, hipStream_t stream, bool adj) {
   SSP_CHECK_ARG(wino_tile_ok(tile), "wino_output: tile must be 2 or 4");
   const WinoGeom g = wino_geom(B, H, W, tile);
   const int P = ssp_wino_planes(tile);
   SspProfScope prof(prof_kind, stream, 4.0 * a.Cout * ((double)B * H * W * (a.accumulate ? 2.0 : 1.0) * (a.bn_partial ? 2.0 : 1.0) + (double)P * g.T));
   const bool wide = a.Cout >= 256 && (ssp_option(SSP_OPT_WINO_VARIANT) & 4);
   const dim3 grid((unsigned)((g.T + SSP_WINO_TG - 1) / SSP_WINO_TG), (unsigned)ssp_cdiv(a.Cout, wide ? 256 : 64));
+  if (adj) {
+    if (tile == 2 && wide) hipLaunchKernelGGL((wino_dgrad_finish_kernel<2, 64>), grid, dim3(256), 0, stream, a, g);
+    else if (tile == 2) hipLaunchKernelGGL((wino_dgrad_finish_kernel<2, 16>), grid, dim3(256), 0, stream, a, g);
+    else if (wide) hipLaunchKernelGGL((wino_dgrad_finish_kernel<4, 64>), grid, dim3(256), 0, stream, a, g);
+    else hipLaunchKernelGGL((wino_dgrad_finish_kernel<4, 16>), grid, dim3(256), 0, stream, a, g);
+    SSP_CHECK_LAUNCH("wino_dgrad_finish");
+    return SSP_OK;
+  }
   if (tile == 2 && wide) hipLaunchKernelGGL((wino_output_kernel<2, 64>), grid, dim3(256), 0, stream, a, g);
   else if (tile == 2) hipLaunchKernelGGL((wino_output_kernel<2, 16>), grid, dim3(256), 0, stream, a, g);
   else if (wide) hipLaunchKernelGGL((wino_output_kernel<4, 64>), grid, dim3(256), 0, stream, a, g);
diff --git a/singleshotpose_amd/csrc/ssp_api.hip b/singleshotpose_amd/csrc/ssp_api.hip
--- a/singleshotpose_amd/csrc/ssp_api.hip
+++ b/singleshotpose_amd/csrc/ssp_api.hip
@@ -10,8 +10,10 @@
 int ssp_conv_igemm_launch(const float* in, const float* wt, float* out, const float* bias, float* stats, int B, int H,
                           int W, int Cin, int Cout, int ldin, int ldout, int R, int accumulate, float* ws,
                           int64_t ws_floats, int plan, int prof_kind, hipStream_t stream,
-                          const float* escale = nullptr, float act_slope = 1.f, const SspBnBwdFuse* bnb = nullptr);
+                          const float* escale = nullptr, float act_slope = 1.f, const SspBnBwdFuse* bnb = nullptr,
+                          bool adj = false, const float* dM = nullptr);
 int64_t ssp_wino_ws_floats(int B, int H, int W, int Cin, int Cout, int tile);
+int64_t ssp_wino_adj_ws_floats(int B, int H, int W, int Cout_dy, int Cin_dx, int tile, bool own_dm);
 int ssp_conv_wgrad_launch(const float* dy, const float* x, float* dw, int B, int H, int W, int Cin, int Cout, int lddy,
                           int ldx, int R, hipStream_t stream);
 int64_t ssp_conv_wgrad_wino_ws_floats(int B, int H, int W, int Cin, int Cout, int tile);
@@ -264,6 +266,37 @@
   return ssp_conv_igemm_launch(dy, wt, dx, nullptr, nullptr, B, H, W, Cout_dy, Cin_dx, lddy, lddx, R, 0, workspace,
                                workspace_floats, plan, SSP_PROF_CONV_DGRAD, (hipStream_t)stream, nullptr, 1.f, &f);
 }
+int ssp_wino_outgrad_transform_t(const float* dy, int lddy, float* dM, int B, int H, int W, int C, int tile, void* stream) {
+  return ssp_wino_outgrad_launch(dy, lddy, dM, B, H, W, C, tile, (hipStream_t)stream, SSP_PROF_WINO_DGRAD);
+}
+int ssp_wino_filter_transform_adj_t(const float* w9d, float* Ut, int rows, int K, int tile, void* stream) {
+  return ssp_wino_filter_launch(w9d, Ut, rows, K, tile, (hipStream_t)stream, true);
+}
+int64_t ssp_conv_dgrad_adj_workspace_floats(int B, int H, int W, int Cout_dy, int Cin_dx, int plan, int own_dm) {
+  const int tile = ssp_wino_plan_tile(plan);
+  if (!tile || ssp_wino_plan_fused(plan)) return 0;
+  return ssp_wino_adj_ws_floats(B, H, W, Cout_dy, Cin_dx, tile, own_dm != 0);
+}
+int ssp_conv_dgrad_adj(const float* dy, const float* wt, float* dx, int B, int H, int W, int Cout_dy, int Cin_dx, int lddy,
+                       int lddx, int R, int accumulate, int plan, float* workspace, int64_t workspace_floats,
+                       const float* dM, void* stream) {
+  return ssp_conv_igemm_launch(dy, wt, dx, nullptr, nullptr, B, H, W, Cout_dy, Cin_dx, lddy, lddx, R, accumulate,
+                               workspace, workspace_floats, plan, SSP_PROF_CONV_DGRAD, (hipStream_t)stream, nullptr, 1.f,
+                               nullptr, true, dM);
+}
+int ssp_conv_dgrad_adj_bnbwd(const float* dy, const float* wt, float* dx, int B, int H, int W, int Cout_dy, int Cin_dx,
+                             int lddy, int lddx, int R, int plan, float* workspace, int64_t workspace_floats,
+                             const float* raw, int ldraw, const float* scale, const float* shift, const float* mean,
+                             const float* invstd, float slope, float* partial, int partial_rows, const float* dM,
+                             void* stream) {
+  SspBnBwdFuse f = {raw, ldraw, scale, shift, mean, invstd, slope, partial, partial_rows};
+  if (partial == nullptr) {
+    ssp_set_error("conv_dgrad_adj_bnbwd: partial must not be NULL (use ssp_conv_dgrad_adj)");
+    return SSP_ERR_ARG;
+  }
+  return ssp_conv_igemm_launch(dy, wt, dx, nullptr, nullptr, B, H, W, Cout_dy, Cin_dx, lddy, lddx, R, 0, workspace,
+                               workspace_floats, plan, SSP_PROF_CONV_DGRAD, (hipStream_t)stream, nullptr, 1.f, &f, true, dM);
+}
 int ssp_bn_act_bwd_partials(const float* x, int ldx, const float* g, int ldg, float* dx, int lddx, const float* scale,
                             const float* shift, const float* mean, const float* invstd, int C, int B, int H, int W,
                             float slope, int training, float* partial, int npartial, int zero_after, float* dgamma,
diff --git a/singleshotpose_amd/engine.py b/singleshotpose_amd/engine.py
--- a/singleshotpose_amd/engine.py
+++ b/singleshotpose_amd/engine.py
@@ -15,6 +15,9 @@
                12823, 6423, 6424, 206414, 212813, 406413, 406414, 412813)
 IGEMM_LATENCY_CANDS = (6418, 12818, 6428, 12828, 6438)
 WINO_GEMM_CANDS = (6413, 6414, 12813, 12814)
+
+
+_SHARE_DM = os.environ.get('SSP_WINO_SHARE_DM', '1') != '0'
 
 
 def _tune_tag():
@@ -181,6 +184,7 @@
     wino_u = wino_ud = None
     wino_ws = wino_ws_floats = None
     wgrad_wino = 0
+    dgrad_adj = False
     ws_dgrad = 0
     fwd_fams = None
     stats = None
@@ -708,6 +712,11 @@
         self._plan_bn_fusion()
         self._fit_workspace()
 
+    def _adjoint_rule(self, cs):
+        t = wino_tile(cs.plan_dgrad)
+        return bool(_SHARE_DM and not cs.first and t and not wino_fused(cs.plan_dgrad) and cs.wgrad_wino == t and
+                    cs.coutp == cs.cout)
+
     def _wgrad_key(self, cs):
         return ('wgrad', self.B, cs.H, cs.W, cs.cinp, cs.cout, cs.ldraw, cs.inp.ld, _tune_tag())
 
@@ -842,9 +851,11 @@
         _lib.call('ssp_repack_dgrad_packed' if cs.packed else 'ssp_repack_dgrad', src.data_ptr(),
                   _ptr(self._dpack, cs.doff), cs.cout, cs.cin, cs.coutp, cs.k, stream.cuda_stream)
         tile = wino_tile(cs.plan_dgrad)
+        cs.dgrad_adj = self._adjoint_rule(cs)
         if tile:
-            _lib.call('ssp_wino_filter_transform_t', _ptr(self._dpack, cs.doff), self._wino_ud(cs, tile).data_ptr(), cs.cin,
-                      cs.coutp, tile, stream.cuda_stream)
+            _lib.call('ssp_wino_filter_transform_adj_t' if cs.dgrad_adj else 'ssp_wino_filter_transform_t',
+                      _ptr(self._dpack, cs.doff), self._wino_ud(cs, tile).data_ptr(), cs.cin, cs.coutp, tile,
+                      stream.cuda_stream)
 
     def _autotune(self, which):
         B = self.B
@@ -1384,24 +1395,25 @@
             self.grads[ind] = g
         return g
 
-    def _dgrad(self, cs, src, dy_ptr, dy_ld, written, fused_stats, st, fold=True):
+    def _dgrad(self, cs, src, dy_ptr, dy_ld, written, fused_stats, st, fold=True, dm_ptr=None):
         call = _lib.call
         B = self.B
         gin = self._grad_buf(src, cs.inp)
         scs = cs.bn_fuse_src
         dwt = (self._wino_ud(cs, wino_tile(cs.plan_dgrad)).data_ptr() if wino_tile(cs.plan_dgrad)
                else _ptr(self._dpack, cs.doff))
+        adj = (dm_ptr, st) if cs.dgrad_adj else (st,)
         if scs is not None and fold and src not in written:
             sv = scs.vec
-            call('ssp_conv_dgrad_bnbwd', dy_ptr, dwt, gin.ptr, B, cs.H, cs.W,
+            call('ssp_conv_dgrad_adj_bnbwd' if cs.dgrad_adj else 'ssp_conv_dgrad_bnbwd', dy_ptr, dwt, gin.ptr, B, cs.H, cs.W,
                  cs.coutp, cs.cin, dy_ld, gin.ld, cs.k, cs.plan_dgrad, self.ws.data_ptr(), self.ws_floats,
                  scs.raw.data_ptr(), scs.ldraw, sv[2].data_ptr(), sv[3].data_ptr(), sv[0].data_ptr(),
-                 sv[1].data_ptr(), scs.slope, scs.bnp[0].data_ptr(), scs.bnp[1], st)
+                 sv[1].data_ptr(), scs.slope, scs.bnp[0].data_ptr(), scs.bnp[1], *adj)
             fused_stats.add(src)
         else:
-            call('ssp_conv_dgrad', dy_ptr, dwt, gin.ptr, B, cs.H, cs.W, cs.coutp,
+            call('ssp_conv_dgrad_adj' if cs.dgrad_adj else 'ssp_conv_dgrad', dy_ptr, dwt, gin.ptr, B, cs.H, cs.W, cs.coutp,
                  cs.cin, dy_ld, gin.ld, cs.k, 1 if src in written else 0, cs.plan_dgrad, self.ws.data_ptr(),
-                 self.ws_floats, st)
+                 self.ws_floats, *adj)
         written.add(src)
 
     def backward(self, grad_out, want_input=False, want_params=True):
@@ -1621,16 +1633,22 @@
         src = None if cs.first else cs.inp.producer
         owner = None if src is None else (self.convs.get(src - 1) if src in self.fused_pool else self.convs.get(src))
         defer = params and tail_sched and owner is not None and owner.first_live and s.dgrad[0]
+        dm_ptr = None
+        if cs.dgrad_adj and s.dgrad[0] and s.wgrad and cs.packed and cs.wgrad_wino:
+            t = cs.wgrad_wino
+            dm_ptr = _ptr(self._wino_ws(cs), (t + 2) ** 2 * _lib.query('ssp_conv_wino_tiles', B, cs.H, cs.W, t) * cs.cinp)
+            call('ssp_wino_outgrad_transform_t', dy_ptr, dy_ld, dm_ptr, B, cs.H, cs.W, cs.cout, cs.wgrad_wino, st)
         if defer:
-            self._dgrad(cs, src, dy_ptr, dy_ld, written, fused_stats, st, s.fold_bn)
+            self._dgrad(cs, src, dy_ptr, dy_ld, written, fused_stats, st, s.fold_bn, dm_ptr)
         if params:
             side.wait_stream(main)
         if s.wgrad:
             gw = gview(cs.conv.weight, cs.packed)
             if cs.packed and cs.wgrad_wino:
                 wws = self._wino_ws(cs)
-                call('ssp_conv_wgrad_wino_t', dy_ptr, None if cs.v_live else cs.inp.ptr, gw.data_ptr(),
-                     B, cs.H, cs.W, cs.cinp, cs.cout, dy_ld, cs.inp.ld, cs.wgrad_wino, wws.data_ptr(), wws.numel(), st2)
+                call('ssp_conv_wgrad_wino_t', None if dm_ptr is not None else dy_ptr, None if cs.v_live else cs.inp.ptr,
+                     gw.data_ptr(), B, cs.H, cs.W, cs.cinp, cs.cout, dy_ld, cs.inp.ld, cs.wgrad_wino, wws.data_ptr(),
+                     wws.numel(), st2)
                 cs.v_live = False
             elif cs.packed:
                 call('ssp_conv_wgrad', dy_ptr, cs.inp.ptr, gw.data_ptr(), B, cs.H, cs.W, cs.cinp, cs.cout, dy_ld,
@@ -1647,7 +1665,7 @@
             if cs.first:
                 self._input_dgrad(cs, dy_ptr, dy_ld, written, st)
             else:
-                self._dgrad(cs, src, dy_ptr, dy_ld, written, fused_stats, st, s.fold_bn)
+                self._dgrad(cs, src, dy_ptr, dy_ld, written, fused_stats, st, s.fold_bn, dm_ptr)
 
     def _input_gbuf(self, written):
         gin = self._grad_buf(INPUT, self.input_act)
```

New measurement: 2594 images/s, median of 6. 1.02x the previous value.
